# NVlabs/ODISE

Hardware: AMD Instinct MI355X
Metric: panoptic-inference images/sec @1024x1024 (higher is better)
Workload: dtype f16

## Files before the change

### include/odise_hip_tools.h

```cpp
#ifndef ODISE_HIP_TOOLS_H
#define ODISE_HIP_TOOLS_H

#include "odise_hip.h"

#ifdef __cplusplus
extern "C" {
#endif

int odise_hip_sizeof_gemm_desc(void);
int odise_hip_sizeof_conv_desc(void);
int odise_hip_sizeof_attn_desc(void);
int odise_hip_sizeof_post_desc(void);
int odise_hip_sizeof_infer_desc(void);

int odise_hip_gemm_forced(odise_hip_ctx* ctx, const odise_gemm_desc* d, int tile, int splitk);
int odise_hip_conv2d_forced(odise_hip_ctx* ctx, const odise_conv_desc* d, int tile, int splitk);
int odise_hip_last_tile(void);
int odise_hip_gemm_ln(odise_hip_ctx* ctx, const odise_gemm_desc* d, const float* part, int parts, float inv_c, float eps, const float* colsum,
                      float* final_out, const float* fin, const float* rowsum, float* stats_out);
int odise_hip_conv2d_gn_forced(odise_hip_ctx* ctx, const odise_conv_desc* d, int tile, int splitk, const float* gamma, const float* beta,
                               int groups, float eps, int act, void* y_norm, float* stats_scratch, int* stats_blocks);
int odise_hip_gemm_debug(int flags);

int odise_hip_post_generic(int on);
int odise_hip_sem_tile(int tile);
int odise_hip_gn_tuning(int chunk_factor, int fold_in_apply);
int odise_hip_msda_unfused(int on);
int odise_hip_msda_fused_forward(odise_hip_ctx* ctx, const void* value, const float* off, const float* aw, const int* hs3, const int* ws3, int B, int M, int fused,
                                 void* out, float* loc_scratch, float* w_scratch);

int odise_hip_stage_timeline(odise_hip_ctx* ctx, int on);
int odise_hip_stage_timeline_read(odise_hip_ctx* ctx, char* names, int names_cap, float* gpu_ms, double* host_ms, int cap, int* n);

int odise_hip_prefetch_stats(odise_hip_ctx* ctx, int* enqueued, int* hits, int* dropped, int* failed);

int odise_hip_launch_log(odise_hip_ctx* ctx, int on);
int odise_hip_launch_log_read(odise_hip_ctx* ctx, int* out6, int cap, int* n);

int odise_hip_set_lanes(odise_hip_ctx* ctx, int lanes);

int odise_hip_backbone_maps(odise_hip_ctx* ctx, float** out4, int* shape_bchw4x4);

int odise_hip_mfma_probe(odise_hip_ctx* ctx, float* host_out);

int odise_hip_maskclip_token_mask(odise_hip_ctx* ctx, const void* logits_f16, void* out_u8, int B, int Q, int h, int w, int S, int patch, int T,
                                  int64_t ldm, int plain);
#ifdef __cplusplus
}
#endif
#endif
```

### odise_amd/csrc/common.h

```cpp
#pragma once
#include <hip/hip_runtime.h>
#include <hip/hip_fp16.h>
#include <stdint.h>
#include <stdio.h>
#include <atomic>
#include <string>

#include "../../include/odise_hip.h"

namespace odise {

typedef _Float16 f16;
typedef _Float16 f16x4 __attribute__((ext_vector_type(4)));
typedef _Float16 f16x8 __attribute__((ext_vector_type(8)));
typedef float f32x4 __attribute__((ext_vector_type(4)));
typedef float f32x16 __attribute__((ext_vector_type(16)));

void set_error(const char* fmt, ...);

#define ODISE_CHECK_HIP(expr)                                                              \
    do {                                                                                   \
        hipError_t _e = (expr);                                                            \
        if (_e != hipSuccess) {                                                            \
            ::odise::set_error("%s:%d: %s failed: %s", __FILE__, __LINE__, #expr,          \
                               hipGetErrorString(_e));                                     \
            return ODISE_ERR_HIP;                                                          \
        }                                                                                  \
    } while (0)

#define ODISE_REQUIRE(cond, ...)                                                           \
    do {                                                                                   \
        if (!(cond)) {                                                                     \
            ::odise::set_error(__VA_ARGS__);                                               \
            return ODISE_ERR_ARG;                                                          \
        }                                                                                  \
    } while (0)

#define ODISE_TRY(expr)                \
    do {                               \
        int _rc = (expr);              \
        if (_rc != ODISE_OK) return _rc; \
    } while (0)

static inline int64_t ceil_div(int64_t a, int64_t b) { return (a + b - 1) / b; }
static inline int64_t round_up(int64_t a, int64_t b) { return ceil_div(a, b) * b; }

__device__ __forceinline__ float mul_sigmoid(float x, float kx) { return x * __builtin_amdgcn_rcpf(1.0f + __expf(-kx)); }

__device__ __forceinline__ float gelu_erf(float v) {
    const float x = v * 0.70710678118654752f;
    const float a = fabsf(x);
    const float t = __builtin_amdgcn_rcpf(1.0f + 0.3275911f * a);
    const float p = t * (0.254829592f + t * (-0.284496736f + t * (1.421413741f + t * (-1.453152027f + t * 1.061405429f))));
    const float r = 1.0f - p * __expf(-a * a);
    return 0.5f * v * (1.0f + copysignf(r, x));
}

__device__ __forceinline__ float act_apply(float v, int act) {
    switch (act) {
        case ODISE_ACT_SILU: return mul_sigmoid(v, v);
        case ODISE_ACT_RELU: return v > 0.f ? v : 0.f;
        case ODISE_ACT_GELU: return gelu_erf(v);
        case ODISE_ACT_QUICKGELU: return mul_sigmoid(v, 1.702f * v);
        default: return v;
    }
}

}

struct odise_hip_ctx {
    int device = 0;
    hipStream_t stream = nullptr;
    bool own_stream = false;
    int cu_count = 256;
    int max_lds_optin = 65536;
    void* ws = nullptr;
    size_t ws_bytes = 0;
    void* zeros = nullptr;
    hipEvent_t ev0 = nullptr, ev1 = nullptr;
    void* models = nullptr;
    void* jpeg_host = nullptr;
    size_t jpeg_host_bytes = 0;
    void* jpeg_dev = nullptr;
    size_t jpeg_dev_bytes = 0;
    hipEvent_t jpeg_ev = nullptr;
    hipStream_t stream2 = nullptr;
    void* ws2 = nullptr;
    hipEvent_t ev_fork = nullptr, ev_mid = nullptr, ev_join = nullptr;
    hipEvent_t ev_mclip = nullptr;
    int lanes = 2;
    int prefetch_cu_eighths = 0;
    int prefetch_start = 1;
    hipStream_t stream3 = nullptr;
    void* ws3 = nullptr;
    hipEvent_t ev_pf_go = nullptr, ev_pf_done = nullptr;
    void* comm = nullptr;
    int clip_ln_fold = 0;
    int maskclip_passes = 0;
    int attn_kv_resident = 0;
    int64_t vae_chunk_bytes = 0;
    void* probe = nullptr;
    void* stages = nullptr;
    void* launch_log = nullptr;
    void* rle_buf = nullptr;
    size_t rle_bytes = 0;
};

namespace odise {
struct LdsAttrOnce {
    std::atomic<uint64_t> done{0};
};
static inline int ensure_dyn_lds(odise_hip_ctx* ctx, LdsAttrOnce& once, const void* kernel, int bytes) {
    const int d = ctx->device;
    if (d >= 0 && d < 64 && ((once.done.load(std::memory_order_acquire) >> d) & 1)) return ODISE_OK;
    ODISE_CHECK_HIP(hipFuncSetAttribute(kernel, hipFuncAttributeMaxDynamicSharedMemorySize, bytes));
    if (d >= 0 && d < 64) once.done.fetch_or(1ull << d, std::memory_order_release);
    return ODISE_OK;
}
}

namespace odise {
struct LaunchProbe {
    int conv = 0, M = 0, N = 0, K = 0;
    int cap = 0, n = 0;
    hipEvent_t* ev = nullptr;
    bool armed = false;
};
static inline LaunchProbe* probe_match(odise_hip_ctx* ctx, bool conv, int M, int N, int K) {
    LaunchProbe* p = (LaunchProbe*)ctx->probe;
    return (p && p->armed && p->n < p->cap && (p->conv != 0) == conv && p->M == M && p->N == N && p->K == K) ? p : nullptr;
}
void probe_release(odise_hip_ctx* ctx);
void stage_mark(odise_hip_ctx* ctx, const char* name);
void stage_log_release(odise_hip_ctx* ctx);
struct LaunchRec { int conv, M, N, K, tile, split; };
void launch_log_push(odise_hip_ctx* ctx, const LaunchRec& r);
void launch_log_release(odise_hip_ctx* ctx);
constexpr int kLnPartCols = 64;
struct LnEpi {
    const float* part = nullptr;
    int P = 0;
    float inv_c = 0.f, eps = 0.f;
    const float* colsum = nullptr;
    float* final_out = nullptr;
    const float* fin = nullptr;
    const float* rowsum = nullptr;
    float* stats_out = nullptr;
};
bool conv3_c8_ok(const odise_conv_desc* d);
int launch_conv3_c8(odise_hip_ctx* ctx, const odise_conv_desc* d, float* gn_stats, int* stats_blocks);
int gemm_forced(odise_hip_ctx* ctx, const odise_gemm_desc* d, int force_tile, int force_split, const LnEpi* ln = nullptr);
int gemm_ln(odise_hip_ctx* ctx, const odise_gemm_desc* d, const LnEpi& ln);
void jpeg_release(odise_hip_ctx* ctx);
void rle_release(odise_hip_ctx* ctx);
void comm_release(odise_hip_ctx* ctx);
}
```

### odise_amd/csrc/engine.cpp

```cpp
#include <stdlib.h>

#include "engine.h"

#include <string.h>

namespace odise {

void unet_destroy(ModelStore* ms);
void extractor_destroy(ModelStore* ms);
void maskgen_destroy(ModelStore* ms);
void classify_destroy(ModelStore* ms);

ModelStore* store_of(odise_hip_ctx* ctx) {
    if (!ctx->models) ctx->models = new ModelStore();
    return (ModelStore*)ctx->models;
}

void free_allocs(std::vector<void*>& owned) {
    if (owned.empty()) return;
    (void)hipDeviceSynchronize();
    for (void* p : owned) (void)hipFree(p);
    owned.clear();
}

void models_destroy(odise_hip_ctx* ctx) {
    if (!ctx->models) return;
    ModelStore* ms = (ModelStore*)ctx->models;
    unet_destroy(ms);
    extractor_destroy(ms);
    maskgen_destroy(ms);
    classify_destroy(ms);
    for (void* p : ms->dev_allocs) (void)hipFree(p);
    if (ms->arena.base) (void)hipFree(ms->arena.base);
    if (ms->arena2.base) (void)hipFree(ms->arena2.base);
    if (ms->mclip.buf) (void)hipFree(ms->mclip.buf);
    for (Arena& a : ms->pf.arena)
        if (a.base) (void)hipFree(a.base);
    delete ms;
    ctx->models = nullptr;
}

int ensure_prefetch_lane(odise_hip_ctx* ctx, ModelStore* ms, int slot, size_t arena_bytes) {
    if (!ctx->stream3) {
        int lo = 0, hi = 0;
        ODISE_CHECK_HIP(hipDeviceGetStreamPriorityRange(&lo, &hi));
        const int e8 = ctx->prefetch_cu_eighths;
        hipStream_t st = nullptr;
        void* ws = nullptr;
        hipEvent_t go = nullptr, done = nullptr;
        hipError_t err;
        if (e8 >= 1 && e8 <= 7) {
            uint32_t mask[8];
            const uint32_t byte = (1u << e8) - 1u;
            for (uint32_t& m : mask) m = byte * 0x01010101u;
            err = hipExtStreamCreateWithCUMask(&st, 8, mask);
        } else {
            err = hipStreamCreateWithPriority(&st, hipStreamNonBlocking, lo);
        }
        if (err == hipSuccess) err = hipMalloc(&ws, ctx->ws_bytes);
        if (err == hipSuccess) err = hipEventCreateWithFlags(&go, hipEventDisableTiming);
        if (err == hipSuccess) err = hipEventCreateWithFlags(&done, hipEventDisableTiming);
        if (err != hipSuccess) {
            if (done) (void)hipEventDestroy(done);
            if (go) (void)hipEventDestroy(go);
            if (ws) (void)hipFree(ws);
            if (st) (void)hipStreamDestroy(st);
            set_error("prefetch lane: %s", hipGetErrorString(err));
            return ODISE_ERR_HIP;
        }
        ctx->stream3 = st; ctx->ws3 = ws; ctx->ev_pf_go = go; ctx->ev_pf_done = done;
    }
    Arena& a = ms->pf.arena[slot];
    if (a.cap < arena_bytes) {
        ODISE_CHECK_HIP(hipStreamSynchronize(ctx->stream3));
        ODISE_CHECK_HIP(hipStreamSynchronize(ctx->stream));
        if (a.base) ODISE_CHECK_HIP(hipFree(a.base));
        a = Arena();
        ODISE_CHECK_HIP(hipMalloc((void**)&a.base, arena_bytes));
        a.cap = arena_bytes;
    }
    return ODISE_OK;
}

int ensure_lane2(odise_hip_ctx* ctx, ModelStore* ms, size_t arena_bytes) {
    if (!ctx->stream2) {
        int lo = 0, hi = 0;
        ODISE_CHECK_HIP(hipDeviceGetStreamPriorityRange(&lo, &hi));
        int prio = hi;
#ifdef ODISE_TOOLS
        if (getenv("ODISE_LANE2_NORMAL_PRIORITY")) prio = lo;
#endif
        ODISE_CHECK_HIP(hipStreamCreateWithPriority(&ctx->stream2, hipStreamNonBlocking, prio));
        ODISE_CHECK_HIP(hipMalloc(&ctx->ws2, ctx->ws_bytes));
        ODISE_CHECK_HIP(hipEventCreateWithFlags(&ctx->ev_fork, hipEventDisableTiming));
        ODISE_CHECK_HIP(hipEventCreateWithFlags(&ctx->ev_mid, hipEventDisableTiming));
        ODISE_CHECK_HIP(hipEventCreateWithFlags(&ctx->ev_join, hipEventDisableTiming));
        ODISE_CHECK_HIP(hipEventCreateWithFlags(&ctx->ev_mclip, hipEventDisableTiming));
    }
    if (ms->arena2.cap < arena_bytes) {
        ODISE_CHECK_HIP(hipStreamSynchronize(ctx->stream));
        ODISE_CHECK_HIP(hipStreamSynchronize(ctx->stream2));
        if (ms->arena2.base) ODISE_CHECK_HIP(hipFree(ms->arena2.base));
        ms->arena2 = Arena();
        ODISE_CHECK_HIP(hipMalloc((void**)&ms->arena2.base, arena_bytes));
        ms->arena2.cap = arena_bytes;
    }
    return ODISE_OK;
}

const HostTensor* Packer::find(const std::string& key) {
    auto it = ms->host.find(prefix + key);
    if (it == ms->host.end()) {
        if (missing.empty()) missing = prefix + key;
        return nullptr;
    }
    return &it->second;
}

int Packer::upload(const void* host, size_t bytes, void** dev) {
    ODISE_CHECK_HIP(hipMalloc(dev, bytes ? bytes : 16));
    ms->track(*dev);
    ODISE_CHECK_HIP(hipMemcpy(*dev, host, bytes, hipMemcpyHostToDevice));
    return ODISE_OK;
}

int Packer::vec_f32(const std::string& key, float** out, int64_t expect) {
    const HostTensor* t = find(key);
    if (!t) {
        set_error("weights: missing key '%s'", (prefix + key).c_str());
        return ODISE_ERR_STATE;
    }
    if (t->numel() != expect) {
        set_error("weights: '%s' has %lld elements, expected %lld", (prefix + key).c_str(), (long long)t->numel(), (long long)expect);
        return ODISE_ERR_STATE;
    }
    return upload(t->data.data(), t->data.size() * sizeof(float), (void**)out);
}

int Packer::conv(const std::string& key, ConvW& out, bool bias) {
    const HostTensor* t = find(key + ".weight");
    if (!t || t->shape.size() != 4) {
        set_error("weights: missing or non-4D conv weight '%s.weight'", (prefix + key).c_str());
        return ODISE_ERR_STATE;
    }
    const int O = (int)t->shape[0], I = (int)t->shape[1], KH = (int)t->shape[2], KW = (int)t->shape[3];
    if (KH != KW) {
        set_error("weights: non-square conv kernel '%s'", (prefix + key).c_str());
        return ODISE_ERR_STATE;
    }
    const int Ip = (int)round_up(I, 8);
    std::vector<f16> packed((size_t)O * KH * KW * Ip, (f16)0.f);
    for (int o = 0; o < O; ++o)
        for (int i = 0; i < I; ++i)
            for (int y = 0; y < KH; ++y)
                for (int x = 0; x < KW; ++x)
                    packed[(((size_t)o * KH + y) * KW + x) * Ip + i] = (f16)t->data[(((size_t)o * I + i) * KH + y) * KW + x];
    out.cin = I; out.cin_pad = Ip; out.cout = O; out.k = KH;
    ODISE_TRY(upload(packed.data(), packed.size() * sizeof(f16), (void**)&out.w));
    out.b = nullptr;
    if (bias) ODISE_TRY(vec_f32(key + ".bias", &out.b, O));
    return ODISE_OK;
}

int Packer::linear(const std::string& key, LinW& out, bool bias) {
    const HostTensor* t = find(key + ".weight");
    if (!t || t->shape.size() < 2) {
        set_error("weights: missing linear weight '%s.weight'", (prefix + key).c_str());
        return ODISE_ERR_STATE;
    }
    const int O = (int)t->shape[0], I = (int)t->shape[1];
    if (t->numel() != (int64_t)O * I || I % 8 != 0) {
        set_error("weights: '%s.weight' is not a [O,I] / [O,I,1,1] matrix with I %% 8 == 0", (prefix + key).c_str());
        return ODISE_ERR_STATE;
    }
    std::vector<f16> packed((size_t)O * I);
    for (size_t i = 0; i < packed.size(); ++i) packed[i] = (f16)t->data[i];
    out.in = I; out.out = O;
    ODISE_TRY(upload(packed.data(), packed.size() * sizeof(f16), (void**)&out.w));
    out.b = nullptr;
    if (bias) ODISE_TRY(vec_f32(key + ".bias", &out.b, O));
    return ODISE_OK;
}

int Packer::norm(const std::string& key, NormW& out) {
    const HostTensor* t = find(key + ".weight");
    if (!t) {
        set_error("weights: missing norm weight '%s.weight'", (prefix + key).c_str());
        return ODISE_ERR_STATE;
    }
    out.c = (int)t->numel();
    ODISE_TRY(vec_f32(key + ".weight", &out.g, out.c));
    ODISE_TRY(vec_f32(key + ".bias", &out.b, out.c));
    return ODISE_OK;
}

void* Exec::alloc_bytes(size_t bytes) {
    void* p = ms->arena.alloc(bytes);
    if (!p) set_error("arena exhausted: need %zu more bytes (capacity %zu, used %zu)", bytes, ms->arena.cap, ms->arena.off);
    return p;
}

int Exec::alloc(Act& a, int n, int h, int w, int c) {
    a.n = n; a.h = h; a.w = w; a.c = c;
    a.p = (f16*)alloc_bytes((size_t)a.elems() * sizeof(f16));
    return a.p ? ODISE_OK : ODISE_ERR_NOMEM;
}

int Exec::gemm(const odise_gemm_desc& d) {
    ms->macs += (double)d.M * d.N * d.K * (d.batch > 1 ? d.batch : 1);
    return odise_hip_gemm(ctx, &d);
}

int Exec::attention(const odise_attn_desc& d) {
    ms->macs += 2.0 * d.B * d.H * (double)d.Lq * d.Lk * d.D;
    return odise_hip_attention(ctx, &d);
}

int Exec::conv(const Act& x, const ConvW& w, Act& y, int stride, int pad, bool upsample, const Act* residual,
               const float* per_image_add, int64_t pia_ld, int act, int pad_t, int pad_l, int oh, int ow) {
    if (x.c != w.cin_pad) {
        set_error("conv: input has %d channels, weight expects %d", x.c, w.cin_pad);
        return ODISE_ERR_ARG;
    }
    if (pad < 0) pad = w.k / 2;
    if (pad_t < 0) pad_t = pad;
    if (pad_l < 0) pad_l = pad;
    const int hin = upsample ? 2 * x.h : x.h, win = upsample ? 2 * x.w : x.w;
    if (oh < 0) oh = (hin + 2 * pad - w.k) / stride + 1;
    if (ow < 0) ow = (win + 2 * pad - w.k) / stride + 1;
    if (!y.p) ODISE_TRY(alloc(y, x.n, oh, ow, w.cout));
    odise_conv_desc d;
    memset(&d, 0, sizeof(d));
    d.N = x.n; d.H = x.h; d.W = x.w; d.Cin = x.c;
    d.Cout = w.cout; d.KH = w.k; d.KW = w.k; d.stride = stride; d.pad_t = pad_t; d.pad_l = pad_l; d.OH = oh; d.OW = ow;
    d.upsample2x = upsample ? 1 : 0;
    d.X = x.p; d.Wt = w.w; d.Y = y.p; d.y_dtype = ODISE_F16;
    d.bias = w.b;
    d.residual = residual ? residual->p : nullptr;
    d.per_image_add = per_image_add;
    d.per_image_add_ld = pia_ld;
    d.act = act;
    ms->macs += (double)x.n * oh * ow * w.cout * w.k * w.k * w.cin;
    y.gn_blocks = 0;
#ifdef ODISE_TOOLS
    if (y.gn_part && getenv("ODISE_NO_GN_FUSION")) return odise_hip_conv2d(ctx, &d);
#endif
    if (y.gn_part) return conv_forced(ctx, &d, -1, 0, y.gn_part, &y.gn_blocks);
    return odise_hip_conv2d(ctx, &d);
}

int Exec::alloc_gn_stats(Act& a) {
    const int64_t blocks = ceil_div((int64_t)a.h * a.w, 64);
    a.gn_part = (float*)alloc_bytes((size_t)a.n * blocks * a.c * 2 * sizeof(float));
    a.gn_blocks = 0;
    return a.gn_part ? ODISE_OK : ODISE_ERR_NOMEM;
}

int Exec::linear(const f16* x, int64_t M, const LinW& w, f16* y, int act, const f16* residual, bool geglu) {
    odise_gemm_desc d;
    memset(&d, 0, sizeof(d));
    d.M = (int)M; d.N = w.out; d.K = w.in;
    d.A = x; d.lda = w.in;
    d.W = w.w; d.ldw = w.in;
    d.C = y; d.ldc = geglu ? w.out / 2 : w.out; d.c_dtype = ODISE_F16;
    d.bias_n = w.b;
    d.residual = residual; d.ldr = d.ldc;
    d.act = act; d.geglu = geglu ? 1 : 0; d.alpha = 1.f; d.batch = 1;
    return gemm(d);
}

int Exec::group_norm(const Act& x, const NormW& w, Act& y, float eps, int act) {
    if (!y.p) ODISE_TRY(alloc(y, x.n, x.h, x.w, x.c));
    if (x.gn_part && x.gn_blocks > 0)
        return group_norm_from_colpart(ctx, x.p, y.p, w.g, w.b, x.n, x.h * x.w, x.c, 32, eps, act, x.gn_part, x.gn_blocks);
    return odise_hip_group_norm(ctx, x.p, y.p, w.g, w.b, x.n, x.h * x.w, x.c, 32, eps, act);
}

int Exec::layer_norm(const f16* x, f16* y, int64_t rows, const NormW& w, float eps) {
    return odise_hip_layer_norm(ctx, x, y, w.g, w.b, (int)rows, w.c, eps);
}

}

using namespace odise;

extern "C" int odise_hip_load_weight(odise_hip_ctx* ctx, const char* name, const float* host_data, const int64_t* shape, int ndim) {
    ODISE_REQUIRE(ctx && name && host_data && (ndim == 0 || shape), "load_weight: null argument");
    ODISE_REQUIRE(ndim >= 0 && ndim <= 4, "load_weight: rank %d not in [0,4]", ndim);
    ModelStore* ms = store_of(ctx);
    HostTensor t;
    int64_t n = 1;
    for (int i = 0; i < ndim; ++i) {
        ODISE_REQUIRE(shape[i] >= 0, "load_weight: negative dim");
        t.shape.push_back(shape[i]);
        n *= shape[i];
    }
    t.data.assign(host_data, host_data + n);
    ms->host[std::string(name)] = std::move(t);
    return ODISE_OK;
}

extern "C" int odise_hip_clear_host_weights(odise_hip_ctx* ctx) {
    ODISE_REQUIRE(ctx, "clear_host_weights: null context");
    store_of(ctx)->host.clear();
    return ODISE_OK;
}
```

### odise_amd/csrc/engine.h

```cpp
#pragma once
#include <map>
#include <utility>
#include <string>
#include <vector>

#include "common.h"

namespace odise {

struct HostTensor {
    std::vector<float> data;
    std::vector<int64_t> shape;
    int64_t numel() const {
        int64_t n = 1;
        for (auto s : shape) n *= s;
        return n;
    }
};

struct Arena {
    char* base = nullptr;
    size_t cap = 0, off = 0, peak = 0;
    void* alloc(size_t bytes) {
        off = (off + 255) & ~(size_t)255;
        if (off + bytes > cap) return nullptr;
        void* p = base + off;
        off += bytes;
        if (off > peak) peak = off;
        return p;
    }
    size_t mark() const { return off; }
    void release(size_t m) { off = m; }
    void reset() { off = 0; }
};

struct Act {
    f16* p = nullptr;
    int n = 0, h = 0, w = 0, c = 0;
    float* gn_part = nullptr;
    int gn_blocks = 0;
    int64_t pixels() const { return (int64_t)n * h * w; }
    int64_t elems() const { return pixels() * c; }
};

struct ConvW {
    f16* w = nullptr;
    float* b = nullptr;
    int cin = 0, cin_pad = 0, cout = 0, k = 1;
};
struct LinW {
    f16* w = nullptr;
    float* b = nullptr;
    int in = 0, out = 0;
};
struct NormW {
    float* g = nullptr;
    float* b = nullptr;
    int c = 0;
};

struct UNetModel;

struct EncoderOut {
    Act tap0, tap1;
    Act xt, zdec;
};
struct PrefetchKey {
    int B = 0, layout = 0;
    std::vector<const void*> images;
    std::vector<int> hw;
    bool operator==(const PrefetchKey& o) const { return B == o.B && layout == o.layout && images == o.images && hw == o.hw; }
};
struct Prefetch {
    bool has_pending = false, has_ready = false;
    PrefetchKey pending, ready;
    int ready_slot = 0;
    EncoderOut out;
    int crops = 0;
    bool use_now = false;
    int n_enqueued = 0, n_hits = 0, n_dropped = 0, n_failed = 0;
    Arena arena[2];
};

struct ClipKV {
    void* buf = nullptr;
    size_t cap = 0;
    f16* qk = nullptr;
    f16* vt = nullptr;
    f16* cls = nullptr;
    int B = 0, TP = 0, layers = 0, width = 0;
    size_t qk_stride = 0, vt_stride = 0;
    int64_t ldvt = 0;
    const float* plan_image = nullptr;
    int plan_B = 0, plan_H = 0, plan_W = 0;
    bool planned = false, ready = false, on_lane2 = false;
};

struct ModelStore {
    std::map<std::string, HostTensor> host;
    std::vector<void*> dev_allocs;
    std::vector<void*>* alloc_sink = nullptr;
    void track(void* p) { (alloc_sink ? *alloc_sink : dev_allocs).push_back(p); }
    Arena arena;
    Arena arena2;
    Prefetch pf;
    ClipKV mclip;
    UNetModel* unet = nullptr;
    struct ExtractorModel* extractor = nullptr;
    struct MaskGenModel* maskgen = nullptr;
    struct ClassifyModel* classify = nullptr;
    double macs = 0.0;
};

ModelStore* store_of(odise_hip_ctx* ctx);
struct AllocScope {
    ModelStore* ms;
    std::vector<void*>* prev;
    AllocScope(ModelStore* m, std::vector<void*>& owned) : ms(m), prev(m->alloc_sink) { m->alloc_sink = &owned; }
    ~AllocScope() { ms->alloc_sink = prev; }
};
void free_allocs(std::vector<void*>& owned);

struct Packer {
    odise_hip_ctx* ctx;
    ModelStore* ms;
    std::string prefix;
    std::string missing;

    const HostTensor* find(const std::string& key);
    int upload(const void* host, size_t bytes, void** dev);
    int conv(const std::string& key, ConvW& out, bool bias = true);
    int linear(const std::string& key, LinW& out, bool bias = true);
    int norm(const std::string& key, NormW& out);
    int vec_f32(const std::string& key, float** out, int64_t expect);
};

struct Exec {
    odise_hip_ctx* ctx;
    ModelStore* ms;
    int alloc(Act& a, int n, int h, int w, int c);
    int alloc_gn_stats(Act& a);
    void* alloc_bytes(size_t bytes);

    int conv(const Act& x, const ConvW& w, Act& y, int stride = 1, int pad = -1, bool upsample = false, const Act* residual = nullptr,
             const float* per_image_add = nullptr, int64_t pia_ld = 0, int act = ODISE_ACT_NONE, int pad_t = -1, int pad_l = -1,
             int oh = -1, int ow = -1);
    int linear(const f16* x, int64_t M, const LinW& w, f16* y, int act = ODISE_ACT_NONE, const f16* residual = nullptr,
               bool geglu = false);
    int group_norm(const Act& x, const NormW& w, Act& y, float eps, int act);
    int layer_norm(const f16* x, f16* y, int64_t rows, const NormW& w, float eps);
    int gemm(const odise_gemm_desc& d);
    int attention(const odise_attn_desc& d);
};


int ensure_lane2(odise_hip_ctx* ctx, ModelStore* ms, size_t arena_bytes);
struct Lane2 {
    odise_hip_ctx* ctx;
    ModelStore* ms;
    hipStream_t s0;
    void* w0;
    Lane2(odise_hip_ctx* c, ModelStore* m) : ctx(c), ms(m), s0(c->stream), w0(c->ws) {
        ctx->stream = ctx->stream2;
        ctx->ws = ctx->ws2;
        std::swap(ms->arena, ms->arena2);
    }
    ~Lane2() {
        ctx->stream = s0;
        ctx->ws = w0;
        std::swap(ms->arena, ms->arena2);
    }
};

int ensure_prefetch_lane(odise_hip_ctx* ctx, ModelStore* ms, int slot, size_t arena_bytes);
struct PrefetchLane {
    odise_hip_ctx* ctx;
    ModelStore* ms;
    int slot;
    hipStream_t s0;
    void* w0;
    void* stages0;
    PrefetchLane(odise_hip_ctx* c, ModelStore* m, int sl) : ctx(c), ms(m), slot(sl), s0(c->stream), w0(c->ws), stages0(c->stages) {
        ctx->stream = ctx->stream3;
        ctx->ws = ctx->ws3;
        ctx->stages = nullptr;
        std::swap(ms->arena, ms->pf.arena[slot]);
    }
    ~PrefetchLane() {
        ctx->stream = s0;
        ctx->ws = w0;
        ctx->stages = stages0;
        std::swap(ms->arena, ms->pf.arena[slot]);
    }
};

int ensure_arena(odise_hip_ctx* ctx, ModelStore* ms, size_t bytes);
int unet_build(odise_hip_ctx* ctx, const char* prefix);
int unet_prepare_timestep(odise_hip_ctx* ctx, ModelStore* ms, UNetModel* u, int B, int t);
int unet_launch(odise_hip_ctx* ctx, ModelStore* ms, UNetModel* u, const float* x_t, const f16* x_nhwc, const float* context,
                const float* cond_emb, int B, int h, int w, bool standalone);
const Act* unet_taps(ModelStore* ms);
size_t extractor_arena_bytes(int B, int H, int W);
const Act* extractor_taps(ModelStore* ms);
bool extractor_ready(ModelStore* ms);
int extractor_launch(odise_hip_ctx* ctx, ModelStore* ms, const float* image, int B, int H, int W, bool standalone, bool join = true);
int extractor_join(odise_hip_ctx* ctx);
int extractor_encoder_only(odise_hip_ctx* ctx, ModelStore* ms, const float* image, int B, int H, int W, EncoderOut& out);
size_t encoder_arena_bytes(int B, int H, int W);

struct LatentW {
    float wq[4][8];
    float bq[4];
    float wp[4][4];
    float bp[4];
    float scale, qa, qb;
};
int launch_latent_heads(odise_hip_ctx* ctx, const f16* h, const float* noise, f16* xt, f16* zdec, float* latent, int B, int P,
                        const LatentW& w);
int launch_image_to_nhwc(odise_hip_ctx* ctx, const float* x, f16* y, int N, int C, int HW, int Cpad, const float* scale3,
                         const float* shift3);
int launch_clip_preprocess(odise_hip_ctx* ctx, const float* x, f16* y, int N, int H, int W, int S);
int launch_softmax_rows(odise_hip_ctx* ctx, const f16* x, f16* y, int64_t rows, int cols, int64_t ld, float scale);
int launch_clip_assemble(odise_hip_ctx* ctx, const f16* patches, const float* cls, const float* pos, f16* tok, int B, int T, int extra,
                         int TP, int Cw);
int clip_tower(Exec& ex, const Act& img, int extra, const uint8_t* mask, int64_t ldm, f16* out, ClipKV* kv = nullptr, int kv_images = 0);
bool maskclip_kv_available(odise_hip_ctx* ctx, ModelStore* ms, int B);
int maskclip_image_pass(Exec& ex, const float* image01, int B, int H, int W);
int maskclip_mask_pass(Exec& ex, int Q, const uint8_t* mask, int64_t ldm, int64_t stride_mask, f16* out);
int maskclip_planned_pass(odise_hip_ctx* ctx, ModelStore* ms);
int clip_dims(ModelStore* ms, int* image, int* patch, int* tokens, int* out_dim);
int launch_cond_inputs(odise_hip_ctx* ctx, const float* proj, const float* A1, const float* A2, float* out, int B, int T, int Cw);


int launch_crop_extract(odise_hip_ctx* ctx, const float* img, float* crops, int B, int C, int H, int W, int S, int K, const int* boxes_dev);
int launch_crop_resize_bicubic(odise_hip_ctx* ctx, const float* img, float* crops, int B, int C, int H, int W, int s, int S, int K, const int* boxes_dev);
int launch_upsample_nearest(odise_hip_ctx* ctx, const f16* x, f16* y, int N, int H, int W, int OH, int OW, int C);
int launch_stitch(odise_hip_ctx* ctx, const f16* feat, f16* out, float* out_nchw, int B, int K, const int* boxes_dev, int ch, int cw, int OH,
                  int OW, int C);
int launch_broadcast_rows(odise_hip_ctx* ctx, const f16* x, f16* y, int64_t n, int B);
int layer_norm_add_table(odise_hip_ctx* ctx, const void* x, void* y, const float* gamma, const float* beta, int rows, int C, float eps, f16* y2,
                         const float* table, int P);
int launch_add_vec_table(odise_hip_ctx* ctx, const f16* x, const float* vec, const float* table, f16* y, int64_t N, int P, int C);
bool msda_fused_ok(int M, int D, int L, int P);
int launch_msda_fused(odise_hip_ctx* ctx, const f16* value, const float* off, const float* aw, f16* out, const int* Hs, const int* Ws, const int* starts, int B,
                      int S, int M, int Lq, int ld_off = 0, int ld_aw = 0);
int launch_msda_prepare(odise_hip_ctx* ctx, const float* off, const float* aw, float* loc, float* w, int B, int Lq, int M, int L, int P,
                        const int* Hs, const int* Ws, const int* starts);
int launch_bilinear_add(odise_hip_ctx* ctx, const f16* a, const f16* b, f16* y, int N, int H, int W, int OH, int OW, int C);
int launch_mask_binarize_f16(odise_hip_ctx* ctx, const f16* mask, f16* m01, float* inv, int64_t rows, int HW);
int launch_attn_mask(odise_hip_ctx* ctx, const f16* logits, uint8_t* out, int64_t rows, int H, int W, int oh, int ow, int64_t ldm);
int launch_attn_mask_f32(odise_hip_ctx* ctx, const float* logits, uint8_t* out, int64_t rows, int H, int W, int oh, int ow, int64_t ldm);


struct PostGeom {
    int h4, w4;
    int ph, pw;
    int ih, iw;
    int oh, ow;
    int Q, Qpad;
};
int launch_resize_bilinear_norm(odise_hip_ctx* ctx, const float* x, f16* y, int B, int H, int W, int S);
int launch_maskclip_token_mask(odise_hip_ctx* ctx, const f16* logits, uint8_t* out, int B, int Q, int h, int w, int S, int patch, int T,
                               int64_t ldm);
int launch_l2_normalize_f16(odise_hip_ctx* ctx, const f16* x, f16* y, int64_t rows, int C);
int launch_l2_normalize_f32(odise_hip_ctx* ctx, const float* x, f16* y, int64_t rows, int C);
int launch_classify_rows(odise_hip_ctx* ctx, const float* L1, const float* L2, const int* seg, const int* ovl, const float* binary, float* out, int64_t rows, int K,
                         int Ktot, float ls1, float ls2, float alpha, float beta);
int launch_postprocess_pixels(odise_hip_ctx* ctx, const f16* logits, const float* kscore, f16* S, int* ids, int* counts, const PostGeom& g, const f16* PT = nullptr,
                              float* sem = nullptr, int K = 0, unsigned int* stats_partial = nullptr);
bool postprocess_pixels_tiled(const PostGeom& g);
int postprocess_pixels_stat_blocks(const PostGeom& g);
int launch_column_fold(odise_hip_ctx* ctx, const unsigned int* partial, float* out2, int nb, int Qpad);
bool postprocess_pixels_fuses_semantic(const PostGeom& g);
int launch_column_stats(odise_hip_ctx* ctx, const f16* S, unsigned int* partial, float* out2, int npix, int Qpad);
int launch_panoptic_write(odise_hip_ctx* ctx, const int* ids, const int* map, int* seg, int npix);
int launch_instance_masks(odise_hip_ctx* ctx, const f16* logits, const int* idx, float* out, int n, const PostGeom& g, const int* n_dev = nullptr);
bool instance_masks_x4(const PostGeom& g);
int launch_post_decide(odise_hip_ctx* ctx, const float* mask_cls, float* kscore, int* label, f16* semT, float* probs, int B, int Q, int Qpad, int K,
                       float object_mask_threshold);
int launch_panoptic_decide(odise_hip_ctx* ctx, const int* counts, const float* kscore, const int* label, const uint8_t* isthing, int* map, int* table,
                           int Q, int K, double overlap_threshold, int max_segments, int* stuff_scratch);
int launch_instance_topk(odise_hip_ctx* ctx, const float* probs, const float* inst_stats, const uint8_t* isthing, int* table, float* scores, int B,
                         int Q, int Qpad, int K, int topk, int things_only);
int launch_image_pad(odise_hip_ctx* ctx, const void* src, int layout, int h, int w, float* dst, int Hp, int Wp);
int launch_semantic_argmax(odise_hip_ctx* ctx, const f16* S, const f16* PT, int* out, int npix, int Qpad, int K);
struct HeadOutputs {
    const f16* pred_masks;
    const f16* mask_embed;
    int B, Q, C, h4, w4;
    float logit_scale;
    const float* class_logits;
};
int head_outputs(ModelStore* ms, HeadOutputs* out);
void maskgen_invalidate_outputs(ModelStore* ms);

int conv_forced(odise_hip_ctx* ctx, const odise_conv_desc* d, int force_tile, int force_split, float* gn_stats, int* stats_blocks);
int group_norm_from_colpart(odise_hip_ctx* ctx, const void* x, void* y, const float* gamma, const float* beta, int N, int HW, int C, int groups,
                            float eps, int act, const float* colpart, int nblk);

}
```

### odise_amd/csrc/extractor.cpp

```cpp
#include <math.h>
#include <string.h>

#include <functional>
#include "engine.h"

namespace odise {

struct VaeRes {
    NormW n1, n2;
    ConvW c1, c2, nin;
    bool has_nin = false;
};
struct VaeAttn {
    NormW norm;
    LinW qk, v, proj;
    float* v_bias = nullptr;
    int c = 0;
};
struct ClipBlock {
    NormW ln1, ln2;
    LinW qk, v, out, fc, proj;
    float* v_bias = nullptr;
    LinW qk_f, v_f, fc_f;
    float *qk_cs = nullptr, *v_cs = nullptr, *fc_cs = nullptr, *v_f_bias = nullptr;
};

struct ExtractorModel {
    std::vector<void*> owned;
    bool built = false;
    ConvW enc_conv_in, enc_conv_out;
    VaeRes enc_blocks[4][2];
    ConvW enc_down[3];
    VaeRes enc_mid1, enc_mid2;
    VaeAttn enc_attn;
    NormW enc_norm_out;
    ConvW dec_conv_in;
    VaeRes dec_mid1, dec_mid2;
    VaeAttn dec_attn;
    VaeRes dec_l3[3], dec_l2[2];
    ConvW dec_up3;
    LatentW lat;
    float* noise = nullptr;
    int noise_hw = 0;
    ConvW clip_conv1;
    float *clip_cls = nullptr, *clip_pos = nullptr;
    NormW clip_ln_pre, clip_ln_post;
    std::vector<ClipBlock> clip_blocks;
    LinW clip_proj;
    int clip_width = 0, clip_heads = 16, clip_tokens = 0, clip_image = 336, clip_patch = 14, clip_out = 768;
    LinW cap_proj;
    LinW cap_time;
    float *cap_A1 = nullptr, *cap_A2 = nullptr;
    int ctx_dim = 768, ted = 1280;
    Act taps[8];
    double last_macs = 0.0;
};

void extractor_destroy(ModelStore* ms) {
    if (ms->extractor) free_allocs(ms->extractor->owned);
    delete ms->extractor;
    ms->extractor = nullptr;
}

static int build_vae_res(Packer& pk, const std::string& key, VaeRes& r) {
    ODISE_TRY(pk.norm(key + ".norm1", r.n1));
    ODISE_TRY(pk.conv(key + ".conv1", r.c1));
    ODISE_TRY(pk.norm(key + ".norm2", r.n2));
    ODISE_TRY(pk.conv(key + ".conv2", r.c2));
    r.has_nin = pk.find(key + ".nin_shortcut.weight") != nullptr;
    if (r.has_nin) ODISE_TRY(pk.conv(key + ".nin_shortcut", r.nin));
    return ODISE_OK;
}

static int build_vae_attn(Packer& pk, const std::string& key, VaeAttn& a) {
    ODISE_TRY(pk.norm(key + ".norm", a.norm));
    a.c = a.norm.c;
    const HostTensor *wq = pk.find(key + ".q.weight"), *wk = pk.find(key + ".k.weight"), *bq = pk.find(key + ".q.bias"),
                     *bk = pk.find(key + ".k.bias");
    const size_t cc = (size_t)a.c * a.c;
    if (!wq || !wk || !bq || !bk || (size_t)wq->numel() != cc || (size_t)wk->numel() != cc) {
        set_error("vae: bad or missing '%s.q/k'", key.c_str());
        return ODISE_ERR_STATE;
    }
    std::vector<f16> qk(2 * cc);
    std::vector<float> b(2 * (size_t)a.c);
    for (size_t i = 0; i < cc; ++i) { qk[i] = (f16)wq->data[i]; qk[cc + i] = (f16)wk->data[i]; }
    for (int i = 0; i < a.c; ++i) { b[i] = bq->data[i]; b[a.c + i] = bk->data[i]; }
    a.qk.in = a.c; a.qk.out = 2 * a.c;
    ODISE_TRY(pk.upload(qk.data(), qk.size() * sizeof(f16), (void**)&a.qk.w));
    ODISE_TRY(pk.upload(b.data(), b.size() * sizeof(float), (void**)&a.qk.b));
    ODISE_TRY(pk.linear(key + ".v", a.v, false));
    ODISE_TRY(pk.vec_f32(key + ".v.bias", &a.v_bias, a.c));
    ODISE_TRY(pk.linear(key + ".proj_out", a.proj));
    return ODISE_OK;
}

static int fold_layer_norm(Packer& pk, const float* W, const float* bias, int O, int I, const float* gamma, const float* beta, LinW& lw, float** bias_dev,
                           float** cs_dev) {
    std::vector<f16> wf((size_t)O * I);
    std::vector<float> bf(O), cs(O);
    for (int o = 0; o < O; ++o) {
        double bb = bias[o], c = 0.0;
        for (int i = 0; i < I; ++i) {
            const float w = W[(size_t)o * I + i];
            const f16 h = (f16)(w * gamma[i]);
            wf[(size_t)o * I + i] = h;
            c += (double)(float)h;
            bb += (double)w * beta[i];
        }
        bf[o] = (float)bb;
        cs[o] = (float)c;
    }
    lw.in = I; lw.out = O; lw.b = nullptr;
    ODISE_TRY(pk.upload(wf.data(), wf.size() * sizeof(f16), (void**)&lw.w));
    ODISE_TRY(pk.upload(bf.data(), bf.size() * sizeof(float), (void**)bias_dev));
    ODISE_TRY(pk.upload(cs.data(), cs.size() * sizeof(float), (void**)cs_dev));
    return ODISE_OK;
}

static int build_clip_block(Packer& pk, const std::string& key, ClipBlock& b, int W) {
    ODISE_TRY(pk.norm(key + ".ln_1", b.ln1));
    ODISE_TRY(pk.norm(key + ".ln_2", b.ln2));
    const HostTensor* w = pk.find(key + ".attn.in_proj_weight");
    const HostTensor* bias = pk.find(key + ".attn.in_proj_bias");
    if (!w || !bias || w->numel() != (int64_t)3 * W * W || bias->numel() != 3 * W) {
        set_error("clip: bad or missing '%s.attn.in_proj_*'", key.c_str());
        return ODISE_ERR_STATE;
    }
    const size_t ww = (size_t)W * W;
    std::vector<f16> qk(2 * ww), v(ww);
    for (size_t i = 0; i < 2 * ww; ++i) qk[i] = (f16)w->data[i];
    for (size_t i = 0; i < ww; ++i) v[i] = (f16)w->data[2 * ww + i];
    b.qk.in = W; b.qk.out = 2 * W;
    ODISE_TRY(pk.upload(qk.data(), qk.size() * sizeof(f16), (void**)&b.qk.w));
    ODISE_TRY(pk.upload(bias->data.data(), (size_t)2 * W * sizeof(float), (void**)&b.qk.b));
    b.v.in = W; b.v.out = W; b.v.b = nullptr;
    ODISE_TRY(pk.upload(v.data(), v.size() * sizeof(f16), (void**)&b.v.w));
    ODISE_TRY(pk.upload(bias->data.data() + 2 * W, (size_t)W * sizeof(float), (void**)&b.v_bias));
    ODISE_TRY(pk.linear(key + ".attn.out_proj", b.out));
    ODISE_TRY(pk.linear(key + ".mlp.c_fc", b.fc));
    ODISE_TRY(pk.linear(key + ".mlp.c_proj", b.proj));
    const HostTensor *g1 = pk.find(key + ".ln_1.weight"), *b1 = pk.find(key + ".ln_1.bias");
    const HostTensor *g2 = pk.find(key + ".ln_2.weight"), *b2 = pk.find(key + ".ln_2.bias");
    const HostTensor *fw = pk.find(key + ".mlp.c_fc.weight"), *fb = pk.find(key + ".mlp.c_fc.bias");
    if (!g1 || !b1 || !g2 || !b2 || !fw || !fb || g1->numel() != W || b1->numel() != W || g2->numel() != W || b2->numel() != W ||
        fw->numel() != (int64_t)4 * W * W || fb->numel() != 4 * W) {
        set_error("clip: bad or missing '%s.ln_* / mlp.c_fc'", key.c_str());
        return ODISE_ERR_STATE;
    }
    ODISE_TRY(fold_layer_norm(pk, w->data.data(), bias->data.data(), 2 * W, W, g1->data.data(), b1->data.data(), b.qk_f, &b.qk_f.b, &b.qk_cs));
    ODISE_TRY(fold_layer_norm(pk, w->data.data() + 2 * ww, bias->data.data() + 2 * W, W, W, g1->data.data(), b1->data.data(), b.v_f, &b.v_f_bias, &b.v_cs));
    ODISE_TRY(fold_layer_norm(pk, fw->data.data(), fb->data.data(), 4 * W, W, g2->data.data(), b2->data.data(), b.fc_f, &b.fc_f.b, &b.fc_cs));
    return ODISE_OK;
}

static int extractor_build(odise_hip_ctx* ctx) {
    ModelStore* ms = store_of(ctx);
    extractor_destroy(ms);
    ms->pf.has_pending = ms->pf.has_ready = ms->pf.use_now = false;
    ExtractorModel* e = new ExtractorModel();
    ms->extractor = e;
    ODISE_TRY(unet_build(ctx, "model.diffusion_model."));
    AllocScope scope(ms, e->owned);
    Packer pk{ctx, ms, "first_stage_model.", ""};
    ODISE_TRY(pk.conv("encoder.conv_in", e->enc_conv_in));
    for (int l = 0; l < 4; ++l) {
        for (int b = 0; b < 2; ++b)
            ODISE_TRY(build_vae_res(pk, "encoder.down." + std::to_string(l) + ".block." + std::to_string(b), e->enc_blocks[l][b]));
        if (l < 3) ODISE_TRY(pk.conv("encoder.down." + std::to_string(l) + ".downsample.conv", e->enc_down[l]));
    }
    ODISE_TRY(build_vae_res(pk, "encoder.mid.block_1", e->enc_mid1));
    ODISE_TRY(build_vae_attn(pk, "encoder.mid.attn_1", e->enc_attn));
    ODISE_TRY(build_vae_res(pk, "encoder.mid.block_2", e->enc_mid2));
    ODISE_TRY(pk.norm("encoder.norm_out", e->enc_norm_out));
    ODISE_TRY(pk.conv("encoder.conv_out", e->enc_conv_out));
    ODISE_TRY(pk.conv("decoder.conv_in", e->dec_conv_in));
    ODISE_TRY(build_vae_res(pk, "decoder.mid.block_1", e->dec_mid1));
    ODISE_TRY(build_vae_attn(pk, "decoder.mid.attn_1", e->dec_attn));
    ODISE_TRY(build_vae_res(pk, "decoder.mid.block_2", e->dec_mid2));
    for (int b = 0; b < 3; ++b) ODISE_TRY(build_vae_res(pk, "decoder.up.3.block." + std::to_string(b), e->dec_l3[b]));
    ODISE_TRY(pk.conv("decoder.up.3.upsample.conv", e->dec_up3));
    for (int b = 0; b < 2; ++b) ODISE_TRY(build_vae_res(pk, "decoder.up.2.block." + std::to_string(b), e->dec_l2[b]));
    {
        const HostTensor *wq = pk.find("quant_conv.weight"), *bq = pk.find("quant_conv.bias"), *wp = pk.find("post_quant_conv.weight"),
                         *bp = pk.find("post_quant_conv.bias");
        if (!wq || !bq || !wp || !bp || wq->numel() != 64 || bq->numel() != 8 || wp->numel() != 16 || bp->numel() != 4) {
            set_error("vae: bad or missing quant_conv / post_quant_conv (expected 8x8 and 4x4 1x1 convs)");
            return ODISE_ERR_STATE;
        }
        for (int c = 0; c < 4; ++c) {
            for (int k = 0; k < 8; ++k) e->lat.wq[c][k] = wq->data[c * 8 + k];
            e->lat.bq[c] = bq->data[c];
            for (int k = 0; k < 4; ++k) e->lat.wp[c][k] = wp->data[c * 4 + k];
            e->lat.bp[c] = bp->data[c];
        }
        e->lat.scale = 0.18215f;
        const double beta0 = pow(sqrt(0.00085), 2.0);
        e->lat.qa = (float)sqrt(1.0 - beta0);
        e->lat.qb = (float)sqrt(1.0 - (1.0 - beta0));
    }
    Packer pc{ctx, ms, "clip.visual.", ""};
    ODISE_TRY(pc.conv("conv1", e->clip_conv1, false));
    e->clip_width = e->clip_conv1.cout;
    e->clip_patch = e->clip_conv1.k;
    const HostTensor* pos = pc.find("positional_embedding");
    if (!pos || pos->shape.size() != 2 || pos->shape[1] != e->clip_width) {
        set_error("clip: bad or missing visual.positional_embedding");
        return ODISE_ERR_STATE;
    }
    e->clip_tokens = (int)pos->shape[0];
    {
        const int grid = (int)lround(sqrt((double)(e->clip_tokens - 1)));
        e->clip_image = grid * e->clip_patch;
    }
    ODISE_TRY(pc.vec_f32("positional_embedding", &e->clip_pos, (int64_t)e->clip_tokens * e->clip_width));
    ODISE_TRY(pc.vec_f32("class_embedding", &e->clip_cls, e->clip_width));
    ODISE_TRY(pc.norm("ln_pre", e->clip_ln_pre));
    ODISE_TRY(pc.norm("ln_post", e->clip_ln_post));
    for (int i = 0;; ++i) {
        const std::string key = "transformer.resblocks." + std::to_string(i);
        if (!pc.find(key + ".ln_1.weight")) break;
        ClipBlock b;
        ODISE_TRY(build_clip_block(pc, key, b, e->clip_width));
        e->clip_blocks.push_back(b);
    }
    if (e->clip_blocks.empty()) {
        set_error("clip: no transformer.resblocks found");
        return ODISE_ERR_STATE;
    }
    e->clip_heads = e->clip_width / 64;
    {
        const HostTensor* pr = pc.find("proj");
        if (!pr || pr->shape.size() != 2 || pr->shape[0] != e->clip_width) {
            set_error("clip: bad or missing visual.proj");
            return ODISE_ERR_STATE;
        }
        e->clip_out = (int)pr->shape[1];
        std::vector<f16> wt((size_t)e->clip_out * e->clip_width);
        for (int o = 0; o < e->clip_out; ++o)
            for (int i = 0; i < e->clip_width; ++i) wt[(size_t)o * e->clip_width + i] = (f16)pr->data[(size_t)i * e->clip_out + o];
        e->clip_proj.in = e->clip_width; e->clip_proj.out = e->clip_out; e->clip_proj.b = nullptr;
        ODISE_TRY(pc.upload(wt.data(), wt.size() * sizeof(f16), (void**)&e->clip_proj.w));
    }
    Packer pf{ctx, ms, "backbone.feature_extractor.", ""};
    ODISE_TRY(pf.linear("clip_project.linear", e->cap_proj));
    e->ctx_dim = e->cap_proj.out;
    {
        const HostTensor *unc = pf.find("ldm_extractor.ldm.uncond_inputs"), *alpha = pf.find("alpha_cond"),
                         *posc = pf.find("clip_project.positional_embedding");
        const int64_t n = (int64_t)77 * e->ctx_dim;
        if (!unc || !alpha || !posc || unc->numel() != n || alpha->numel() != n || posc->numel() != n) {
            set_error("captioner: bad or missing uncond_inputs / alpha_cond / clip_project.positional_embedding");
            return ODISE_ERR_STATE;
        }
        std::vector<float> A1(n), A2(n);
        for (int64_t i = 0; i < n; ++i) {
            A2[i] = tanhf(alpha->data[i]);
            A1[i] = unc->data[i] + A2[i] * posc->data[i];
        }
        ODISE_TRY(pf.upload(A1.data(), n * sizeof(float), (void**)&e->cap_A1));
        ODISE_TRY(pf.upload(A2.data(), n * sizeof(float), (void**)&e->cap_A2));
    }
    {
        const HostTensor *w = pf.find("time_embed_project.linear.weight"), *b = pf.find("time_embed_project.linear.bias"),
                         *post = pf.find("time_embed_project.positional_embedding"), *al = pf.find("alpha_cond_time_embed");
        if (!w || !b || !post || !al || w->shape.size() != 2 || post->numel() != w->shape[0] || al->numel() != w->shape[0]) {
            set_error("captioner: bad or missing time_embed_project / alpha_cond_time_embed (num_timesteps must be 1)");
            return ODISE_ERR_STATE;
        }
        e->ted = (int)w->shape[0];
        const int in = (int)w->shape[1];
        std::vector<f16> wf((size_t)e->ted * in);
        std::vector<float> bf(e->ted);
        for (int o = 0; o < e->ted; ++o) {
            const float t = tanhf(al->data[o]);
            for (int i = 0; i < in; ++i) wf[(size_t)o * in + i] = (f16)(t * w->data[(size_t)o * in + i]);
            bf[o] = t * (b->data[o] + post->data[o]);
        }
        e->cap_time.in = in; e->cap_time.out = e->ted;
        ODISE_TRY(pf.upload(wf.data(), wf.size() * sizeof(f16), (void**)&e->cap_time.w));
        ODISE_TRY(pf.upload(bf.data(), bf.size() * sizeof(float), (void**)&e->cap_time.b));
    }
    {
        const HostTensor* nz = pf.find("ldm_extractor.shared_noise");
        if (!nz || nz->shape.size() != 4 || nz->shape[1] != 4) {
            set_error("extractor: bad or missing ldm_extractor.shared_noise [1,4,h,w]");
            return ODISE_ERR_STATE;
        }
        e->noise_hw = (int)(nz->shape[2] * nz->shape[3]);
        ODISE_TRY(pf.upload(nz->data.data(), nz->data.size() * sizeof(float), (void**)&e->noise));
    }
    e->built = true;
    return ODISE_OK;
}

static Act crop_slice(const Act& a, int n0, int n) {
    Act s = a;
    s.p = a.p + (size_t)n0 * a.h * a.w * a.c;
    s.n = n;
    s.gn_part = nullptr;
    s.gn_blocks = 0;
    return s;
}

static int vae_chunk(const odise_hip_ctx* ctx, int B, size_t per_crop_bytes) {
    if (ctx->vae_chunk_bytes <= 0) return B;
    const int64_t c = ctx->vae_chunk_bytes / (int64_t)per_crop_bytes;
    return (int)std::max<int64_t>(1, std::min<int64_t>(B, c));
}

static int run_vae_res(Exec& ex, const VaeRes& w, const Act& x, Act& out) {
    if (!out.p) ODISE_TRY(ex.alloc(out, x.n, x.h, x.w, w.c1.cout));
    ODISE_REQUIRE(out.n == x.n && out.h == x.h && out.w == x.w && out.c == w.c1.cout, "vae block: output tensor does not match");
    ODISE_TRY(ex.alloc_gn_stats(out));
    const size_t mk = ex.ms->arena.mark();
    Act t1, h, t2, sk;
    ODISE_TRY(ex.group_norm(x, w.n1, t1, 1e-6f, ODISE_ACT_SILU));
    ODISE_TRY(ex.alloc(h, x.n, x.h, x.w, w.c1.cout));
    ODISE_TRY(ex.alloc_gn_stats(h));
    ODISE_TRY(ex.conv(t1, w.c1, h, 1, 1));
    ODISE_TRY(ex.group_norm(h, w.n2, t2, 1e-6f, ODISE_ACT_SILU));
    const Act* resid = &x;
    if (w.has_nin) {
        ODISE_TRY(ex.conv(x, w.nin, sk, 1, 0));
        resid = &sk;
    }
    ODISE_TRY(ex.conv(t2, w.c2, out, 1, 1, false, resid));
    ex.ms->arena.release(mk);
    return ODISE_OK;
}

static int run_vae_attn(Exec& ex, const VaeAttn& w, const Act& x, Act& out) {
    const int C = w.c;
    const int64_t HW = (int64_t)x.h * x.w, M = x.pixels();
    ODISE_TRY(ex.alloc(out, x.n, x.h, x.w, C));
    const size_t mk = ex.ms->arena.mark();
    Act t;
    ODISE_TRY(ex.group_norm(x, w.norm, t, 1e-6f, ODISE_ACT_NONE));
    const int64_t ldv = round_up(HW, 8);
    ODISE_REQUIRE(HW % 8 == 0, "vae attention: H*W=%lld must be a multiple of 8", (long long)HW);
    f16* qk = (f16*)ex.alloc_bytes((size_t)M * 2 * C * 2);
    f16* vt = (f16*)ex.alloc_bytes((size_t)x.n * C * ldv * 2);
    f16* S = (f16*)ex.alloc_bytes((size_t)x.n * HW * ldv * 2);
    f16* o = (f16*)ex.alloc_bytes((size_t)M * C * 2);
    if (!qk || !vt || !S || !o) return ODISE_ERR_NOMEM;
    ODISE_TRY(ex.linear(t.p, M, w.qk, qk));
    odise_gemm_desc d;
    memset(&d, 0, sizeof(d));
    d.M = C; d.N = (int)HW; d.K = C;
    d.A = w.v.w; d.lda = C; d.W = t.p; d.ldw = C; d.strideW = HW * C;
    d.C = vt; d.ldc = ldv; d.strideC = (int64_t)C * ldv; d.c_dtype = ODISE_F16;
    d.bias_m = w.v_bias; d.alpha = 1.f; d.batch = x.n;
    ODISE_TRY(ex.gemm(d));
    memset(&d, 0, sizeof(d));
    d.M = (int)HW; d.N = (int)HW; d.K = C;
    d.A = qk; d.lda = 2 * C; d.strideA = HW * 2 * C;
    d.W = qk + C; d.ldw = 2 * C; d.strideW = HW * 2 * C;
    d.C = S; d.ldc = ldv; d.strideC = HW * ldv; d.c_dtype = ODISE_F16;
    d.alpha = 1.0f / sqrtf((float)C); d.batch = x.n;
    ODISE_TRY(ex.gemm(d));
    ODISE_TRY(launch_softmax_rows(ex.ctx, S, S, (int64_t)x.n * HW, (int)HW, ldv, 1.0f));
    memset(&d, 0, sizeof(d));
    d.M = (int)HW; d.N = C; d.K = (int)HW;
    d.A = S; d.lda = ldv; d.strideA = HW * ldv;
    d.W = vt; d.ldw = ldv; d.strideW = (int64_t)C * ldv;
    d.C = o; d.ldc = C; d.strideC = HW * C; d.c_dtype = ODISE_F16;
    d.alpha = 1.f; d.batch = x.n;
    ODISE_TRY(ex.gemm(d));
    ODISE_TRY(ex.linear(o, M, w.proj, out.p, ODISE_ACT_NONE, x.p));
    ex.ms->arena.release(mk);
    return ODISE_OK;
}

int clip_tower(Exec& ex, const Act& img, int extra, const uint8_t* mask, int64_t ldm, f16* out, ClipKV* kv, int kv_images) {
    ExtractorModel* e = ex.ms->extractor;
    const int B = img.n, S = e->clip_image, Wd = e->clip_width, T = e->clip_tokens, G = S / e->clip_patch;
    const int TA = T + extra;
    const int TP = (int)round_up(TA, 8);
    const size_t mk = ex.ms->arena.mark();
    Act patches;
    ODISE_TRY(ex.conv(img, e->clip_conv1, patches, e->clip_patch, 0, false, nullptr, nullptr, 0, ODISE_ACT_NONE, 0, 0, G, G));
    const int64_t M = (int64_t)B * TP;
    const int64_t ldvt = kv ? kv->ldvt : M;
    const int Bk = kv ? kv_images : 0;
    ODISE_REQUIRE(!kv || (extra == 0 && Bk >= 1 && Bk <= B && kv->B == Bk && kv->TP == TP), "clip_tower: key / value store laid out for another batch");
    f16* x = (f16*)ex.alloc_bytes((size_t)M * Wd * 2);
    f16* x2 = (f16*)ex.alloc_bytes((size_t)M * Wd * 2);
    f16* n = (f16*)ex.alloc_bytes((size_t)M * Wd * 2);
    f16* qk = kv ? kv->qk : (f16*)ex.alloc_bytes((size_t)M * 2 * Wd * 2);
    f16* vt = kv ? kv->vt : (f16*)ex.alloc_bytes((size_t)Wd * ldvt * 2);
    f16* att = (f16*)ex.alloc_bytes((size_t)M * Wd * 2);
    f16* hid = (f16*)ex.alloc_bytes((size_t)M * 4 * Wd * 2);
    if (!x || !x2 || !n || !qk || !vt || !att || !hid) return ODISE_ERR_NOMEM;
    if (TP > TA) ODISE_CHECK_HIP(hipMemsetAsync(att, 0, (size_t)M * Wd * 2, ex.ctx->stream));
    ODISE_TRY(launch_clip_assemble(ex.ctx, patches.p, e->clip_cls, e->clip_pos, n, B, T, extra, TP, Wd));
    ODISE_TRY(ex.layer_norm(n, x, M, e->clip_ln_pre, 1e-5f));
    if (kv) ODISE_TRY(launch_broadcast_rows(ex.ctx, x, kv->cls, Wd, 1));
    const int heads = e->clip_heads, D = Wd / heads;
    const int fold_mode = ex.ctx->clip_ln_fold;
    const bool fold = Wd % 256 == 0 && (fold_mode == 1 || (fold_mode == 0 && M >= 8192));
    const int P = Wd / kLnPartCols;
    float *part_a = nullptr, *part_b = nullptr, *fin = nullptr;
    if (fold) {
        part_a = (float*)ex.alloc_bytes((size_t)M * P * 2 * sizeof(float));
        part_b = (float*)ex.alloc_bytes((size_t)M * P * 2 * sizeof(float));
        fin = (float*)ex.alloc_bytes((size_t)M * 2 * sizeof(float));
        if (!part_a || !part_b || !fin) return ODISE_ERR_NOMEM;
    }
    auto lin = [&](const f16* a, const LinW& w, f16* y, int act, const f16* residual, const LnEpi& ln) -> int {
        odise_gemm_desc d;
        memset(&d, 0, sizeof(d));
        d.M = (int)M; d.N = w.out; d.K = w.in;
        d.A = a; d.lda = w.in; d.W = w.w; d.ldw = w.in;
        d.C = y; d.ldc = w.out; d.c_dtype = ODISE_F16;
        d.bias_n = w.b; d.residual = residual; d.ldr = w.out;
        d.act = act; d.alpha = 1.f; d.batch = 1;
        ex.ms->macs += (double)d.M * d.N * d.K;
        return gemm_ln(ex.ctx, &d, ln);
    };
    bool first = true;
    int layer = 0;
    for (const ClipBlock& b : e->clip_blocks) {
        const bool folded1 = fold && !first;
        first = false;
        if (kv) {
            qk = kv->qk + (size_t)layer * kv->qk_stride;
            vt = kv->vt + (size_t)layer * kv->vt_stride;
            ++layer;
        }
        odise_gemm_desc d;
        memset(&d, 0, sizeof(d));
        d.M = Wd; d.N = (int)M; d.K = Wd;
        d.lda = Wd; d.ldw = Wd;
        d.C = vt; d.ldc = ldvt; d.c_dtype = ODISE_F16;
        d.alpha = 1.f; d.batch = 1;
        if (folded1) {
            LnEpi l1;
            l1.part = part_b; l1.P = P; l1.inv_c = 1.f / (float)Wd; l1.eps = 1e-5f; l1.colsum = b.qk_cs; l1.final_out = fin;
            ODISE_TRY(lin(x, b.qk_f, qk, ODISE_ACT_NONE, nullptr, l1));
            LnEpi lv;
            lv.fin = fin; lv.rowsum = b.v_cs;
            d.A = b.v_f.w; d.W = x; d.bias_m = b.v_f_bias;
            ex.ms->macs += (double)d.M * d.N * d.K;
            ODISE_TRY(gemm_ln(ex.ctx, &d, lv));
        } else {
            ODISE_TRY(ex.layer_norm(x, n, M, b.ln1, 1e-5f));
            ODISE_TRY(ex.linear(n, M, b.qk, qk));
            d.A = b.v.w; d.W = n; d.bias_m = b.v_bias;
            ODISE_TRY(ex.gemm(d));
        }
        const bool last = &b == &e->clip_blocks.back();
        if (kv && last && Bk == B) {
            ex.ms->arena.release(mk);
            return ODISE_OK;
        }
        odise_attn_desc a;
        memset(&a, 0, sizeof(a));
        const bool cls_only = extra == 0 && last;
        a.B = B; a.H = heads; a.Lq = cls_only ? 1 : TA; a.Lk = T; a.D = D;
        a.Q = qk; a.ldq = 2 * Wd; a.strideQ = (int64_t)TP * 2 * Wd;
        a.K = qk + Wd; a.ldk = 2 * Wd; a.strideK = (int64_t)TP * 2 * Wd;
        a.Vt = vt; a.ldvt = ldvt; a.strideVt = TP;
        a.O = att; a.ldo = Wd; a.strideO = (int64_t)TP * Wd;
        if (extra > 0) { a.mask = mask; a.ldmask = ldm; a.strideMask = (int64_t)TA * ldm; }
        a.scale = 1.0f / sqrtf((float)D);
        if (Bk > 0 && Bk < B) {
            odise_attn_desc ac = a;
            ac.B = B - Bk;
            ac.Q = qk + (size_t)Bk * a.strideQ; ac.K = qk + Wd + (size_t)Bk * a.strideK; ac.Vt = vt + (size_t)Bk * a.strideVt; ac.O = att + (size_t)Bk * a.strideO;
            ODISE_TRY(ex.attention(ac));
            if (!last) {
                a.B = Bk;
                ODISE_TRY(ex.attention(a));
            }
        } else {
            ODISE_TRY(ex.attention(a));
        }
        if (cls_only) {
            const int Bc = B - Bk;
            const size_t skip = (size_t)Bk * TP * Wd;
            f16* x2c = (f16*)ex.alloc_bytes((size_t)Bc * Wd * 2);
            f16* nc = (f16*)ex.alloc_bytes((size_t)Bc * Wd * 2);
            f16* hc = (f16*)ex.alloc_bytes((size_t)Bc * 4 * Wd * 2);
            f16* xc = (f16*)ex.alloc_bytes((size_t)Bc * Wd * 2);
            if (!x2c || !nc || !hc || !xc) return ODISE_ERR_NOMEM;
            memset(&d, 0, sizeof(d));
            d.M = Bc; d.N = Wd; d.K = Wd;
            d.A = att + skip; d.lda = (int64_t)TP * Wd; d.W = b.out.w; d.ldw = Wd;
            d.C = x2c; d.ldc = Wd; d.c_dtype = ODISE_F16; d.bias_n = b.out.b;
            d.residual = x + skip; d.ldr = (int64_t)TP * Wd; d.alpha = 1.f; d.batch = 1;
            ODISE_TRY(ex.gemm(d));
            ODISE_TRY(ex.layer_norm(x2c, nc, Bc, b.ln2, 1e-5f));
            ODISE_TRY(ex.linear(nc, Bc, b.fc, hc, ODISE_ACT_QUICKGELU));
            ODISE_TRY(ex.linear(hc, Bc, b.proj, xc, ODISE_ACT_NONE, x2c));
            ODISE_TRY(ex.layer_norm(xc, nc, Bc, e->clip_ln_post, 1e-5f));
            memset(&d, 0, sizeof(d));
            d.M = Bc; d.N = e->clip_out; d.K = Wd; d.A = nc; d.lda = Wd; d.W = e->clip_proj.w; d.ldw = Wd;
            d.C = out; d.ldc = e->clip_out; d.c_dtype = ODISE_F16; d.alpha = 1.f; d.batch = 1;
            ODISE_TRY(ex.gemm(d));
            ex.ms->arena.release(mk);
            return ODISE_OK;
        }
        if (fold) {
            LnEpi lo, lf, lp;
            lo.stats_out = part_a;
            ODISE_TRY(lin(att, b.out, x2, ODISE_ACT_NONE, x, lo));
            lf.part = part_a; lf.P = P; lf.inv_c = 1.f / (float)Wd; lf.eps = 1e-5f; lf.colsum = b.fc_cs;
            ODISE_TRY(lin(x2, b.fc_f, hid, ODISE_ACT_QUICKGELU, nullptr, lf));
            lp.stats_out = part_b;
            ODISE_TRY(lin(hid, b.proj, x, ODISE_ACT_NONE, x2, lp));
        } else {
            ODISE_TRY(ex.linear(att, M, b.out, x2, ODISE_ACT_NONE, x));
            ODISE_TRY(ex.layer_norm(x2, n, M, b.ln2, 1e-5f));
            ODISE_TRY(ex.linear(n, M, b.fc, hid, ODISE_ACT_QUICKGELU));
            ODISE_TRY(ex.linear(hid, M, b.proj, x, ODISE_ACT_NONE, x2));
        }
    }
    ODISE_TRY(ex.layer_norm(x, n, M, e->clip_ln_post, 1e-5f));
    odise_gemm_desc d;
    memset(&d, 0, sizeof(d));
    d.N = e->clip_out; d.K = Wd; d.W = e->clip_proj.w; d.ldw = Wd;
    d.C = out; d.ldc = e->clip_out; d.c_dtype = ODISE_F16; d.alpha = 1.f;
    if (extra == 0) {
        d.M = B; d.A = n; d.lda = (int64_t)TP * Wd; d.batch = 1;
    } else {
        d.M = extra; d.A = n + (size_t)T * Wd; d.lda = Wd; d.strideA = (int64_t)TP * Wd;
        d.strideC = (int64_t)extra * e->clip_out; d.batch = B;
    }
    ODISE_TRY(ex.gemm(d));
    ex.ms->arena.release(mk);
    return ODISE_OK;
}


static int maskclip_kv_layout(odise_hip_ctx* ctx, ModelStore* ms, int B, int others) {
    const ExtractorModel* e = ms->extractor;
    ClipKV& kv = ms->mclip;
    kv.ready = false;
    const int Wd = e->clip_width, L = (int)e->clip_blocks.size();
    const int TP = (int)round_up(e->clip_tokens, 8);
    const size_t Mp = (size_t)B * TP, Mo = (size_t)others * TP;
    const size_t rows = Mp * L + Mo;
    const size_t need = (rows * 2 * Wd + (size_t)Wd * rows + Wd) * sizeof(f16) + 256;
    if (kv.cap < need) {
        ODISE_CHECK_HIP(hipDeviceSynchronize());
        if (kv.buf) ODISE_CHECK_HIP(hipFree(kv.buf));
        kv.buf = nullptr;
        kv.cap = 0;
        ODISE_CHECK_HIP(hipMalloc(&kv.buf, need + need / 8));
        kv.cap = need + need / 8;
    }
    kv.qk = (f16*)kv.buf;
    kv.vt = kv.qk + rows * 2 * Wd;
    kv.cls = kv.vt + (size_t)Wd * rows;
    kv.B = B; kv.TP = TP; kv.layers = L; kv.width = Wd;
    kv.qk_stride = Mp * 2 * Wd; kv.vt_stride = Mp; kv.ldvt = (int64_t)rows;
    return ODISE_OK;
}

bool maskclip_kv_available(odise_hip_ctx* ctx, ModelStore* ms, int B) {
    if (maskclip_kv_layout(ctx, ms, B, 0) == ODISE_OK) return true;
    (void)hipGetLastError();
    return false;
}

int maskclip_image_pass(Exec& ex, const float* image01, int B, int H, int W) {
    ExtractorModel* e = ex.ms->extractor;
    ODISE_TRY(maskclip_kv_layout(ex.ctx, ex.ms, B, 0));
    const int S = e->clip_image;
    const size_t mk = ex.ms->arena.mark();
    Act img;
    int rc = ex.alloc(img, B, S, S, 8);
    if (rc == ODISE_OK) rc = launch_resize_bilinear_norm(ex.ctx, image01, img.p, B, H, W, S);
    if (rc == ODISE_OK) rc = clip_tower(ex, img, 0, nullptr, 0, nullptr, &ex.ms->mclip, B);
    ex.ms->arena.release(mk);
    return rc;
}

int maskclip_mask_pass(Exec& ex, int Q, const uint8_t* mask, int64_t ldm, int64_t stride_mask, f16* out) {
    ExtractorModel* e = ex.ms->extractor;
    const ClipKV& kv = ex.ms->mclip;
    const int B = kv.B, TP = kv.TP, Wd = e->clip_width, T = e->clip_tokens, heads = e->clip_heads, D = Wd / heads;
    ODISE_REQUIRE(kv.buf && kv.layers == (int)e->clip_blocks.size() && kv.width == Wd, "maskclip: the image-token pass has not run for this tower");
    const int64_t M = (int64_t)B * Q;
    const size_t mk = ex.ms->arena.mark();
    f16* x = (f16*)ex.alloc_bytes((size_t)M * Wd * 2);
    f16* x2 = (f16*)ex.alloc_bytes((size_t)M * Wd * 2);
    f16* n = (f16*)ex.alloc_bytes((size_t)M * Wd * 2);
    f16* q = (f16*)ex.alloc_bytes((size_t)M * Wd * 2);
    f16* att = (f16*)ex.alloc_bytes((size_t)M * Wd * 2);
    f16* hid = (f16*)ex.alloc_bytes((size_t)M * 4 * Wd * 2);
    if (!x || !x2 || !n || !q || !att || !hid) return ODISE_ERR_NOMEM;
    ODISE_TRY(launch_broadcast_rows(ex.ctx, kv.cls, x, Wd, (int)M));
    int layer = 0;
    for (const ClipBlock& b : e->clip_blocks) {
        ODISE_TRY(ex.layer_norm(x, n, M, b.ln1, 1e-5f));
        LinW wq = b.qk;
        wq.out = Wd;
        ODISE_TRY(ex.linear(n, M, wq, q));
        odise_attn_desc a;
        memset(&a, 0, sizeof(a));
        a.B = B; a.H = heads; a.Lq = Q; a.Lk = T; a.D = D;
        a.Q = q; a.ldq = Wd; a.strideQ = (int64_t)Q * Wd;
        a.K = kv.qk + (size_t)layer * kv.qk_stride + Wd; a.ldk = 2 * Wd; a.strideK = (int64_t)TP * 2 * Wd;
        a.Vt = kv.vt + (size_t)layer * kv.vt_stride; a.ldvt = kv.ldvt; a.strideVt = TP;
        a.O = att; a.ldo = Wd; a.strideO = (int64_t)Q * Wd;
        a.mask = mask; a.ldmask = ldm; a.strideMask = stride_mask;
        a.scale = 1.0f / sqrtf((float)D);
        ODISE_TRY(ex.attention(a));
        ODISE_TRY(ex.linear(att, M, b.out, x2, ODISE_ACT_NONE, x));
        ODISE_TRY(ex.layer_norm(x2, n, M, b.ln2, 1e-5f));
        ODISE_TRY(ex.linear(n, M, b.fc, hid, ODISE_ACT_QUICKGELU));
        ODISE_TRY(ex.linear(hid, M, b.proj, x, ODISE_ACT_NONE, x2));
        ++layer;
    }
    ODISE_TRY(ex.layer_norm(x, n, M, e->clip_ln_post, 1e-5f));
    odise_gemm_desc d;
    memset(&d, 0, sizeof(d));
    d.M = (int)M; d.N = e->clip_out; d.K = Wd; d.A = n; d.lda = Wd; d.W = e->clip_proj.w; d.ldw = Wd;
    d.C = out; d.ldc = e->clip_out; d.c_dtype = ODISE_F16; d.alpha = 1.f; d.batch = 1;
    ODISE_TRY(ex.gemm(d));
    ex.ms->arena.release(mk);
    return ODISE_OK;
}

int clip_dims(ModelStore* ms, int* image, int* patch, int* tokens, int* out_dim) {
    ExtractorModel* e = ms->extractor;
    if (!e || !e->built) return ODISE_ERR_STATE;
    if (image) *image = e->clip_image;
    if (patch) *patch = e->clip_patch;
// ... 328 lines not shown
```

### odise_amd/csrc/gemm.hip

```cpp
#include "common.h"
#include <stdlib.h>

#ifdef ODISE_TOOLS
#define ODISE_ABLATE(g, bit) ((g).dbg & (bit))
#else
#define ODISE_ABLATE(g, bit) false
#endif

namespace odise {

struct GemmEpi {
    void* C;
    int64_t ldc;
    int c_dtype;
    const float* bias_n;
    const float* bias_m;
    const float* scale_m;
    const f16* residual;
    int64_t ldr;
    const float* rowgroup_add;
    int rows_per_group;
    int64_t ldg;
    int act;
    int geglu;
    float alpha;
    int64_t strideC, strideR;
    int fast;
    int f16path;
    const float* ln_part;
    int ln_P;
    float ln_inv_c, ln_eps;
    const float* ln_colsum;
    float* ln_final_out;
    const float* ln_final;
    const float* ln_rowsum;
    float* ln_stats_out;
    float* gn_stats;
};

struct ConvGeom {
    int H, W, Cin, KH, KW, stride, pad_t, pad_l, OH, OW, ups;
    int chunk_major;
    int halo_tx, halo_ty;
};

struct GemmArgs {
    int M, N, K;
    const f16* A;
    int64_t lda, strideA;
    const f16* W;
    int64_t ldw, strideW;
    GemmEpi epi;
    ConvGeom cg;
    int splitk;
    int ktiles_per_split;
    float* ws;
    const f16* zeros;
    int dbg;
    int stats_blocks;
    int epi_block;
};

__device__ __forceinline__ void lds_barrier() {
    asm volatile("s_waitcnt lgkmcnt(0)" ::: "memory");
    __builtin_amdgcn_s_barrier();
}

__device__ __forceinline__ void glds16(const void* gsrc, void* lds_base) {
    __builtin_amdgcn_global_load_lds((const __attribute__((address_space(1))) void*)gsrc,
                                     (__attribute__((address_space(3))) void*)lds_base, 16, 0, 0);
}

__device__ __forceinline__ void epi_store8(const GemmEpi& e, float (&v)[8], int m, int n, int N, int z) {
    const int nvalid = (N - n) < 8 ? (N - n) : 8;
    if (nvalid <= 0) return;
#pragma unroll
    for (int i = 0; i < 8; ++i) {
        float x = v[i] * e.alpha;
        if (e.scale_m) x *= e.scale_m[m];
        if (i < nvalid) {
            if (e.bias_n) x += e.bias_n[n + i];
            if (e.bias_m) x += e.bias_m[m];
            if (e.rowgroup_add) x += e.rowgroup_add[(int64_t)(m / e.rows_per_group) * e.ldg + n + i];
        }
        v[i] = x;
    }
    if (e.geglu) {
        float o[4];
#pragma unroll
        for (int i = 0; i < 4; ++i) o[i] = v[2 * i] * gelu_erf(v[2 * i + 1]);
        const int no = n >> 1;
        const int nov = nvalid >> 1;
        if (e.c_dtype == ODISE_F16) {
            f16* c = (f16*)e.C + (int64_t)z * e.strideC + (int64_t)m * e.ldc + no;
            if (nov == 4 && ((e.ldc & 3) == 0)) {
                f16x4 t;
                t[0] = (f16)o[0]; t[1] = (f16)o[1]; t[2] = (f16)o[2]; t[3] = (f16)o[3];
                *reinterpret_cast<f16x4*>(c) = t;
            } else {
                for (int i = 0; i < nov; ++i) c[i] = (f16)o[i];
            }
        } else {
            float* c = (float*)e.C + (int64_t)z * e.strideC + (int64_t)m * e.ldc + no;
            for (int i = 0; i < nov; ++i) c[i] = o[i];
        }
        return;
    }
#pragma unroll
    for (int i = 0; i < 8; ++i) v[i] = act_apply(v[i], e.act);
    if (e.residual) {
        const f16* r = e.residual + (int64_t)z * e.strideR + (int64_t)m * e.ldr + n;
        if (nvalid == 8 && ((e.ldr & 7) == 0)) {
            const f16x8 t = *reinterpret_cast<const f16x8*>(r);
#pragma unroll
            for (int i = 0; i < 8; ++i) v[i] += (float)t[i];
        } else {
            for (int i = 0; i < nvalid; ++i) v[i] += (float)r[i];
        }
    }
    if (e.c_dtype == ODISE_F16) {
        f16* c = (f16*)e.C + (int64_t)z * e.strideC + (int64_t)m * e.ldc + n;
        if (nvalid == 8 && ((e.ldc & 7) == 0)) {
            f16x8 t;
#pragma unroll
            for (int i = 0; i < 8; ++i) t[i] = (f16)v[i];
            *reinterpret_cast<f16x8*>(c) = t;
        } else {
            for (int i = 0; i < nvalid; ++i) c[i] = (f16)v[i];
        }
    } else {
        float* c = (float*)e.C + (int64_t)z * e.strideC + (int64_t)m * e.ldc + n;
        if (nvalid == 8 && ((e.ldc & 3) == 0)) {
            *reinterpret_cast<float4*>(c) = make_float4(v[0], v[1], v[2], v[3]);
            *reinterpret_cast<float4*>(c + 4) = make_float4(v[4], v[5], v[6], v[7]);
        } else {
            for (int i = 0; i < nvalid; ++i) c[i] = v[i];
        }
    }
}

__device__ __forceinline__ void epi_fast8(const GemmEpi& e, float (&v)[8], int m, int n, int z, float* rounded = nullptr) {
    float b[8];
#pragma unroll
    for (int i = 0; i < 8; ++i) b[i] = 0.f;
    if (e.bias_n) {
        const float4 b0 = *reinterpret_cast<const float4*>(e.bias_n + n);
        const float4 b1 = *reinterpret_cast<const float4*>(e.bias_n + n + 4);
        b[0] = b0.x; b[1] = b0.y; b[2] = b0.z; b[3] = b0.w; b[4] = b1.x; b[5] = b1.y; b[6] = b1.z; b[7] = b1.w;
    }
    if (e.rowgroup_add) {
        const float* rg = e.rowgroup_add + (int64_t)((unsigned)m / (unsigned)e.rows_per_group) * e.ldg + n;
        const float4 r0 = *reinterpret_cast<const float4*>(rg);
        const float4 r1 = *reinterpret_cast<const float4*>(rg + 4);
        b[0] += r0.x; b[1] += r0.y; b[2] += r0.z; b[3] += r0.w; b[4] += r1.x; b[5] += r1.y; b[6] += r1.z; b[7] += r1.w;
    }
    float alpha = e.alpha;
    if (e.scale_m) alpha *= e.scale_m[m];
    if (e.bias_m) {
        const float bm = e.bias_m[m];
#pragma unroll
        for (int i = 0; i < 8; ++i) b[i] += bm;
    }
#pragma unroll
    for (int i = 0; i < 8; ++i) v[i] = v[i] * alpha + b[i];
    if (e.geglu) {
        float o[4];
#pragma unroll
        for (int i = 0; i < 4; ++i) o[i] = v[2 * i] * gelu_erf(v[2 * i + 1]);
        const int64_t off = (int64_t)z * e.strideC + (int64_t)m * e.ldc + (n >> 1);
        if (e.c_dtype == ODISE_F16) {
            f16x4 t;
#pragma unroll
            for (int i = 0; i < 4; ++i) t[i] = (f16)o[i];
            *reinterpret_cast<f16x4*>((f16*)e.C + off) = t;
        } else {
            *reinterpret_cast<float4*>((float*)e.C + off) = make_float4(o[0], o[1], o[2], o[3]);
        }
        return;
    }
    f16x8 r = {0, 0, 0, 0, 0, 0, 0, 0};
    if (e.residual) r = *reinterpret_cast<const f16x8*>(e.residual + (int64_t)z * e.strideR + (int64_t)m * e.ldr + n);
    if (e.act == ODISE_ACT_SILU) {
#pragma unroll
        for (int i = 0; i < 8; ++i) v[i] = mul_sigmoid(v[i], v[i]);
    } else if (e.act == ODISE_ACT_RELU) {
#pragma unroll
        for (int i = 0; i < 8; ++i) v[i] = v[i] > 0.f ? v[i] : 0.f;
    } else if (e.act == ODISE_ACT_QUICKGELU) {
#pragma unroll
        for (int i = 0; i < 8; ++i) v[i] = mul_sigmoid(v[i], 1.702f * v[i]);
    } else if (e.act == ODISE_ACT_GELU) {
#pragma unroll
        for (int i = 0; i < 8; ++i) v[i] = gelu_erf(v[i]);
    }
    const int64_t off = (int64_t)z * e.strideC + (int64_t)m * e.ldc + n;
    if (e.c_dtype == ODISE_F16) {
        f16x8 t;
#pragma unroll
        for (int i = 0; i < 8; ++i) t[i] = (f16)(v[i] + (float)r[i]);
        *reinterpret_cast<f16x8*>((f16*)e.C + off) = t;
        if (rounded) {
#pragma unroll
            for (int i = 0; i < 8; ++i) rounded[i] = (float)t[i];
        }
    } else {
        float* c = (float*)e.C + off;
        *reinterpret_cast<float4*>(c) = make_float4(v[0] + (float)r[0], v[1] + (float)r[1], v[2] + (float)r[2], v[3] + (float)r[3]);
        *reinterpret_cast<float4*>(c + 4) = make_float4(v[4] + (float)r[4], v[5] + (float)r[5], v[6] + (float)r[6], v[7] + (float)r[7]);
    }
}

constexpr int plain_lds_bytes(int BM, int BN, int WAVES_M) {
    const int stage = (BM + BN) * 64 * 2 * 2;
    const int all_rows = BM * (BN + 4) * 4;
    const int f32 = (all_rows > stage && (160 * 1024) / all_rows == (160 * 1024) / stage) ? all_rows : stage;
    const int f16_all = BM * (BN + 8) * 2;
    return (f16_all > f32 && f16_all <= 160 * 1024 && (160 * 1024) / f16_all == (160 * 1024) / f32) ? f16_all : f32;
}
constexpr int pp_lds_bytes(int BM, int BN, int WAVES_M) {
    const int stage = (BM + BN) * 64 * 2 * 2;
    const int half_rows = (BM / 2) * (BN + 4) * 4;
    const int f32 = (half_rows > stage && half_rows <= 160 * 1024) ? half_rows : stage;
    const int f16_all = BM * (BN + 8) * 2;
    return (f16_all > f32 && f16_all <= 160 * 1024) ? f16_all : f32;
}
constexpr int halo_lds_bytes(int BN) {
    const int layout = 2 * BN * 64 * 2 + 2 * (41 + 1) * 1024;
    const int all = 256 * (BN + 4) * 4;
    const int epi = all <= 160 * 1024 ? all : all / 2;
    return layout > epi ? layout : epi;
}
constexpr int epi16_bytes(int BM, int BN, int WAVES_M, int EW) { return EW * (BM / WAVES_M) * (BN + 8) * 2; }
constexpr int epi16_wave_rows(int BM, int BN, int WAVES_M, int lds_bytes) {
    int ew = lds_bytes / ((BM / WAVES_M) * (BN + 8) * 2);
    if (ew < 1) ew = 1;
    if (ew > WAVES_M) ew = WAVES_M;
    while (WAVES_M % ew) --ew;
    return ew;
}
constexpr int epi16_rows_if_enabled(int BM, int BN, int WAVES_M, int lds_bytes) {
    return (BN != 320 && BM * BN >= 256 * 128) ? epi16_wave_rows(BM, BN, WAVES_M, lds_bytes) : 0;
}
constexpr int max_int(int a, int b) { return a > b ? a : b; }
constexpr int halo4_lds_bytes(int BN) {
    const int layout = 2 * BN * 64 * 2 + (41 + 1) * 1024;
    const int f16_all = 256 * (BN + 8) * 2;
    const int f32_row = 64 * (BN + 4) * 4;
    return max_int(max_int(layout, f16_all <= 80 * 1024 ? f16_all : 0), f32_row);
}
constexpr int epi_wave_rows(int BM, int BN, int WAVES_M, int lds_bytes) {
    const int per_row = (BM / WAVES_M) * (BN + 4) * 4;
    int wg = lds_bytes / per_row;
    if (wg < 1) wg = 1;
    if (wg > WAVES_M) wg = WAVES_M;
    while (WAVES_M % wg) --wg;
    return wg;
}
constexpr int epi_lds_bytes(int BM, int BN, int WAVES_M, int WG) { return WG * (BM / WAVES_M) * (BN + 4) * 4; }

struct FragLayout {
    static constexpr int NR = 2, NC = 2;
    static __device__ __forceinline__ int row(int lane, int rr) { return 16 * rr + (lane & 15); }
    static __device__ __forceinline__ int col(int lane, int cc) { return 16 * cc + 4 * (lane >> 4); }
    static __device__ __forceinline__ bool leader(int lane) { return lane < 16; }
    static __device__ __forceinline__ float row_sum(float v) { v += __shfl_xor(v, 16); return v + __shfl_xor(v, 32); }
};
typedef f32x4 AccBlock[4];
template <int BM, int BN, int WAVES_M, int WAVES_N>
using WaveAcc = AccBlock[BM / WAVES_M / 32][BN / WAVES_N / 32];
template <int TM, int TN>
__device__ __forceinline__ float acc_get(const AccBlock (&a)[TM][TN], int p, int j, int r) { return a[p][j][r >> 2][r & 3]; }

template <int BM, int BN, int WAVES_M, int WAVES_N, int EW, bool HALO, bool STATS, bool GEGLU>
__device__ __forceinline__ void gemm_epilogue_f16(const GemmArgs& g, WaveAcc<BM, BN, WAVES_M, WAVES_N>& acc, char* smem, int m0, int n0, int zb) {
    constexpr int NT = 64 * WAVES_M * WAVES_N;
    constexpr int WTM = BM / WAVES_M, WTN = BN / WAVES_N;
    constexpr int TM = WTM / 32, TN = WTN / 32;
    using FL = FragLayout;
    constexpr int NR = FL::NR, NC = FL::NC, TR = TM * NR;
    constexpr int ROWS = EW * WTM;
    constexpr int BNO = GEGLU ? BN / 2 : BN;
    constexpr int PITCH = BN + 8;
    constexpr int CH = BNO / 8;
    constexpr int TOTAL = ROWS * CH, ITERS = (TOTAL + NT - 1) / NT;
    const GemmEpi& e = g.epi;
    const int tid = threadIdx.x;
    const int lane = tid & 63;
    const int wave = tid >> 6;
    const int wm = wave / WAVES_N, wn = wave % WAVES_N;
    f16* stg = reinterpret_cast<f16*>(smem);
    const int NO = GEGLU ? (g.N >> 1) : g.N;
    const int no0 = GEGLU ? (n0 >> 1) : n0;
    auto row_to_m = [&](int rt) -> int {
        if (HALO) {
            const int patch = m0 / BM;
            const int per_img = g.cg.halo_tx * g.cg.halo_ty;
            const int img = patch / per_img, pr = patch - img * per_img;
            const int oy = (pr / g.cg.halo_tx) * 16 + (rt >> 4), ox = (pr % g.cg.halo_tx) * 16 + (rt & 15);
            return (oy < g.cg.OH && ox < g.cg.OW) ? (img * g.cg.OH + oy) * g.cg.OW + ox : g.M;
        }
        return m0 + rt;
    };
    const bool stats = STATS && (NT % CH == 0) && e.gn_stats != nullptr;
    constexpr bool LN_OK = !HALO && !STATS && !GEGLU;
    const float* const ln_part = LN_OK ? e.ln_part : nullptr;
    const float* const ln_colsum = LN_OK ? e.ln_colsum : nullptr;
    float* const ln_final_out = LN_OK ? e.ln_final_out : nullptr;
    const float* const ln_final = LN_OK ? e.ln_final : nullptr;
    const float* const ln_rowsum = LN_OK ? e.ln_rowsum : nullptr;
    float* const ln_stats_out = LN_OK ? e.ln_stats_out : nullptr;
    float s8[8], q8[8];
#pragma unroll
    for (int i = 0; i < 8; ++i) s8[i] = q8[i] = 0.f;
#pragma unroll
    for (int gp = 0; gp < WAVES_M / EW; ++gp) {
        if (gp > 0) lds_barrier();
        if (wm / EW == gp) {
            int mr[TR];
            float alpha_r[TR], bm_r[TR];
            unsigned grp_r[TR];
            constexpr int NPW = (WTN % kLnPartCols == 0) ? WTN / kLnPartCols : 1;
            float r1_r[TR], rs_r[TR], ps_r[TR][NPW], pq_r[TR][NPW];
#pragma unroll
            for (int p = 0; p < TR; ++p) {
                const int m = row_to_m(wm * WTM + (p / NR) * 32 + FL::row(lane, p % NR));
                mr[p] = m;
                const bool ok = m < g.M;
                float alpha = e.alpha;
                if (e.scale_m && ok) alpha *= e.scale_m[m];
                r1_r[p] = rs_r[p] = 0.f;
#pragma unroll
                for (int u = 0; u < NPW; ++u) ps_r[p][u] = pq_r[p][u] = 0.f;
                if (ln_part && ok) {
                    const float* pp = ln_part + (int64_t)m * e.ln_P * 2;
                    float s1 = 0.f, s2 = 0.f;
                    for (int i = 0; i < e.ln_P; ++i) { s1 += pp[2 * i]; s2 += pp[2 * i + 1]; }
                    const float mean = s1 * e.ln_inv_c;
                    const float var = fmaxf(s2 * e.ln_inv_c - mean * mean, 0.f);
                    const float rstd = rsqrtf(var + e.ln_eps);
                    alpha *= rstd;
                    r1_r[p] = -mean * rstd;
                    if (ln_final_out && n0 == 0 && wn == 0 && FL::leader(lane)) {
                        ln_final_out[2 * (int64_t)m] = r1_r[p];
                        ln_final_out[2 * (int64_t)m + 1] = rstd;
                    }
                }
                if (ln_rowsum && ok) rs_r[p] = ln_rowsum[m];
                alpha_r[p] = alpha;
                bm_r[p] = (e.bias_m && ok) ? e.bias_m[m] : 0.f;
                grp_r[p] = (e.rowgroup_add && ok) ? (unsigned)m / (unsigned)e.rows_per_group : 0u;
            }
#pragma unroll
            for (int j = 0; j < TN; ++j)
#pragma unroll
                for (int q = 0; q < NC; ++q) {
                    const int cl = wn * WTN + j * 32 + FL::col(lane, q);
                    const int n = n0 + cl;
                    const bool nok = n < g.N;
                    float4 bn = make_float4(0.f, 0.f, 0.f, 0.f);
                    if (e.bias_n && nok) bn = *reinterpret_cast<const float4*>(e.bias_n + n);
                    float4 cs4 = make_float4(0.f, 0.f, 0.f, 0.f), fa = cs4, fb = cs4;
                    if (ln_colsum && nok) cs4 = *reinterpret_cast<const float4*>(ln_colsum + n);
                    if (ln_final && nok) {
                        fa = *reinterpret_cast<const float4*>(ln_final + 2 * (int64_t)n);
// ... 1233 lines not shown
    __syncthreads();
    if (ODISE_ABLATE(g, 4)) return;
    gemm_epilogue<BM, BN, WAVES_M, WAVES_N, epi_wave_rows(BM, BN, WAVES_M, pp_lds_bytes(BM, BN, WAVES_M)), false, (CONV && BM == 512), true,
                  epi16_rows_if_enabled(BM, BN, WAVES_M, pp_lds_bytes(BM, BN, WAVES_M)), !CONV, pp_lds_bytes(BM, BN, WAVES_M)>(g, acc, smem, m0, n0, z, zb, split);
}


namespace pp2 {
constexpr int read_phase(int l, int JA, int TPB, int PT) { return l < JA ? 0 : ((l - JA) * TPB) / PT; }
constexpr int slot(int l, int JA, int NP, int TPB, int PT) {
    return l < JA ? (NP >= 3 ? 1 + (l * (NP - 1)) / JA : 1) : read_phase(l, JA, TPB, PT) + 1;
}
constexpr int allowed(int p, int nf, int JA, int JB, int NP, int TPB, int PT) {
    const int NL = JA + JB;
    const int np = p + 2, Tn = np / NP, pn = np % NP;
    int last = -1;
    for (int T = 0; T <= Tn && T <= nf; ++T)
        for (int l = 0; l < NL; ++l)
            if (T < Tn || read_phase(l, JA, TPB, PT) <= pn) {
                const int key = (T * (NP + 1) + slot(l, JA, NP, TPB, PT)) * 64 + l;
                if (key > last) last = key;
            }
    int cnt = 0;
    for (int T = 0; T <= 2 && T <= nf; ++T)
        for (int l = 0; l < NL; ++l) {
            const int sl = slot(l, JA, NP, TPB, PT);
            const int time = (T - 2) * NP + sl;
            const int key = (T * (NP + 1) + sl) * 64 + l;
            if (time <= p && key > last) ++cnt;
        }
    return cnt;
}
template <int NF, int JA, int JB, int NP, int TPB, int PT>
__device__ __forceinline__ void wait_phase(int p) {
    switch (p) {
        case 0: wait_vmcnt<allowed(0, NF, JA, JB, NP, TPB, PT)>(); break;
        case 1: wait_vmcnt<allowed(1, NF, JA, JB, NP, TPB, PT)>(); break;
        case 2: wait_vmcnt<allowed(NP > 2 ? 2 : 0, NF, JA, JB, NP, TPB, PT)>(); break;
        case 3: wait_vmcnt<allowed(NP > 3 ? 3 : 0, NF, JA, JB, NP, TPB, PT)>(); break;
        default: wait_vmcnt<allowed(NP > 4 ? 4 : 0, NF, JA, JB, NP, TPB, PT)>(); break;
    }
}
}

template <int BM, int BN, int WAVES_N, int PT, bool CONV>
__global__ void __launch_bounds__(512) gemm_pp2_kernel(GemmArgs g) {
    constexpr int BK = 64, WAVES_M = 8 / WAVES_N;
    constexpr int WTN = BN / WAVES_N;
    constexpr int TM = 2, TN = WTN / 32;
    constexpr int NP = (TN + PT - 1) / PT;
    constexpr int JA = BM / 64, JB = BN / 64;
    constexpr int TPB = TN / JB;
    constexpr int NL = JA + JB;
    constexpr int A_BYTES = BM * BK * 2, B_BYTES = BN * BK * 2, STAGE_BYTES = A_BYTES + B_BYTES;
    static_assert(PT == 1 || PT == 2, "one or two N-tiles per phase");
    static_assert(BM / WAVES_M == 64 && WTN % 32 == 0 && TN % JB == 0, "bad tile");
    extern __shared__ __attribute__((aligned(16))) char smem[];

    const int tid = threadIdx.x;
    const int lane = tid & 63;
    const int wave = __builtin_amdgcn_readfirstlane(tid >> 6);
    const int wm = wave / WAVES_N, wn = wave % WAVES_N;
    const int grp = wave >> 2;
    const int hi = lane >> 5, l31 = lane & 31;
    int bx, by;
    {
        const int nbx = gridDim.x, nb = gridDim.x * gridDim.y;
        const int bid = blockIdx.y * nbx + blockIdx.x;
        const int q = nb >> 3, r = nb & 7;
        const int xcd = bid & 7, idx = bid >> 3;
        const int logical = (xcd < r ? xcd * (q + 1) : r * (q + 1) + (xcd - r) * q) + idx;
        by = logical / nbx;
        bx = logical - by * nbx;
    }
    const int m0 = by * BM;
    const int n0 = bx * BN;
    const int z = blockIdx.z;
    const bool split = g.splitk > 1;
    const int zb = split ? 0 : z;
    const int nk_total = g.K / BK;
    int kt_begin = 0, kt_end = nk_total;
    if (split) {
        kt_begin = z * g.ktiles_per_split;
        kt_end = kt_begin + g.ktiles_per_split;
        if (kt_end > nk_total) kt_end = nk_total;
    }
    const f16* Ab = g.A + (int64_t)zb * g.strideA;
    const f16* Wb = g.W + (int64_t)zb * g.strideW;

    const int rbase = wave * 8 + (lane >> 3);
    const int ls = (lane & 7) ^ ((rbase >> 1) & 7);
    int64_t a_off[JA];
    int a_iy0[JA], a_ix0[JA];
#pragma unroll
    for (int j = 0; j < JA; ++j) {
        const int m = m0 + rbase + 64 * j;
        const bool ok = m < g.M;
        if (CONV) {
            const int ohw = g.cg.OH * g.cg.OW;
            const int mm = ok ? m : 0;
            const int img = mm / ohw;
            const int rem = mm - img * ohw;
            const int oy = rem / g.cg.OW;
            const int ox = rem - oy * g.cg.OW;
            a_iy0[j] = ok ? oy * g.cg.stride - g.cg.pad_t : -(1 << 28);
            a_ix0[j] = ox * g.cg.stride - g.cg.pad_l;
            a_off[j] = ((int64_t)img * g.cg.H * g.cg.W + (int64_t)a_iy0[j] * g.cg.W + a_ix0[j]) * g.cg.Cin + ls * 8;
        } else {
            a_iy0[j] = ok ? 0 : -1;
            a_ix0[j] = 0;
            a_off[j] = (int64_t)m * g.lda + ls * 8;
        }
    }
    constexpr int RB = 64 / WAVES_N;
    const int b_row0 = (WAVES_N == 2) ? (wave >> 2) * WTN + (wave & 3) * 8 : wave * 8;
    const int nb0 = n0 + b_row0 + (lane >> 3);
    const int64_t b_off0 = (int64_t)nb0 * g.ldw + ls * 8;
    const int b_lds0 = b_row0 * 128;

    struct TileK {
        int ky, kx, c0;
        int64_t a_delta;
        int kw;
    };
    auto finish = [&](TileK& t) {
        if (CONV) {
            t.a_delta = ((int64_t)t.ky * g.cg.W + t.kx) * g.cg.Cin + t.c0;
            t.kw = (t.ky * g.cg.KW + t.kx) * g.cg.Cin + t.c0;
        } else {
            t.a_delta = t.c0;
            t.kw = t.c0;
        }
    };
    auto decode = [&](int kt) {
        TileK t;
        t.ky = t.kx = 0;
        t.c0 = kt * BK;
        if (CONV) {
            int tap;
            if (g.cg.chunk_major) {
                const int taps = g.cg.KH * g.cg.KW;
                const int chunk = kt / taps;
                tap = kt - chunk * taps;
                t.c0 = chunk * BK;
            } else {
                tap = (kt * BK) / g.cg.Cin;
                t.c0 = kt * BK - tap * g.cg.Cin;
            }
            t.ky = tap / g.cg.KW;
            t.kx = tap - t.ky * g.cg.KW;
        }
        finish(t);
        return t;
    };
    auto advance = [&](TileK& t) {
        if (CONV) {
            if (g.cg.chunk_major) {
                if (++t.kx == g.cg.KW) {
                    t.kx = 0;
                    if (++t.ky == g.cg.KH) { t.ky = 0; t.c0 += BK; }
                }
            } else {
                t.c0 += BK;
                if (t.c0 == g.cg.Cin) {
                    t.c0 = 0;
                    if (++t.kx == g.cg.KW) { t.kx = 0; ++t.ky; }
                }
            }
        } else {
            t.c0 += BK;
        }
        finish(t);
    };
    auto issue_A = [&](int j, int stage, const TileK& t) {
        bool ok;
        if (CONV) {
            const int iy = a_iy0[j] + t.ky, ix = a_ix0[j] + t.kx;
            ok = (unsigned)iy < (unsigned)g.cg.H && (unsigned)ix < (unsigned)g.cg.W;
        } else {
            ok = a_iy0[j] >= 0;
        }
        const f16* src = ok ? Ab + a_off[j] + t.a_delta : g.zeros;
        glds16(src, smem + stage * STAGE_BYTES + (j * 64 + wave * 8) * 128);
    };
    auto issue_B = [&](int j, int stage, const TileK& t) {
        const bool ok = (nb0 + j * RB) < g.N;
        const f16* src = ok ? Wb + b_off0 + (int64_t)(j * RB) * g.ldw + t.kw : g.zeros;
        glds16(src, smem + stage * STAGE_BYTES + A_BYTES + b_lds0 + j * RB * 128);
    };

    AccBlock acc[TM][TN];
#pragma unroll
    for (int i = 0; i < TM; ++i)
#pragma unroll
        for (int j = 0; j < TN; ++j) acc_zero(acc[i][j]);

    const int lrow = Frag::lrow(lane), lkq = Frag::lk(lane);
    int koff[Frag::NSTEP];
#pragma unroll
    for (int s = 0; s < Frag::NSTEP; ++s) koff[s] = (Frag::kslot(s, lkq) ^ ((lrow >> 1) & 7)) << 4;
    const int a_lane_off = (wm * 64 + lrow) * 128;
    const int b_lane_off = A_BYTES + (wn * WTN + lrow) * 128;

    auto issue_slot = [&](int sl, int stage, const TileK& t) {
#pragma unroll
        for (int l = 0; l < NL; ++l)
            if (pp2::slot(l, JA, NP, TPB, PT) == sl) {
                if (l < JA) issue_A(l, stage, t);
                else issue_B(l - JA, stage, t);
            }
    };
    constexpr int pro1 = []() { int c = 0; for (int l = 0; l < JA + JB; ++l) c += pp2::slot(l, JA, NP, TPB, PT) < NP ? 1 : 0; return c; }();
    TileK t1 = decode(kt_begin), t2;
    if (kt_begin < kt_end) {
        const TileK t0 = t1;
        advance(t1);
#pragma unroll
        for (int sl = 1; sl <= NP; ++sl) issue_slot(sl, 0, t0);
        if (kt_begin + 1 < kt_end) {
#pragma unroll
            for (int sl = 1; sl < NP; ++sl) issue_slot(sl, 1, t1);
            wait_vmcnt<pro1>();
        } else {
            wait_vmcnt<0>();
        }
    }
    t2 = t1;
    advance(t2);
    __builtin_amdgcn_s_barrier();
    f16x8 af[TM][Frag::NSTEP][Frag::PER], bf[PT][Frag::NSTEP][Frag::PER];
    {
        const char* fa = smem + a_lane_off;
        const char* fb = smem + b_lane_off;
#pragma unroll
        for (int s = 0; s < Frag::NSTEP; ++s)
#pragma unroll
            for (int u = 0; u < Frag::PER; ++u) {
#pragma unroll
                for (int i = 0; i < TM; ++i) af[i][s][u] = *reinterpret_cast<const f16x8*>(fa + koff[s] + i * 4096 + u * 2048);
#pragma unroll
                for (int jj = 0; jj < PT; ++jj) bf[jj][s][u] = *reinterpret_cast<const f16x8*>(fb + koff[s] + jj * 4096 + u * 2048);
            }
    }
    if (grp == 1) __builtin_amdgcn_s_barrier();

    for (int kt = kt_begin; kt < kt_end; ++kt) {
        const int cur = (kt - kt_begin) & 1;
        const bool has1 = (kt + 1) < kt_end, has2 = (kt + 2) < kt_end;
#pragma unroll
        for (int p = 0; p < NP; ++p) {
            const int j0 = PT * p;
            if (p == 0) {
                if (has1) issue_slot(NP, cur ^ 1, t1);
            } else {
                if (has2) issue_slot(p, cur, t2);
            }
            if (has2) pp2::wait_phase<2, JA, JB, NP, TPB, PT>(p);
            else if (has1) pp2::wait_phase<1, JA, JB, NP, TPB, PT>(p);
            else pp2::wait_phase<0, JA, JB, NP, TPB, PT>(p);
            asm volatile("s_waitcnt lgkmcnt(0)" ::: "memory");
            __builtin_amdgcn_sched_barrier(0);
            __builtin_amdgcn_s_barrier();
            __builtin_amdgcn_sched_barrier(0);
            const bool next_in_tile = (p + 1 < NP);
            const bool have_next = next_in_tile || has1;
            const char* nfa = smem + (cur ^ 1) * STAGE_BYTES + a_lane_off;
            const char* nfb = smem + (next_in_tile ? cur : (cur ^ 1)) * STAGE_BYTES + b_lane_off + (next_in_tile ? (j0 + PT) * 4096 : 0);
            __builtin_amdgcn_s_setprio(1);
#pragma unroll
            for (int s = 0; s < Frag::NSTEP; ++s) {
#pragma unroll
                for (int jj = 0; jj < PT; ++jj)
#pragma unroll
                    for (int i = 0; i < TM; ++i) mma_step(acc[i][j0 + jj], bf[jj][s], af[i][s]);
                if (have_next) {
#pragma unroll
                    for (int u = 0; u < Frag::PER; ++u) {
                        if (!next_in_tile) {
#pragma unroll
                            for (int i = 0; i < TM; ++i) af[i][s][u] = *reinterpret_cast<const f16x8*>(nfa + koff[s] + i * 4096 + u * 2048);
                        }
#pragma unroll
                        for (int jj = 0; jj < PT; ++jj) bf[jj][s][u] = *reinterpret_cast<const f16x8*>(nfb + koff[s] + jj * 4096 + u * 2048);
                    }
                }
            }
            __builtin_amdgcn_s_setprio(0);
            __builtin_amdgcn_sched_barrier(0);
            __builtin_amdgcn_s_barrier();
            __builtin_amdgcn_sched_barrier(0);
        }
        t1 = t2;
        advance(t2);
    }
    if (grp == 0) __builtin_amdgcn_s_barrier();
    asm volatile("s_waitcnt vmcnt(0) lgkmcnt(0)" ::: "memory");
    __syncthreads();
    if (ODISE_ABLATE(g, 4)) return;
    gemm_epilogue<BM, BN, WAVES_M, WAVES_N, epi_wave_rows(BM, BN, WAVES_M, pp_lds_bytes(BM, BN, WAVES_M)), false, CONV, true,
                  epi16_rows_if_enabled(BM, BN, WAVES_M, pp_lds_bytes(BM, BN, WAVES_M)), !CONV, pp_lds_bytes(BM, BN, WAVES_M)>(g, acc, smem, m0, n0, z, zb, split);
}


template <int BN, int PT>
__global__ void __launch_bounds__(512) conv3_halo_kernel(GemmArgs g) {
    constexpr int BM = 256, BK = 64, WAVES_N = 2, WAVES_M = 4;
    constexpr int WTN = BN / WAVES_N;
    constexpr int TM = 2, TN = WTN / 32;
    constexpr int NP = 2;
    constexpr int JB = BN / 64;
    constexpr int LB = JB / 2;
    constexpr int RB = 32;
    constexpr int HW_ = 18, HPIX = HW_ * HW_;
    constexpr int HGROUPS = (HPIX + 7) / 8;
    constexpr int H = 6;
    constexpr int B_BYTES = BN * BK * 2;
    constexpr int HALO_BYTES = (HGROUPS + 1) * 1024;
    constexpr int HALO0 = 2 * B_BYTES;
    static_assert(TN == PT * NP && JB == 2 * LB, "two phases of PT N-tiles, one B piece per N-tile");
    extern __shared__ __attribute__((aligned(16))) char smem[];

    const int tid = threadIdx.x;
    const int lane = tid & 63;
    const int wave = __builtin_amdgcn_readfirstlane(tid >> 6);
    const int wm = wave / WAVES_N, wn = wave % WAVES_N;
    const int grp = wave >> 2;
    const int hi = lane >> 5, l31 = lane & 31;
    int bx, by;
    {
        const int nbx = gridDim.x, nb = gridDim.x * gridDim.y;
        const int bid = blockIdx.y * nbx + blockIdx.x;
        const int q = nb >> 3, r = nb & 7;
        const int xcd = bid & 7, idx = bid >> 3;
        const int logical = (xcd < r ? xcd * (q + 1) : r * (q + 1) + (xcd - r) * q) + idx;
        by = logical / nbx;
        bx = logical - by * nbx;
    }
    const int m0 = by * BM;
    const int n0 = bx * BN;
    const int z = blockIdx.z;
    const bool split = g.splitk > 1;
    const int zb = 0;
    const int nk_total = g.K / BK;
    int kt_begin = 0, kt_end = nk_total;
    if (split) {
        kt_begin = z * g.ktiles_per_split;
        kt_end = kt_begin + g.ktiles_per_split;
        if (kt_end > nk_total) kt_end = nk_total;
    }
    const f16* Ab = g.A;
    const f16* Wb = g.W;
    const int per_img = g.cg.halo_tx * g.cg.halo_ty;
    const int img = by / per_img, pr = by - img * per_img;
    const int py0 = (pr / g.cg.halo_tx) * 16 - 1, px0 = (pr % g.cg.halo_tx) * 16 - 1;

    int64_t h_off[H];
#pragma unroll
    for (int h = 0; h < H; ++h) {
        const int group = h * 8 + wave;
        const int hp = group * 8 + (lane >> 3);
        h_off[h] = -1;
        if (group < HGROUPS && hp < HPIX) {
            const int hy = hp / HW_, hx = hp - hy * HW_;
            const int iy = py0 + hy, ix = px0 + hx;
            const int up = g.cg.ups ? 1 : 0;
            if ((unsigned)iy < (unsigned)(g.cg.H << up) && (unsigned)ix < (unsigned)(g.cg.W << up))
                h_off[h] = (((int64_t)img * g.cg.H + (iy >> up)) * g.cg.W + (ix >> up)) * g.cg.Cin + (((lane & 7) ^ ((hx >> 1) & 7)) << 3);
        }
    }
    auto issue_halo = [&](int chunk) {
        char* dst = smem + HALO0 + (chunk & 1) * HALO_BYTES;
#pragma unroll
        for (int h = 0; h < H; ++h) {
            const int group = h * 8 + wave;
            const f16* src = h_off[h] >= 0 ? Ab + h_off[h] + chunk * BK : g.zeros;
            glds16(src, dst + (group < HGROUPS ? group : HGROUPS) * 1024);
        }
    };
    const int rbase = wave * 8 + (lane >> 3);
    const int ls = (lane & 7) ^ ((rbase >> 1) & 7);
    const int b_row0 = (wave >> 2) * WTN + (wave & 3) * 8;
    const int nb0 = n0 + b_row0 + (lane >> 3);
    const int64_t b_off0 = (int64_t)nb0 * g.ldw + ls * 8;
    const int b_lds0 = b_row0 * 128;
    auto issue_B = [&](int j, int stage, int kw) {
        const bool ok = (nb0 + j * RB) < g.N;
        const f16* src = ok ? Wb + b_off0 + (int64_t)(j * RB) * g.ldw + kw : g.zeros;
        glds16(src, smem + stage * B_BYTES + b_lds0 + j * RB * 128);
    };
    struct TileK {
        int ky, kx, chunk, kw;
    };
    auto finish = [&](TileK& t) { t.kw = (t.ky * 3 + t.kx) * g.cg.Cin + t.chunk * BK; };
    auto advance = [&](TileK& t) {
        if (++t.kx == 3) {
            t.kx = 0;
            if (++t.ky == 3) { t.ky = 0; ++t.chunk; }
        }
        finish(t);
    };

    AccBlock acc[TM][TN];
#pragma unroll
    for (int i = 0; i < TM; ++i)
#pragma unroll
        for (int j = 0; j < TN; ++j) acc_zero(acc[i][j]);

    const int lrow = Frag::lrow(lane), lkq = Frag::lk(lane);
    int koff[Frag::NSTEP];
#pragma unroll
    for (int s = 0; s < Frag::NSTEP; ++s) koff[s] = (Frag::kslot(s, lkq) ^ ((lrow >> 1) & 7)) << 4;
    const int b_lane_off = (wn * WTN + lrow) * 128;
    const int a_pix0 = (wm * 4 + (lrow >> 4)) * HW_ + (lrow & 15);

    auto read_a = [&](const TileK& t, int s, f16x8 (&dst)[TM][Frag::NSTEP][Frag::PER]) {
        const char* ha = smem + HALO0 + (t.chunk & 1) * HALO_BYTES;
        const int pix = a_pix0 + t.ky * HW_ + t.kx;
        const int key = (((lrow & 15) + t.kx) >> 1) & 7;
#pragma unroll
        for (int i = 0; i < TM; ++i)
#pragma unroll
            for (int u = 0; u < Frag::PER; ++u)
                dst[i][s][u] = *reinterpret_cast<const f16x8*>(ha + (pix + (i * 2 + u) * HW_) * 128 + ((Frag::kslot(s, lkq) ^ key) << 4));
    };
    TileK t0;
    t0.ky = t0.kx = 0;
    t0.chunk = kt_begin / 9;
    finish(t0);
    TileK t1 = t0, t2;
    if (kt_begin < kt_end) {
        advance(t1);
        issue_halo(t0.chunk);
#pragma unroll
        for (int j = 0; j < JB; ++j) issue_B(j, 0, t0.kw);
        if (kt_begin + 1 < kt_end) {
#pragma unroll
            for (int j = 0; j < LB; ++j) issue_B(j, 1, t1.kw);
            wait_vmcnt<LB>();
        } else {
            wait_vmcnt<0>();
        }
    }
    t2 = t1;
    advance(t2);
    __builtin_amdgcn_s_barrier();
    TileK tc = t0;
    f16x8 af[TM][Frag::NSTEP][Frag::PER], bf[PT][Frag::NSTEP][Frag::PER];
    {
        const char* fb = smem + b_lane_off;
#pragma unroll
        for (int s = 0; s < Frag::NSTEP; ++s) {
            read_a(tc, s, af);
#pragma unroll
            for (int jj = 0; jj < PT; ++jj)
#pragma unroll
                for (int u = 0; u < Frag::PER; ++u) bf[jj][s][u] = *reinterpret_cast<const f16x8*>(fb + koff[s] + jj * 4096 + u * 2048);
        }
    }
    if (grp == 1) __builtin_amdgcn_s_barrier();

    for (int kt = kt_begin; kt < kt_end; ++kt) {
        const int cur = (kt - kt_begin) & 1;
        const bool has1 = (kt + 1) < kt_end, has2 = (kt + 2) < kt_end;
        const bool opens = tc.ky == 0 && tc.kx == 0;
        const bool halo_next = opens && (kt + 9) < kt_end;
#pragma unroll
        for (int p = 0; p < NP; ++p) {
            const int j0 = PT * p;
            if (p == 0) {
                if (has1) {
#pragma unroll
                    for (int j = LB; j < JB; ++j) issue_B(j, cur ^ 1, t1.kw);
                }
                if (halo_next) issue_halo(tc.chunk + 1);
                if (halo_next) { if (has1) wait_vmcnt<LB + H>(); else wait_vmcnt<H>(); }
                else { if (has1) wait_vmcnt<LB>(); else wait_vmcnt<0>(); }
            } else {
                if (has2) {
#pragma unroll
                    for (int j = 0; j < LB; ++j) issue_B(j, cur, t2.kw);
                }
                if (halo_next) { if (has2) wait_vmcnt<LB + H>(); else wait_vmcnt<H>(); }
                else { if (has2) wait_vmcnt<LB>(); else wait_vmcnt<0>(); }
            }
            asm volatile("s_waitcnt lgkmcnt(0)" ::: "memory");
            __builtin_amdgcn_sched_barrier(0);
            __builtin_amdgcn_s_barrier();
            __builtin_amdgcn_sched_barrier(0);
            const bool next_in_tile = (p + 1 < NP);
            const bool have_next = next_in_tile || has1;
            const char* nfb = smem + (next_in_tile ? cur : (cur ^ 1)) * B_BYTES + b_lane_off + (next_in_tile ? (j0 + PT) * 4096 : 0);
            __builtin_amdgcn_s_setprio(1);
#pragma unroll
            for (int s = 0; s < Frag::NSTEP; ++s) {
#pragma unroll
                for (int jj = 0; jj < PT; ++jj)
#pragma unroll
                    for (int i = 0; i < TM; ++i) mma_step(acc[i][j0 + jj], bf[jj][s], af[i][s]);
                if (have_next) {
                    if (!next_in_tile) read_a(t1, s, af);
#pragma unroll
                    for (int jj = 0; jj < PT; ++jj)
#pragma unroll
                        for (int u = 0; u < Frag::PER; ++u) bf[jj][s][u] = *reinterpret_cast<const f16x8*>(nfb + koff[s] + jj * 4096 + u * 2048);
                }
            }
            __builtin_amdgcn_s_setprio(0);
            __builtin_amdgcn_sched_barrier(0);
            __builtin_amdgcn_s_barrier();
            __builtin_amdgcn_sched_barrier(0);
        }
        tc = t1;
        t1 = t2;
        advance(t2);
    }
    if (grp == 0) __builtin_amdgcn_s_barrier();
    asm volatile("s_waitcnt vmcnt(0) lgkmcnt(0)" ::: "memory");
    __syncthreads();
    gemm_epilogue<BM, BN, WAVES_M, WAVES_N, epi_wave_rows(BM, BN, WAVES_M, halo_lds_bytes(BN)), true, true, true,
                  epi16_rows_if_enabled(BM, BN, WAVES_M, halo_lds_bytes(BN)), false, halo_lds_bytes(BN)>(g, acc, smem, m0, n0, z, zb, split);
}

template <int BN>
__global__ void __launch_bounds__(256, 2) conv3_halo4_kernel(GemmArgs g) {
    constexpr int BM = 256, BK = 64, WAVES_M = 4, WAVES_N = 1;
    constexpr int TM = 2, TN = BN / 32;
    constexpr int JB = BN / 32;
    constexpr int HW_ = 18, HPIX = HW_ * HW_;
    constexpr int HGROUPS = (HPIX + 7) / 8;
    constexpr int H = 11;
    constexpr int B_BYTES = BN * BK * 2;
    constexpr int HALO0 = 2 * B_BYTES;
    extern __shared__ __attribute__((aligned(16))) char smem[];

    const int tid = threadIdx.x;
    const int lane = tid & 63;
    const int wave = __builtin_amdgcn_readfirstlane(tid >> 6);
    const int wm = wave;
    const int hi = lane >> 5, l31 = lane & 31;
    int bx, by;
    {
        const int nbx = gridDim.x, nb = gridDim.x * gridDim.y;
        const int bid = blockIdx.y * nbx + blockIdx.x;
        const int q = nb >> 3, r = nb & 7;
        const int xcd = bid & 7, idx = bid >> 3;
        const int logical = (xcd < r ? xcd * (q + 1) : r * (q + 1) + (xcd - r) * q) + idx;
        by = logical / nbx;
        bx = logical - by * nbx;
    }
    const int m0 = by * BM;
    const int n0 = bx * BN;
    const int z = blockIdx.z;
    const bool split = g.splitk > 1;
    const int zb = 0;
    const int nk_total = g.K / BK;
    int kt_begin = 0, kt_end = nk_total;
    if (split) {
        kt_begin = z * g.ktiles_per_split;
        kt_end = kt_begin + g.ktiles_per_split;
        if (kt_end > nk_total) kt_end = nk_total;
    }
    const f16* Wb = g.W;
    const int per_img = g.cg.halo_tx * g.cg.halo_ty;
    const int img = by / per_img, pr = by - img * per_img;
    const int py0 = (pr / g.cg.halo_tx) * 16 - 1, px0 = (pr % g.cg.halo_tx) * 16 - 1;
    const f16* Ab = g.A + (int64_t)img * g.cg.H * g.cg.W * g.cg.Cin;

    int h_off[H];
#pragma unroll
    for (int h = 0; h < H; ++h) {
        const int group = h * 4 + wave;
        const int hp = group * 8 + (lane >> 3);
        h_off[h] = -1;
        if (group < HGROUPS && hp < HPIX) {
            const int hy = hp / HW_, hx = hp - hy * HW_;
            const int iy = py0 + hy, ix = px0 + hx;
            const int up = g.cg.ups ? 1 : 0;
            if ((unsigned)iy < (unsigned)(g.cg.H << up) && (unsigned)ix < (unsigned)(g.cg.W << up))
                h_off[h] = ((iy >> up) * g.cg.W + (ix >> up)) * g.cg.Cin + (((lane & 7) ^ ((hx >> 1) & 7)) << 3);
        }
    }
    auto issue_halo = [&](int chunk) {
#pragma unroll
        for (int h = 0; h < H; ++h) {
            const int group = h * 4 + wave;
            const f16* src = h_off[h] >= 0 ? Ab + h_off[h] + chunk * BK : g.zeros;
            glds16(src, smem + HALO0 + (group < HGROUPS ? group : HGROUPS) * 1024);
        }
    };
    const int rb = wave * 8 + (lane >> 3);
    const int ls = (lane & 7) ^ ((rb >> 1) & 7);
    const int64_t b_off0 = (int64_t)(n0 + rb) * g.ldw + ls * 8;
    auto issue_B = [&](int stage, int kw) {
#pragma unroll
        for (int j = 0; j < JB; ++j) {
            const bool ok = (n0 + rb + 32 * j) < g.N;
            const f16* src = ok ? Wb + b_off0 + (int64_t)(32 * j) * g.ldw + kw : g.zeros;
            glds16(src, smem + stage * B_BYTES + (32 * j + wave * 8) * 128);
        }
    };

    AccBlock acc[TM][TN];
#pragma unroll
    for (int i = 0; i < TM; ++i)
#pragma unroll
        for (int j = 0; j < TN; ++j) acc_zero(acc[i][j]);

    const int lrow = Frag::lrow(lane), lkq = Frag::lk(lane);
    int koff[Frag::NSTEP];
#pragma unroll
    for (int s = 0; s < Frag::NSTEP; ++s) koff[s] = (Frag::kslot(s, lkq) ^ ((lrow >> 1) & 7)) << 4;
    const int b_lane_off = lrow * 128;
    const int a_pix0 = (wm * 4 + (lrow >> 4)) * HW_ + (lrow & 15);

    int ky = 0, kx = 0, chunk = kt_begin / 9;
    if (kt_begin < kt_end) {
        issue_halo(chunk);
        issue_B(0, chunk * BK);
    }
    for (int kt = kt_begin; kt < kt_end; ++kt) {
        const int cur = (kt - kt_begin) & 1;
        asm volatile("s_waitcnt vmcnt(0)" ::: "memory");
        __builtin_amdgcn_s_barrier();
        int nky = ky, nkx = kx + 1, nchunk = chunk;
        if (nkx == 3) { nkx = 0; if (++nky == 3) { nky = 0; ++nchunk; } }
        const bool more = kt + 1 < kt_end;
        if (more) issue_B(cur ^ 1, (nky * 3 + nkx) * g.cg.Cin + nchunk * BK);
        const char* ha = smem + HALO0;
        const char* fb = smem + cur * B_BYTES + b_lane_off;
        const int pix = a_pix0 + ky * HW_ + kx;
        const int key = (((lrow & 15) + kx) >> 1) & 7;
        f16x8 af[2][TM][Frag::PER], bf[2][TN][Frag::PER];
        auto read_frags = [&](int s, int b) {
#pragma unroll
            for (int u = 0; u < Frag::PER; ++u) {
#pragma unroll
                for (int i = 0; i < TM; ++i) af[b][i][u] = *reinterpret_cast<const f16x8*>(ha + (pix + (i * 2 + u) * HW_) * 128 + ((Frag::kslot(s, lkq) ^ key) << 4));
#pragma unroll
                for (int j = 0; j < TN; ++j) bf[b][j][u] = *reinterpret_cast<const f16x8*>(fb + koff[s] + j * 4096 + u * 2048);
            }
        };
        read_frags(0, 0);
#pragma unroll
        for (int s = 0; s < Frag::NSTEP; ++s) {
            if (s + 1 < Frag::NSTEP) read_frags(s + 1, (s + 1) & 1);
            __builtin_amdgcn_sched_barrier(0);
#pragma unroll
            for (int j = 0; j < TN; ++j)
#pragma unroll
                for (int i = 0; i < TM; ++i) mma_step(acc[i][j], bf[s & 1][j], af[s & 1][i]);
            __builtin_amdgcn_sched_barrier(0);
        }
        if (more && nchunk != chunk) {
            asm volatile("s_waitcnt lgkmcnt(0)" ::: "memory");
            __builtin_amdgcn_s_barrier();
            issue_halo(nchunk);
        }
        ky = nky; kx = nkx; chunk = nchunk;
    }
    asm volatile("s_waitcnt vmcnt(0) lgkmcnt(0)" ::: "memory");
    __syncthreads();
    gemm_epilogue<BM, BN, WAVES_M, WAVES_N, epi_wave_rows(BM, BN, WAVES_M, halo4_lds_bytes(BN)), true, true, true,
                  epi16_rows_if_enabled(BM, BN, WAVES_M, halo4_lds_bytes(BN)), false, halo4_lds_bytes(BN)>(g, acc, smem, m0, n0, z, zb, split);
}

__global__ void __launch_bounds__(256) splitk_reduce_kernel(const float* __restrict__ ws, int splitk, int M, int N, GemmEpi e) {
    const int CH = (N + 7) / 8;
    const int64_t total = (int64_t)M * CH;
    const bool vec = (N & 3) == 0;
    for (int64_t idx = (int64_t)blockIdx.x * blockDim.x + threadIdx.x; idx < total; idx += (int64_t)gridDim.x * blockDim.x) {
        const int m = (int)(idx / CH);
        const int n = (int)(idx - (int64_t)m * CH) * 8;
        const int nv = (N - n) < 8 ? (N - n) : 8;
        float v[8];
#pragma unroll
        for (int i = 0; i < 8; ++i) v[i] = 0.f;
        if (vec && nv == 8) {
            for (int s = 0; s < splitk; ++s) {
                const float4* w = reinterpret_cast<const float4*>(ws + ((int64_t)s * M + m) * N + n);
                const float4 a = w[0], b = w[1];
                v[0] += a.x; v[1] += a.y; v[2] += a.z; v[3] += a.w;
                v[4] += b.x; v[5] += b.y; v[6] += b.z; v[7] += b.w;
            }
        } else {
            for (int s = 0; s < splitk; ++s) {
                const float* w = ws + ((int64_t)s * M + m) * N + n;
                for (int i = 0; i < nv; ++i) v[i] += w[i];
            }
        }
        if (e.fast && n + 8 <= N) epi_fast8(e, v, m, n, 0);
        else epi_store8(e, v, m, n, N, 0);
    }
}

template <int BM, int BN, int WAVES_M, int WAVES_N, bool CONV>
static int launch_gemm_t(odise_hip_ctx* ctx, GemmArgs& g, int batch) {
    constexpr int NT = 64 * WAVES_M * WAVES_N;
    constexpr int lds = plain_lds_bytes(BM, BN, WAVES_M);
    static_assert(epi_lds_bytes(BM, BN, WAVES_M, epi_wave_rows(BM, BN, WAVES_M, lds)) <= lds, "epilogue staging exceeds the LDS request");
    auto kern = gemm_kernel<BM, BN, WAVES_M, WAVES_N, CONV>;
    if (lds > 65536) {
        static LdsAttrOnce once;
        ODISE_TRY(ensure_dyn_lds(ctx, once, (const void*)kern, lds));
    }
    dim3 grid((unsigned)ceil_div(g.N, BN), (unsigned)ceil_div(g.M, BM), (unsigned)(g.splitk > 1 ? g.splitk : batch));
    hipLaunchKernelGGL(kern, grid, dim3(NT), lds, ctx->stream, g);
    ODISE_CHECK_HIP(hipGetLastError());
    if (g.splitk > 1) {
        const int64_t total = (int64_t)g.M * ceil_div(g.N, 8);
        const int blocks = (int)std::min<int64_t>(ceil_div(total, 256), 2048);
        hipLaunchKernelGGL(splitk_reduce_kernel, dim3(blocks), dim3(256), 0, ctx->stream, g.ws, g.splitk, g.M, g.N, g.epi);
        ODISE_CHECK_HIP(hipGetLastError());
    }
    return ODISE_OK;
}

template <int BM, int BN, int WAVES_N, int PT, bool CONV>
static int launch_gemm_pp(odise_hip_ctx* ctx, GemmArgs& g, int batch) {
    constexpr int lds = pp_lds_bytes(BM, BN, 8 / WAVES_N);
    static_assert(epi_lds_bytes(BM, BN, 8 / WAVES_N, epi_wave_rows(BM, BN, 8 / WAVES_N, lds)) <= lds, "epilogue staging exceeds the LDS request");
    auto kern = gemm_pp_kernel<BM, BN, WAVES_N, PT, CONV>;
    static LdsAttrOnce once;
    ODISE_TRY(ensure_dyn_lds(ctx, once, (const void*)kern, lds));
    dim3 grid((unsigned)ceil_div(g.N, BN), (unsigned)ceil_div(g.M, BM), (unsigned)(g.splitk > 1 ? g.splitk : batch));
    hipLaunchKernelGGL(kern, grid, dim3(512), lds, ctx->stream, g);
    ODISE_CHECK_HIP(hipGetLastError());
    if (g.splitk > 1) {
        const int64_t total = (int64_t)g.M * ceil_div(g.N, 8);
        const int blocks = (int)std::min<int64_t>(ceil_div(total, 256), 2048);
        hipLaunchKernelGGL(splitk_reduce_kernel, dim3(blocks), dim3(256), 0, ctx->stream, g.ws, g.splitk, g.M, g.N, g.epi);
        ODISE_CHECK_HIP(hipGetLastError());
    }
    return ODISE_OK;
}

template <int BM, int BN, int WAVES_N, int PT, bool CONV>
static int launch_gemm_pp2(odise_hip_ctx* ctx, GemmArgs& g, int batch) {
    static_assert((BN / WAVES_N / 32) % PT == 0, "whole phases");
    constexpr int lds = pp_lds_bytes(BM, BN, 8 / WAVES_N);
    auto kern = gemm_pp2_kernel<BM, BN, WAVES_N, PT, CONV>;
    static LdsAttrOnce once;
    ODISE_TRY(ensure_dyn_lds(ctx, once, (const void*)kern, lds));
    dim3 grid((unsigned)ceil_div(g.N, BN), (unsigned)ceil_div(g.M, BM), (unsigned)(g.splitk > 1 ? g.splitk : batch));
    hipLaunchKernelGGL(kern, grid, dim3(512), lds, ctx->stream, g);
    ODISE_CHECK_HIP(hipGetLastError());
    if (g.splitk > 1) {
        const int64_t total = (int64_t)g.M * ceil_div(g.N, 8);
        const int blocks = (int)std::min<int64_t>(ceil_div(total, 256), 2048);
        hipLaunchKernelGGL(splitk_reduce_kernel, dim3(blocks), dim3(256), 0, ctx->stream, g.ws, g.splitk, g.M, g.N, g.epi);
        ODISE_CHECK_HIP(hipGetLastError());
    }
    return ODISE_OK;
}

template <int BN, int PT>
static int launch_conv3_halo(odise_hip_ctx* ctx, GemmArgs& g) {
    constexpr int lds = halo_lds_bytes(BN);
    static_assert(epi_lds_bytes(256, BN, 4, epi_wave_rows(256, BN, 4, lds)) <= lds, "epilogue staging exceeds the LDS request");
    auto kern = conv3_halo_kernel<BN, PT>;
    static LdsAttrOnce once;
    ODISE_TRY(ensure_dyn_lds(ctx, once, (const void*)kern, lds));
    const int n_img = g.M / (g.cg.OH * g.cg.OW);
    dim3 grid((unsigned)ceil_div(g.N, BN), (unsigned)(n_img * g.cg.halo_tx * g.cg.halo_ty), (unsigned)(g.splitk > 1 ? g.splitk : 1));
    hipLaunchKernelGGL(kern, grid, dim3(512), lds, ctx->stream, g);
    ODISE_CHECK_HIP(hipGetLastError());
    if (g.splitk > 1) {
        const int64_t total = (int64_t)g.M * ceil_div(g.N, 8);
        const int blocks = (int)std::min<int64_t>(ceil_div(total, 256), 2048);
        hipLaunchKernelGGL(splitk_reduce_kernel, dim3(blocks), dim3(256), 0, ctx->stream, g.ws, g.splitk, g.M, g.N, g.epi);
        ODISE_CHECK_HIP(hipGetLastError());
    }
    return ODISE_OK;
}

template <int BN>
static int launch_conv3_halo4(odise_hip_ctx* ctx, GemmArgs& g) {
    constexpr int lds = halo4_lds_bytes(BN);
    static_assert(2 * lds <= 160 * 1024, "two blocks must fit a CU's LDS");
    static_assert(epi_lds_bytes(256, BN, 4, epi_wave_rows(256, BN, 4, lds)) <= lds, "epilogue staging exceeds the LDS request");
    auto kern = conv3_halo4_kernel<BN>;
    static LdsAttrOnce once;
    ODISE_TRY(ensure_dyn_lds(ctx, once, (const void*)kern, lds));
    const int n_img = g.M / (g.cg.OH * g.cg.OW);
    dim3 grid((unsigned)ceil_div(g.N, BN), (unsigned)(n_img * g.cg.halo_tx * g.cg.halo_ty), (unsigned)(g.splitk > 1 ? g.splitk : 1));
    hipLaunchKernelGGL(kern, grid, dim3(256), lds, ctx->stream, g);
    ODISE_CHECK_HIP(hipGetLastError());
    if (g.splitk > 1) {
        const int64_t total = (int64_t)g.M * ceil_div(g.N, 8);
        const int blocks = (int)std::min<int64_t>(ceil_div(total, 256), 2048);
        hipLaunchKernelGGL(splitk_reduce_kernel, dim3(blocks), dim3(256), 0, ctx->stream, g.ws, g.splitk, g.M, g.N, g.epi);
        ODISE_CHECK_HIP(hipGetLastError());
    }
    return ODISE_OK;
}

static int g_gemm_debug = 0;
static int g_conv_flags = 0;

static const int kNumTiles = 10;
static const int kTileBM[kNumTiles] = {128, 64, 64, 256, 256, 256, 512, 256, 256, 256};
static const int kTileBN[kNumTiles] = {128, 128, 64, 320, 256, 128, 128, 256, 128, 128};

struct TileCost {
    double t_ktile, t_fixed;
    int slots_per_cu;
};
static const TileCost kTileCost[kNumTiles] = {
    {1.45, 6.0, 2},
    {1.25, 3.5, 3},
    {1.06, 2.6, 4},
    {2.65, 15.0, 1},
    {2.10, 15.0, 1},
    {1.42, 6.0, 1},
    {2.25, 12.0, 1},
    {1.47, 22.5, 1},
    {1.12, 9.0, 1},
    {1.70, 12.0, 2},
};
static const TileCost kTileCostPP[2] = {
    {2.00, 16.0, 1},
    {1.56, 10.0, 1},
};
static const TileCost kTileCostConv512 = {2.5, 16.0, 1};
static const TileCost kTileCostPPConv256 = {1.49, 25.5, 1};
static thread_local int g_last_tile = -1;
static int env_gemm_flags() {
#ifdef ODISE_TOOLS
    static int v = -1;
    if (v < 0) {
        const char* e = getenv("ODISE_GEMM_FLAGS");
        v = e ? atoi(e) : 0;
    }
    return v;
#else
    return 0;
#endif
}

template <bool CONV>
static int launch_gemm_select(odise_hip_ctx* ctx, GemmArgs& g, int batch, int force_tile, int force_split, unsigned tile_mask);

template <bool CONV>
static int launch_gemm(odise_hip_ctx* ctx, GemmArgs& g, int batch, int force_tile, int force_split, unsigned tile_mask = ~0u) {
    LaunchProbe* pr = probe_match(ctx, CONV, g.M, g.N, g.K);
    if (pr && CONV && g.cg.ups) pr = nullptr;
    if (pr) {
        hipStreamCaptureStatus st = hipStreamCaptureStatusNone;
        if (hipStreamIsCapturing(ctx->stream, &st) != hipSuccess || st != hipStreamCaptureStatusNone) pr = nullptr;
    }
    if (!pr) return launch_gemm_select<CONV>(ctx, g, batch, force_tile, force_split, tile_mask);
    const int i = pr->n;
    const bool started = hipEventRecord(pr->ev[2 * i], ctx->stream) == hipSuccess;
    const int rc = launch_gemm_select<CONV>(ctx, g, batch, force_tile, force_split, tile_mask);
    if (started && hipEventRecord(pr->ev[2 * i + 1], ctx->stream) == hipSuccess) pr->n = i + 1;
    else { (void)hipGetLastError(); pr->armed = false; }
    return rc;
}

static int flags_early() { return g_conv_flags | env_gemm_flags(); }
template <bool CONV>
static int launch_gemm_select(odise_hip_ctx* ctx, GemmArgs& g, int batch, int force_tile, int force_split, unsigned tile_mask) {
    const int64_t cus = ctx->cu_count;
    const int nk = (int)ceil_div(g.K, 64);
    bool halo_ok = false;
    int64_t halo_patches = 0;
    if (CONV) {
        const int up = g.cg.ups ? 1 : 0;
        halo_ok = g.cg.KH == 3 && g.cg.KW == 3 && g.cg.stride == 1 && g.cg.pad_t == 1 && g.cg.pad_l == 1 && g.cg.Cin % 64 == 0 &&
                  g.cg.OH == (g.cg.H << up) && g.cg.OW == (g.cg.W << up) && batch == 1 && !(up && (flags_early() & 131072));
        g.cg.halo_tx = (int)ceil_div(g.cg.OW, 16);
        g.cg.halo_ty = (int)ceil_div(g.cg.OH, 16);
        halo_patches = (int64_t)(g.M / (g.cg.OH * g.cg.OW)) * g.cg.halo_tx * g.cg.halo_ty;
    }
    auto blocks = [&](int t) {
        return ((t >= 7 && t <= 9) ? halo_patches : ceil_div(g.M, kTileBM[t])) * ceil_div(g.N, kTileBN[t]) * (int64_t)batch;
    };
    int tile = 2, best_split = 1;
    double best = 1e30;
    const int flags = g_conv_flags | env_gemm_flags();
    const bool pp_base = !(flags & 2) && g.K % 64 == 0 && (!CONV || g.cg.Cin % 64 == 0);
    const bool pp_ok = pp_base && !(CONV && g.cg.ups);
    for (int t = 0; t < kNumTiles; ++t) {
        if (force_tile >= 0 && force_tile < kNumTiles && t != force_tile) continue;
        if (!((tile_mask >> t) & 1)) continue;
        if (t == 6 && (!pp_ok || (flags & 16))) continue;
        if (t >= 7 && t <= 9 && (!halo_ok || !pp_base || (flags & 64))) continue;
        if (t == 9 && (flags & 2048)) continue;
        if (t == 9 && force_tile < 0 && g.N > 128) continue;
        const TileCost& tc = (CONV && pp_ok && t == 4) ? kTileCostPPConv256 : (pp_ok && (t == 3 || t == 4)) ? kTileCostPP[t - 3] :
                             (CONV && t == 6) ? kTileCostConv512 : kTileCost[t];
        if (force_tile < 0) {
            if (kTileBM[t] > 64 && g.M <= kTileBM[t] / 2) continue;
            if (kTileBN[t] > 64 && g.N <= kTileBN[t] / 2 && t != 2) continue;
        }
        const int64_t nb = blocks(t);
        const int64_t slots = cus * tc.slots_per_cu;
        const int max_split = (batch == 1) ? std::max(1, std::min(nk / 2, 32)) : 1;
        for (int sp = 1; sp <= max_split; ++sp) {
            if (force_split > 0 && sp != std::min(force_split, std::max(1, nk))) continue;
            if (sp > 1 && (size_t)sp * g.M * g.N * sizeof(float) > ctx->ws_bytes) break;
            const int per = (t >= 7 && t <= 9) ? (int)ceil_div(nk / 9, sp) * 9 : (int)ceil_div(nk, sp);
            const int eff_sp = (int)ceil_div(nk, per);
            const int64_t nblk = nb * eff_sp;
            const int64_t rounds = ceil_div(nblk, slots);
            const double fill_last = (double)(nblk - (rounds - 1) * slots) / (double)slots;
            double t_us = per * tc.t_ktile * ((double)(rounds - 1) + 0.55 + 0.45 * fill_last) + (double)rounds * tc.t_fixed;
            if (eff_sp > 1) t_us += 4.0 + ((2.0 * eff_sp * 4.0 + 2.0) * (double)g.M * g.N) / 6.0e6;
            if (t_us < best) { best = t_us; tile = t; best_split = eff_sp; }
        }
    }
    if (force_tile >= 0 && force_tile < kNumTiles && !(force_tile == 6 && !pp_ok) && !(force_tile >= 7 && force_tile <= 9 && !(halo_ok && pp_base)))
        tile = force_tile;
    g.splitk = 1;
    g.ktiles_per_split = nk;
    if (force_split > 0 && batch == 1) best_split = std::min(force_split, nk);
    if (best_split > 1 && batch == 1) {
        g.ktiles_per_split = (tile >= 7 && tile <= 9) ? (int)ceil_div(nk / 9, best_split) * 9 : (int)ceil_div(nk, best_split);
        g.splitk = (int)ceil_div(nk, g.ktiles_per_split);
        ODISE_REQUIRE((size_t)g.splitk * g.M * g.N * sizeof(float) <= ctx->ws_bytes, "gemm: split-K workspace too small");
    }
    g_last_tile = tile | (best_split << 8);
    if (ctx->launch_log) launch_log_push(ctx, LaunchRec{(int)CONV, g.M, g.N, g.K, tile, g.splitk});
    if (flags & 32) {
        fprintf(stderr, "GEMMLOG conv=%d M=%d N=%d K=%d batch=%d cin=%d kh=%d h=%d w=%d stride=%d ups=%d tile=%d split=%d pp=%d\n", (int)CONV, g.M, g.N,
                g.K, batch, g.cg.Cin, g.cg.KH, g.cg.H, g.cg.W, g.cg.stride, g.cg.ups, tile, best_split, (int)pp_ok);
    }
    g.ws = (float*)ctx->ws;
    {
        const GemmEpi& e = g.epi;
        const int esz = e.c_dtype == ODISE_F16 ? 2 : 4;
        const int out_vec = (e.geglu ? 4 : 8) * esz;
        auto aligned = [](const void* p, int64_t ld_elems, int64_t stride_elems, int elem, int bytes) {
            return ((uintptr_t)p % bytes) == 0 && (ld_elems * elem) % bytes == 0 && (stride_elems * elem) % bytes == 0;
        };
        bool ok = aligned(e.C, e.ldc, e.strideC, esz, out_vec);
        ok = ok && (!e.residual || (!e.geglu && aligned(e.residual, e.ldr, e.strideR, 2, 16)));
        ok = ok && (!e.bias_n || ((uintptr_t)e.bias_n & 15) == 0);
        ok = ok && (!e.rowgroup_add || (((uintptr_t)e.rowgroup_add & 15) == 0 && e.ldg % 4 == 0));
        ok = ok && (!e.geglu || e.act == ODISE_ACT_NONE);
        g.epi.fast = ok ? 1 : 0;
        const int n_out = e.geglu ? g.N / 2 : g.N;
        g.epi.f16path = (ok && e.c_dtype == ODISE_F16 && g.N % 8 == 0 && n_out % 8 == 0 && aligned(e.C, e.ldc, e.strideC, 2, 16) &&
                         (!e.residual || aligned(e.residual, e.ldr, e.strideR, 2, 8))) ? 1 : 0;
    }
    if (g.epi.ln_part || g.epi.ln_final || g.epi.ln_stats_out) {
        ODISE_REQUIRE(!CONV && (tile == 4 || tile == 5) && g.splitk == 1 && g.epi.f16path && !g.epi.geglu && batch == 1 &&
                          (!g.epi.ln_stats_out || (tile == 4 && g.N % kLnPartCols == 0)),
                      "gemm_ln: M=%d N=%d K=%d cannot take the folded-LayerNorm path", g.M, g.N, g.K);
    }
    g.stats_blocks = 0;
    if (g.epi.gn_stats) {
        const int ohw = CONV ? g.cg.OH * g.cg.OW : 0;
        const bool pp2_used = (tile == 4) && pp_ok && ((flags & 512) || (!(flags & 1024) && CONV));
        bool ok = CONV && g.splitk == 1 && g.epi.fast && g.N % 8 == 0 && ((tile >= 7 && tile <= 9) || (tile == 6 && pp_ok && !(flags & 512)) || pp2_used);
        if (ok && tile >= 7) g.stats_blocks = g.cg.halo_tx * g.cg.halo_ty;
        else if (ok && ohw % kTileBM[tile] == 0) g.stats_blocks = ohw / kTileBM[tile];
        else ok = false;
        if (!ok) { g.epi.gn_stats = nullptr; g.stats_blocks = 0; }
    }
    g.zeros = (const f16*)ctx->zeros;
    g.epi_block = (flags & 32768) ? 1 : 0;
#ifdef ODISE_TOOLS
    static const int freeze_k = (getenv("ODISE_GEMM_FREEZE_K") ? 16 : 0) | (getenv("ODISE_NO_RES_PREFETCH") ? 64 : 0);
    g.dbg = g_gemm_debug | freeze_k;
#else
    g.dbg = 0;
#endif
    if (tile >= 7) {
        g.cg.chunk_major = 1;
        if (tile == 9) return launch_conv3_halo4<128>(ctx, g);
        return tile == 7 ? launch_conv3_halo<256, 2>(ctx, g) : launch_conv3_halo<128, 1>(ctx, g);
    }
    g.cg.halo_tx = g.cg.halo_ty = 0;
    const bool pp2_auto = !(flags & 1024) && ((CONV && tile != 6) || (!CONV && blocks(tile) * (g.splitk > 1 ? g.splitk : 1) <= 2 * cus));
    if ((tile == 3 || tile == 4 || tile == 6) && pp_ok && ((flags & 512) || pp2_auto)) {
        if (tile == 6) return launch_gemm_pp2<512, 128, 1, 2, CONV>(ctx, g, batch);
        if (tile == 3) return launch_gemm_pp2<256, 320, 2, 1, CONV>(ctx, g, batch);
        return launch_gemm_pp2<256, 256, 2, 2, CONV>(ctx, g, batch);
    }
    if ((tile == 3 || tile == 4 || tile == 6) && pp_ok) {
        if (tile == 6) return launch_gemm_pp<512, 128, 1, 2, CONV>(ctx, g, batch);
        if (tile == 3) return launch_gemm_pp<256, 320, 2, 1, CONV>(ctx, g, batch);
        return launch_gemm_pp<256, 256, 2, 2, CONV>(ctx, g, batch);
    }
    switch (tile) {
        case 0: return launch_gemm_t<128, 128, 2, 2, CONV>(ctx, g, batch);
        case 1: return launch_gemm_t<64, 128, 2, 2, CONV>(ctx, g, batch);
        case 3: return launch_gemm_t<256, 320, 4, 2, CONV>(ctx, g, batch);
        case 4: return launch_gemm_t<256, 256, 4, 2, CONV>(ctx, g, batch);
        case 5: return launch_gemm_t<256, 128, 4, 2, CONV>(ctx, g, batch);
        default: return launch_gemm_t<64, 64, 2, 2, CONV>(ctx, g, batch);
    }
}

int conv_forced(odise_hip_ctx* ctx, const odise_conv_desc* d, int force_tile, int force_split, float* gn_stats = nullptr, int* stats_blocks = nullptr);

int gemm_forced(odise_hip_ctx* ctx, const odise_gemm_desc* d, int force_tile, int force_split, const LnEpi* ln) {
    ODISE_REQUIRE(ctx && d, "gemm: null argument");
    ODISE_REQUIRE(d->M >= 0 && d->N >= 0 && d->K > 0, "gemm: bad dims M=%d N=%d K=%d", d->M, d->N, d->K);
    if (d->M == 0 || d->N == 0) return ODISE_OK;
    ODISE_REQUIRE(d->K % 8 == 0, "gemm: K=%d must be a multiple of 8", d->K);
    ODISE_REQUIRE(d->lda % 8 == 0 && d->ldw % 8 == 0, "gemm: lda/ldw must be multiples of 8 (16-byte rows)");
    ODISE_REQUIRE(((uintptr_t)d->A & 15) == 0 && ((uintptr_t)d->W & 15) == 0, "gemm: A/W must be 16-byte aligned");
    ODISE_REQUIRE(d->A && d->W && d->C, "gemm: null device pointer");
    ODISE_REQUIRE(d->c_dtype == ODISE_F16 || d->c_dtype == ODISE_F32, "gemm: bad c_dtype");
    ODISE_REQUIRE(!d->geglu || (d->N % 2 == 0), "gemm: geglu needs even N");
    ODISE_REQUIRE(!d->rowgroup_add || d->rows_per_group > 0, "gemm: rows_per_group must be > 0");
    const int batch = d->batch < 1 ? 1 : d->batch;
    ODISE_REQUIRE(batch == 1 || ((d->strideA % 8 == 0) && (d->strideW % 8 == 0)), "gemm: batch strides must keep 16-byte alignment");
    GemmArgs g;
    g.M = d->M; g.N = d->N; g.K = d->K;
    g.A = (const f16*)d->A; g.lda = d->lda; g.strideA = d->strideA;
    g.W = (const f16*)d->W; g.ldw = d->ldw; g.strideW = d->strideW;
    g.epi.C = d->C; g.epi.ldc = d->ldc; g.epi.c_dtype = d->c_dtype;
    g.epi.bias_n = d->bias_n; g.epi.bias_m = d->bias_m; g.epi.scale_m = d->scale_m;
    g.epi.residual = (const f16*)d->residual; g.epi.ldr = d->ldr;
    g.epi.rowgroup_add = d->rowgroup_add; g.epi.rows_per_group = d->rows_per_group > 0 ? d->rows_per_group : 1;
    g.epi.ldg = d->ldg > 0 ? d->ldg : d->N;
    g.epi.act = d->act; g.epi.geglu = d->geglu; g.epi.alpha = d->alpha;
    g.epi.strideC = d->strideC; g.epi.strideR = d->strideR;
    g.epi.gn_stats = nullptr;
    g.epi.ln_part = nullptr; g.epi.ln_P = 0; g.epi.ln_inv_c = 0.f; g.epi.ln_eps = 0.f; g.epi.ln_colsum = nullptr; g.epi.ln_final_out = nullptr;
    g.epi.ln_final = nullptr; g.epi.ln_rowsum = nullptr; g.epi.ln_stats_out = nullptr;
    if (ln) {
        g.epi.ln_part = ln->part; g.epi.ln_P = ln->P; g.epi.ln_inv_c = ln->inv_c; g.epi.ln_eps = ln->eps; g.epi.ln_colsum = ln->colsum;
        g.epi.ln_final_out = ln->final_out; g.epi.ln_final = ln->fin; g.epi.ln_rowsum = ln->rowsum; g.epi.ln_stats_out = ln->stats_out;
        ODISE_REQUIRE((!ln->part || (ln->P > 0 && ln->colsum)) && (!ln->fin || ln->rowsum), "gemm_ln: incomplete LayerNorm terms");
    }
    g.cg = ConvGeom{};
    if (ln) return launch_gemm<false>(ctx, g, batch, force_tile, 1, ln->stats_out ? (1u << 4) : (1u << 4) | (1u << 5));
    return launch_gemm<false>(ctx, g, batch, force_tile, force_split);
}

int gemm_ln(odise_hip_ctx* ctx, const odise_gemm_desc* d, const LnEpi& ln) { return gemm_forced(ctx, d, -1, 1, &ln); }

int conv_forced(odise_hip_ctx* ctx, const odise_conv_desc* d, int force_tile, int force_split, float* gn_stats, int* stats_blocks) {
    ODISE_REQUIRE(ctx && d, "conv2d: null argument");
    ODISE_REQUIRE(d->N >= 0 && d->H > 0 && d->W > 0 && d->Cin > 0 && d->Cout > 0, "conv2d: bad dims");
    ODISE_REQUIRE(d->Cin % 8 == 0, "conv2d: Cin=%d must be a multiple of 8 (pad the input channels)", d->Cin);
    ODISE_REQUIRE(d->KH >= 1 && d->KW >= 1 && d->stride >= 1 && d->OH > 0 && d->OW > 0, "conv2d: bad kernel geometry");
    ODISE_REQUIRE(d->X && d->Wt && d->Y, "conv2d: null device pointer");
    ODISE_REQUIRE(((uintptr_t)d->X & 15) == 0 && ((uintptr_t)d->Wt & 15) == 0, "conv2d: X/Wt must be 16-byte aligned");
    if (d->N == 0) return ODISE_OK;
    if (force_tile < 0 && force_split <= 0 && conv3_c8_ok(d)) return launch_conv3_c8(ctx, d, gn_stats, stats_blocks);
    GemmArgs g;
    g.M = d->N * d->OH * d->OW;
    g.N = d->Cout;
    g.K = d->KH * d->KW * d->Cin;
    g.A = (const f16*)d->X; g.lda = 0; g.strideA = 0;
    g.W = (const f16*)d->Wt; g.ldw = g.K; g.strideW = 0;
    g.epi.C = d->Y; g.epi.ldc = d->Cout; g.epi.c_dtype = d->y_dtype;
    g.epi.bias_n = d->bias; g.epi.bias_m = nullptr; g.epi.scale_m = nullptr;
    g.epi.residual = (const f16*)d->residual; g.epi.ldr = d->Cout;
    g.epi.rowgroup_add = d->per_image_add; g.epi.rows_per_group = d->OH * d->OW;
    g.epi.ldg = d->per_image_add_ld > 0 ? d->per_image_add_ld : d->Cout;
    g.epi.act = d->act; g.epi.geglu = 0; g.epi.alpha = 1.0f;
    g.epi.strideC = 0; g.epi.strideR = 0;
    g.epi.gn_stats = gn_stats;
    g.epi.ln_part = nullptr; g.epi.ln_P = 0; g.epi.ln_inv_c = 0.f; g.epi.ln_eps = 0.f; g.epi.ln_colsum = nullptr; g.epi.ln_final_out = nullptr;
    g.epi.ln_final = nullptr; g.epi.ln_rowsum = nullptr; g.epi.ln_stats_out = nullptr;
    if (stats_blocks) *stats_blocks = 0;
    g.cg.H = d->H; g.cg.W = d->W; g.cg.Cin = d->Cin; g.cg.KH = d->KH; g.cg.KW = d->KW;
    g.cg.stride = d->stride; g.cg.pad_t = d->pad_t; g.cg.pad_l = d->pad_l; g.cg.OH = d->OH; g.cg.OW = d->OW;
    g.cg.ups = d->upsample2x;
    const int64_t in_bytes = (int64_t)d->N * d->H * d->W * d->Cin * 2;
    g.cg.chunk_major = (d->Cin % 64 == 0 && d->KH * d->KW > 1 && in_bytes <= (128ll << 20)) ? 1 : 0;
    if (d->KH == 1 && d->KW == 1 && d->stride == 1 && d->pad_t == 0 && d->pad_l == 0 && !d->upsample2x && d->OH == d->H &&
        d->OW == d->W) {
        g.lda = d->Cin;
        return launch_gemm<false>(ctx, g, 1, force_tile, force_split);
    }
    const int rc = launch_gemm<true>(ctx, g, 1, force_tile, force_split);
    if (stats_blocks) *stats_blocks = (rc == ODISE_OK) ? g.stats_blocks : 0;
    return rc;
}

int group_norm_from_colpart(odise_hip_ctx* ctx, const void* x, void* y, const float* gamma, const float* beta, int N, int HW, int C, int groups,
                            float eps, int act, const float* colpart, int nblk);

}

extern "C" int odise_hip_gemm_debug(int flags) {
    odise::g_gemm_debug = flags & 15;
    odise::g_conv_flags = (flags >> 4) & 0xfffff;
    return 0;
}
extern "C" int odise_hip_gemm(odise_hip_ctx* ctx, const odise_gemm_desc* d) { return odise::gemm_forced(ctx, d, -1, 0); }
extern "C" int odise_hip_conv2d(odise_hip_ctx* ctx, const odise_conv_desc* d) { return odise::conv_forced(ctx, d, -1, 0); }
extern "C" int odise_hip_gemm_forced(odise_hip_ctx* ctx, const odise_gemm_desc* d, int tile, int splitk) {
    return odise::gemm_forced(ctx, d, tile, splitk);
}
extern "C" int odise_hip_last_tile(void) { return odise::g_last_tile; }
extern "C" int odise_hip_gemm_ln(odise_hip_ctx* ctx, const odise_gemm_desc* d, const float* part, int parts, float inv_c, float eps,
                                 const float* colsum, float* final_out, const float* fin, const float* rowsum, float* stats_out) {
    odise::LnEpi ln;
    ln.part = part; ln.P = parts; ln.inv_c = inv_c; ln.eps = eps; ln.colsum = colsum; ln.final_out = final_out;
    ln.fin = fin; ln.rowsum = rowsum; ln.stats_out = stats_out;
    return odise::gemm_ln(ctx, d, ln);
}
extern "C" int odise_hip_conv2d_forced(odise_hip_ctx* ctx, const odise_conv_desc* d, int tile, int splitk) {
    return odise::conv_forced(ctx, d, tile, splitk);
}
extern "C" int odise_hip_conv2d_gn_forced(odise_hip_ctx* ctx, const odise_conv_desc* d, int tile, int splitk, const float* gamma, const float* beta,
                                          int groups, float eps, int act, void* y_norm, float* stats_scratch, int* stats_blocks) {
    ODISE_REQUIRE(ctx && d && gamma && beta && y_norm && stats_scratch && stats_blocks, "conv2d_gn_forced: null argument");
    ODISE_REQUIRE(d->y_dtype == ODISE_F16, "conv2d_gn_forced: f16 output only");
    if (int rc = odise::conv_forced(ctx, d, tile, splitk, stats_scratch, stats_blocks)) return rc;
    if (*stats_blocks > 0)
        return odise::group_norm_from_colpart(ctx, d->Y, y_norm, gamma, beta, d->N, d->OH * d->OW, d->Cout, groups, eps, act, stats_scratch, *stats_blocks);
    return odise_hip_group_norm(ctx, d->Y, y_norm, gamma, beta, d->N, d->OH * d->OW, d->Cout, groups, eps, act);
}
```

### odise_amd/csrc/norm.hip

```cpp
#include "common.h"
#include <stdlib.h>

namespace odise {

constexpr int GN_MAX_C = 4096;
static int g_gn_chunk_factor = 2;
static int g_ln_rows8 = 32768;
static int g_gn_fold_in_apply = 1;

__global__ void __launch_bounds__(256) gn_partial_kernel(const f16* __restrict__ x, float* __restrict__ partial, int HW, int C,
                                                        int G, int pix_per_chunk) {
    extern __shared__ __attribute__((aligned(16))) float sred[];
    const int n = blockIdx.y, chunk = blockIdx.x, nchunks = gridDim.x;
    const int tid = threadIdx.x;
    const int V = C >> 3;
    const int VW = V < 256 ? V : 256;
    const int PL = 256 / VW;
    float* ssum = sred;
    float* ssq = sred + PL * C;
    const int p_begin = chunk * pix_per_chunk;
    const int p_end = min(HW, p_begin + pix_per_chunk);
    const int pl = tid / VW;
    if (pl < PL) {
        for (int v = tid - pl * VW; v < V; v += VW) {
            float s[8], q[8];
#pragma unroll
            for (int i = 0; i < 8; ++i) s[i] = q[i] = 0.f;
            const f16* xb = x + ((int64_t)n * HW) * C + v * 8;
            int p = p_begin + pl;
            for (; p + 3 * PL < p_end; p += 4 * PL) {
                f16x8 t[4];
#pragma unroll
                for (int u = 0; u < 4; ++u) t[u] = *reinterpret_cast<const f16x8*>(xb + (int64_t)(p + u * PL) * C);
#pragma unroll
                for (int u = 0; u < 4; ++u)
#pragma unroll
                    for (int i = 0; i < 8; ++i) {
                        const float a = (float)t[u][i];
                        s[i] += a;
                        q[i] += a * a;
                    }
            }
            for (; p < p_end; p += PL) {
                const f16x8 t = *reinterpret_cast<const f16x8*>(xb + (int64_t)p * C);
#pragma unroll
                for (int i = 0; i < 8; ++i) {
                    const float a = (float)t[i];
                    s[i] += a;
                    q[i] += a * a;
                }
            }
#pragma unroll
            for (int i = 0; i < 8; ++i) {
                ssum[pl * C + v * 8 + i] = s[i];
                ssq[pl * C + v * 8 + i] = q[i];
            }
        }
    }
    __syncthreads();
    const int cpg = C / G;
    if (tid < G) {
        float s = 0.f, q = 0.f;
        for (int t = 0; t < PL; ++t)
            for (int c = tid * cpg; c < (tid + 1) * cpg; ++c) {
                s += ssum[t * C + c];
                q += ssq[t * C + c];
            }
        float* o = partial + (((int64_t)n * nchunks + chunk) * G + tid) * 2;
        o[0] = s;
        o[1] = q;
    }
}

__global__ void __launch_bounds__(256) gn_finalize_kernel(const float* __restrict__ partial, float* __restrict__ stats, int HW, int C, int G,
                                                         int nchunks, float eps) {
    __shared__ double red[2 * 256];
    const int n = blockIdx.x, tid = threadIdx.x;
    const int cpg = C / G;
    const int nsub = 256 / G;
    const int gI = tid % G, sub = tid / G;
    double s = 0.0, q = 0.0;
    if (sub < nsub) {
        for (int ch = sub; ch < nchunks; ch += nsub) {
            const float* o = partial + (((int64_t)n * nchunks + ch) * G + gI) * 2;
            s += (double)o[0];
            q += (double)o[1];
        }
    }
    red[2 * tid] = s;
    red[2 * tid + 1] = q;
    __syncthreads();
    if (tid < G) {
        s = q = 0.0;
        for (int u = 0; u < nsub; ++u) {
            s += red[2 * (u * G + tid)];
            q += red[2 * (u * G + tid) + 1];
        }
        const double cnt = (double)HW * cpg;
        const double mu = s / cnt;
        double var = q / cnt - mu * mu;
        if (var < 0.0) var = 0.0;
        stats[((int64_t)n * G + tid) * 2] = (float)mu;
        stats[((int64_t)n * G + tid) * 2 + 1] = (float)(1.0 / sqrt(var + (double)eps));
    }
}

__global__ void __launch_bounds__(256) gn_finalize_cols_kernel(const float* __restrict__ colpart, float* __restrict__ stats, int HW, int C, int G,
                                                              int nblk, float eps) {
    __shared__ double red[2 * 256];
    const int gI = blockIdx.x, n = blockIdx.y, tid = threadIdx.x;
    const int cpg = C / G;
    double s = 0.0, q = 0.0;
    for (int b = tid; b < nblk; b += 256) {
        const float* o = colpart + (((int64_t)n * nblk + b) * C + (int64_t)gI * cpg) * 2;
        if ((cpg & 1) == 0) {
            for (int c = 0; c < cpg; c += 2) {
                const float4 v = *reinterpret_cast<const float4*>(o + 2 * c);
                s += (double)v.x + (double)v.z;
                q += (double)v.y + (double)v.w;
            }
        } else {
            for (int c = 0; c < cpg; ++c) {
                s += (double)o[2 * c];
                q += (double)o[2 * c + 1];
            }
        }
    }
    red[2 * tid] = s;
    red[2 * tid + 1] = q;
    __syncthreads();
    for (int w = 128; w > 0; w >>= 1) {
        if (tid < w) {
            red[2 * tid] += red[2 * (tid + w)];
            red[2 * tid + 1] += red[2 * (tid + w) + 1];
        }
        __syncthreads();
    }
    if (tid == 0) {
        const double cnt = (double)HW * cpg;
        const double mu = red[0] / cnt;
        double var = red[1] / cnt - mu * mu;
        if (var < 0.0) var = 0.0;
        stats[((int64_t)n * G + gI) * 2] = (float)mu;
        stats[((int64_t)n * G + gI) * 2 + 1] = (float)(1.0 / sqrt(var + (double)eps));
    }
}

__global__ void __launch_bounds__(256) gn_apply_kernel(const f16* __restrict__ x, f16* __restrict__ y,
                                                      const float* __restrict__ stats, const float* __restrict__ gamma,
                                                      const float* __restrict__ beta, int HW, int C, int G,
                                                      int act, const f16* __restrict__ residual,
                                                      const f16* __restrict__ accum, int nchunks, float eps) {
    extern __shared__ __attribute__((aligned(16))) float sss[];
    float* scale = sss;
    float* shift = sss + C;
    const int n = blockIdx.y, tid = threadIdx.x;
    const int cpg = C / G;
    __shared__ double red[2 * 256];
    __shared__ float gstat[2 * 256];
    if (nchunks > 0) {
        const int nsub = 256 / G;
        const int gI = tid % G, sub = tid / G;
        double s = 0.0, q = 0.0;
        if (sub < nsub) {
            for (int ch = sub; ch < nchunks; ch += nsub) {
                const float2 o = *reinterpret_cast<const float2*>(stats + (((int64_t)n * nchunks + ch) * G + gI) * 2);
                s += (double)o.x;
                q += (double)o.y;
            }
        }
        red[2 * tid] = s;
        red[2 * tid + 1] = q;
        __syncthreads();
        if (tid < G) {
            s = q = 0.0;
            for (int u = 0; u < nsub; ++u) {
                s += red[2 * (u * G + tid)];
                q += red[2 * (u * G + tid) + 1];
            }
            const double cnt = (double)HW * cpg;
            const double mu = s / cnt;
            double var = q / cnt - mu * mu;
            if (var < 0.0) var = 0.0;
            gstat[2 * tid] = (float)mu;
            gstat[2 * tid + 1] = (float)(1.0 / sqrt(var + (double)eps));
        }
        __syncthreads();
    }
    for (int c = tid; c < C; c += blockDim.x) {
        const int gI = c / cpg;
        const float mu = nchunks > 0 ? gstat[2 * gI] : stats[((int64_t)n * G + gI) * 2];
        const float rs = nchunks > 0 ? gstat[2 * gI + 1] : stats[((int64_t)n * G + gI) * 2 + 1];
        const float sc = rs * (gamma ? gamma[c] : 1.f);
        scale[c] = sc;
        shift[c] = (beta ? beta[c] : 0.f) - mu * sc;
    }
    __syncthreads();
    const int C8 = C >> 3;
    const int total = HW * C8;
    const f16* xb = x + (int64_t)n * HW * C;
    f16* yb = y + (int64_t)n * HW * C;
    const f16* rb = residual ? residual + (int64_t)n * HW * C : nullptr;
    const f16* ab = accum ? accum + (int64_t)n * HW * C : nullptr;
    const int stride = gridDim.x * blockDim.x;
    for (int base = blockIdx.x * blockDim.x + tid; base < total; base += 4 * stride) {
        f16x8 v[4], r[4], a[4];
#pragma unroll
        for (int u = 0; u < 4; ++u) {
            const int idx = base + u * stride;
            const f16x8 z = {0, 0, 0, 0, 0, 0, 0, 0};
            v[u] = r[u] = a[u] = z;
            if (idx < total) {
                v[u] = *reinterpret_cast<const f16x8*>(xb + (int64_t)idx * 8);
                if (rb) r[u] = *reinterpret_cast<const f16x8*>(rb + (int64_t)idx * 8);
                if (ab) a[u] = *reinterpret_cast<const f16x8*>(ab + (int64_t)idx * 8);
            }
        }
#pragma unroll
        for (int u = 0; u < 4; ++u) {
            const int idx = base + u * stride;
            if (idx >= total) break;
            const int c0 = (idx % C8) * 8;
            const float4 s0 = *reinterpret_cast<const float4*>(scale + c0), s1 = *reinterpret_cast<const float4*>(scale + c0 + 4);
            const float4 h0 = *reinterpret_cast<const float4*>(shift + c0), h1 = *reinterpret_cast<const float4*>(shift + c0 + 4);
            const float sc[8] = {s0.x, s0.y, s0.z, s0.w, s1.x, s1.y, s1.z, s1.w};
            const float sh[8] = {h0.x, h0.y, h0.z, h0.w, h1.x, h1.y, h1.z, h1.w};
            float t[8];
#pragma unroll
            for (int i = 0; i < 8; ++i) t[i] = (float)v[u][i] * sc[i] + sh[i] + (float)r[u][i];
            if (act == ODISE_ACT_SILU) {
#pragma unroll
                for (int i = 0; i < 8; ++i) t[i] = mul_sigmoid(t[i], t[i]);
            } else if (act != ODISE_ACT_NONE) {
#pragma unroll
                for (int i = 0; i < 8; ++i) t[i] = act_apply(t[i], act);
            }
            f16x8 o;
#pragma unroll
            for (int i = 0; i < 8; ++i) o[i] = (f16)(t[i] + (float)a[u][i]);
            __builtin_nontemporal_store(o, reinterpret_cast<f16x8*>(yb + (int64_t)idx * 8));
        }
    }
}

template <int NV, int R>
__global__ void __launch_bounds__(256) layer_norm_kernel(const f16* __restrict__ x, f16* __restrict__ y,
                                                        const float* __restrict__ gamma, const float* __restrict__ beta,
                                                        int rows, int C, float eps) {
    const int lane = threadIdx.x & 63;
    const int row0 = (blockIdx.x * 4 + (threadIdx.x >> 6)) * R;
    if (row0 >= rows) return;
    f16x8 v[R][NV];
    float s[R];
#pragma unroll
    for (int r = 0; r < R; ++r) {
        s[r] = 0.f;
        const bool rok = row0 + r < rows;
#pragma unroll
        for (int k = 0; k < NV; ++k) {
            const int c = (lane + 64 * k) * 8;
            if (rok && c < C) v[r][k] = *reinterpret_cast<const f16x8*>(x + (int64_t)(row0 + r) * C + c);
        }
    }
#pragma unroll
    for (int r = 0; r < R; ++r) {
#pragma unroll
        for (int k = 0; k < NV; ++k) {
            const int c = (lane + 64 * k) * 8;
            if (c < C) {
#pragma unroll
                for (int i = 0; i < 8; ++i) s[r] += (float)v[r][k][i];
            }
        }
    }
#pragma unroll
    for (int o = 32; o > 0; o >>= 1) {
#pragma unroll
        for (int r = 0; r < R; ++r) s[r] += __shfl_xor(s[r], o);
    }
    float q[R], mu[R];
#pragma unroll
    for (int r = 0; r < R; ++r) {
        mu[r] = s[r] / (float)C;
        q[r] = 0.f;
#pragma unroll
        for (int k = 0; k < NV; ++k) {
            const int c = (lane + 64 * k) * 8;
            if (c < C) {
#pragma unroll
                for (int i = 0; i < 8; ++i) {
                    const float d = (float)v[r][k][i] - mu[r];
                    q[r] += d * d;
                }
            }
        }
    }
#pragma unroll
    for (int o = 32; o > 0; o >>= 1) {
#pragma unroll
        for (int r = 0; r < R; ++r) q[r] += __shfl_xor(q[r], o);
    }
#pragma unroll
    for (int k = 0; k < NV; ++k) {
        const int c = (lane + 64 * k) * 8;
        if (c < C) {
            float gm[8], bt[8];
#pragma unroll
            for (int i = 0; i < 8; ++i) {
                gm[i] = gamma ? gamma[c + i] : 1.f;
                bt[i] = beta ? beta[c + i] : 0.f;
            }
#pragma unroll
            for (int r = 0; r < R; ++r) {
                if (row0 + r < rows) {
                    const float rs = rsqrtf(q[r] / (float)C + eps);
                    f16x8 o;
#pragma unroll
                    for (int i = 0; i < 8; ++i) o[i] = (f16)(((float)v[r][k][i] - mu[r]) * rs * gm[i] + bt[i]);
                    *reinterpret_cast<f16x8*>(y + (int64_t)(row0 + r) * C + c) = o;
                }
            }
        }
    }
}

template <int R>
__global__ void __launch_bounds__(256) layer_norm_half_kernel(const f16* __restrict__ x, f16* __restrict__ y, const float* __restrict__ gamma,
                                                             const float* __restrict__ beta, int rows, int C, float eps, f16* __restrict__ y2,
                                                             const float* __restrict__ table, int P) {
    const int lane = threadIdx.x & 63, l31 = lane & 31, half = lane >> 5;
    const int row0 = ((blockIdx.x * 4 + (threadIdx.x >> 6)) * 2 + half) * R;
    const int c = l31 * 8;
    const bool cok = c < C;
    f16x8 v[R];
    float s[R], q[R], mu[R];
#pragma unroll
    for (int r = 0; r < R; ++r) {
        const f16x8 z = {0, 0, 0, 0, 0, 0, 0, 0};
        v[r] = z;
        if (cok && row0 + r < rows) v[r] = *reinterpret_cast<const f16x8*>(x + (int64_t)(row0 + r) * C + c);
    }
#pragma unroll
    for (int r = 0; r < R; ++r) {
        s[r] = 0.f;
        if (cok) {
#pragma unroll
            for (int i = 0; i < 8; ++i) s[r] += (float)v[r][i];
        }
    }
#pragma unroll
    for (int o = 16; o > 0; o >>= 1) {
#pragma unroll
        for (int r = 0; r < R; ++r) s[r] += __shfl_xor(s[r], o);
    }
#pragma unroll
    for (int r = 0; r < R; ++r) {
        mu[r] = s[r] / (float)C;
        q[r] = 0.f;
        if (cok) {
#pragma unroll
            for (int i = 0; i < 8; ++i) {
                const float d = (float)v[r][i] - mu[r];
                q[r] += d * d;
            }
        }
    }
#pragma unroll
    for (int o = 16; o > 0; o >>= 1) {
#pragma unroll
        for (int r = 0; r < R; ++r) q[r] += __shfl_xor(q[r], o);
    }
    if (!cok) return;
    float gm[8], bt[8];
#pragma unroll
    for (int i = 0; i < 8; ++i) {
        gm[i] = gamma ? gamma[c + i] : 1.f;
        bt[i] = beta ? beta[c + i] : 0.f;
    }
#pragma unroll
    for (int r = 0; r < R; ++r) {
        if (row0 + r < rows) {
            const float rs = rsqrtf(q[r] / (float)C + eps);
            f16x8 o;
#pragma unroll
            for (int i = 0; i < 8; ++i) o[i] = (f16)(((float)v[r][i] - mu[r]) * rs * gm[i] + bt[i]);
            *reinterpret_cast<f16x8*>(y + (int64_t)(row0 + r) * C + c) = o;
            if (y2) {
                const float* tr = table + (int64_t)((row0 + r) % P) * C + c;
                f16x8 o2;
#pragma unroll
                for (int i = 0; i < 8; ++i) o2[i] = (f16)((float)o[i] + tr[i]);
                *reinterpret_cast<f16x8*>(y2 + (int64_t)(row0 + r) * C + c) = o2;
            }
        }
    }
}

}

extern "C" int odise_hip_group_norm_ex(odise_hip_ctx* ctx, const void* x, void* y, const float* gamma, const float* beta, int N,
                                       int HW, int C, int groups, float eps, int act, const void* residual, const void* accum);

extern "C" int odise_hip_group_norm(odise_hip_ctx* ctx, const void* x, void* y, const float* gamma, const float* beta, int N,
                                    int HW, int C, int groups, float eps, int act) {
    return odise_hip_group_norm_ex(ctx, x, y, gamma, beta, N, HW, C, groups, eps, act, nullptr, nullptr);
}

extern "C" int odise_hip_group_norm_ex(odise_hip_ctx* ctx, const void* x, void* y, const float* gamma, const float* beta, int N,
                                       int HW, int C, int groups, float eps, int act, const void* residual, const void* accum) {
    using namespace odise;
    ODISE_REQUIRE(ctx && x && y, "group_norm: null argument");
    ODISE_REQUIRE(N >= 0 && HW > 0 && C > 0 && groups > 0, "group_norm: bad dims");
    ODISE_REQUIRE(C % groups == 0 && C % 8 == 0 && C <= GN_MAX_C, "group_norm: C=%d must be a multiple of 8 and of groups=%d, <= %d", C, groups, GN_MAX_C);
    ODISE_REQUIRE(groups <= 256, "group_norm: groups=%d > 256", groups);
    if (N == 0) return ODISE_OK;
    const int V = C / 8;
    const int VW = V < 256 ? V : 256;
    const int PL = 256 / VW;
    ODISE_REQUIRE((int64_t)HW * (C / 8) < (1ll << 31) - (1 << 24), "group_norm: image too large");
    int64_t want = std::max<int64_t>(1, (int64_t)ctx->cu_count * g_gn_chunk_factor / N);
    int64_t maxc = std::max<int64_t>(1, HW / (4 * PL));
    int nchunks = (int)std::min<int64_t>(std::min<int64_t>(want, maxc), 256);
    const int ppc = (int)ceil_div(HW, nchunks);
    nchunks = (int)ceil_div(HW, ppc);
    const size_t pbytes = ((size_t)N * nchunks * groups * 2 + (size_t)N * groups * 2) * sizeof(float);
    ODISE_REQUIRE(pbytes <= ctx->ws_bytes, "group_norm: workspace too small");
    float* partial = (float*)ctx->ws;
    float* stats = partial + (size_t)N * nchunks * groups * 2;
    hipLaunchKernelGGL(gn_partial_kernel, dim3(nchunks, N), dim3(256), 2 * (size_t)PL * C * sizeof(float), ctx->stream, (const f16*)x,
                       partial, HW, C, groups, ppc);
    ODISE_CHECK_HIP(hipGetLastError());
    const bool fold_in_apply = g_gn_fold_in_apply && nchunks <= 64;
    if (!fold_in_apply) {
        hipLaunchKernelGGL(gn_finalize_kernel, dim3(N), dim3(256), 0, ctx->stream, partial, stats, HW, C, groups, nchunks, eps);
        ODISE_CHECK_HIP(hipGetLastError());
    }
    const int64_t total = (int64_t)HW * (C / 8);
    const int bpi = (int)std::max<int64_t>(1, ceil_div(total, 256 * 4));
    hipLaunchKernelGGL(gn_apply_kernel, dim3(bpi, N), dim3(256), 2 * (size_t)C * sizeof(float), ctx->stream, (const f16*)x, (f16*)y,
                       fold_in_apply ? partial : stats, gamma, beta, HW, C, groups, act, (const f16*)residual, (const f16*)accum, fold_in_apply ? nchunks : 0, eps);
    ODISE_CHECK_HIP(hipGetLastError());
    return ODISE_OK;
}

namespace odise {
int group_norm_from_colpart(odise_hip_ctx* ctx, const void* x, void* y, const float* gamma, const float* beta, int N, int HW, int C, int groups,
                            float eps, int act, const float* colpart, int nblk) {
    ODISE_REQUIRE(ctx && x && y && colpart && nblk > 0, "group_norm: null argument");
    ODISE_REQUIRE(C % groups == 0 && C % 8 == 0 && C <= GN_MAX_C && groups <= 256, "group_norm: bad channel / group count");
    ODISE_REQUIRE((int64_t)HW * (C / 8) < (1ll << 31) - (1 << 24), "group_norm: image too large");
    ODISE_REQUIRE((size_t)N * groups * 2 * sizeof(float) <= ctx->ws_bytes, "group_norm: workspace too small");
    float* stats = (float*)ctx->ws;
    hipLaunchKernelGGL(gn_finalize_cols_kernel, dim3(groups, N), dim3(256), 0, ctx->stream, colpart, stats, HW, C, groups, nblk, eps);
    ODISE_CHECK_HIP(hipGetLastError());
    const int64_t total = (int64_t)HW * (C / 8);
    const int bpi = (int)std::max<int64_t>(1, ceil_div(total, 256 * 4));
    hipLaunchKernelGGL(gn_apply_kernel, dim3(bpi, N), dim3(256), 2 * (size_t)C * sizeof(float), ctx->stream, (const f16*)x, (f16*)y, stats, gamma,
                       beta, HW, C, groups, act, (const f16*)nullptr, (const f16*)nullptr, 0, eps);
    ODISE_CHECK_HIP(hipGetLastError());
    return ODISE_OK;
}
}

namespace odise {
int layer_norm_add_table(odise_hip_ctx* ctx, const void* x, void* y, const float* gamma, const float* beta, int rows, int C, float eps, f16* y2,
                         const float* table, int P) {
    ODISE_REQUIRE(ctx && x && y, "layer_norm: null argument");
    ODISE_REQUIRE(!y2 || (C <= 256 && table && P >= 1), "layer_norm: the second output needs C <= 256 and a table");
    ODISE_REQUIRE(rows >= 0 && C > 0 && C % 8 == 0 && C <= 4096, "layer_norm: C=%d must be a positive multiple of 8, <= 4096", C);
    if (rows == 0) return ODISE_OK;
    auto launch = [&](auto kern, int R) {
        const dim3 grid((unsigned)ceil_div(rows, 4 * R));
        hipLaunchKernelGGL(kern, grid, dim3(256), 0, ctx->stream, (const f16*)x, (f16*)y, gamma, beta, rows, C, eps);
    };
    int many_rows = 2048;
#ifdef ODISE_TOOLS
    if (const char* e = getenv("ODISE_LN_MANY_ROWS")) many_rows = atoi(e);
#endif
    const bool many = rows >= many_rows;
    if (C <= 256) {
        if (many) hipLaunchKernelGGL(layer_norm_half_kernel<4>, dim3((unsigned)ceil_div(rows, 4 * 2 * 4)), dim3(256), 0, ctx->stream, (const f16*)x, (f16*)y, gamma, beta, rows, C, eps, y2, table, P);
        else hipLaunchKernelGGL(layer_norm_half_kernel<1>, dim3((unsigned)ceil_div(rows, 4 * 2)), dim3(256), 0, ctx->stream, (const f16*)x, (f16*)y, gamma, beta, rows, C, eps, y2, table, P);
    } else if (C <= 512) { if (rows >= g_ln_rows8) launch(layer_norm_kernel<1, 8>, 8); else if (many) launch(layer_norm_kernel<1, 4>, 4); else launch(layer_norm_kernel<1, 1>, 1); }
    else if (C <= 1024) { if (many) launch(layer_norm_kernel<2, 4>, 4); else launch(layer_norm_kernel<2, 1>, 1); }
    else if (C <= 2048) { if (many) launch(layer_norm_kernel<4, 2>, 2); else launch(layer_norm_kernel<4, 1>, 1); }
    else launch(layer_norm_kernel<8, 1>, 1);
    ODISE_CHECK_HIP(hipGetLastError());
    return ODISE_OK;
}
}

extern "C" int odise_hip_layer_norm(odise_hip_ctx* ctx, const void* x, void* y, const float* gamma, const float* beta,
                                    int rows, int C, float eps) {
    return odise::layer_norm_add_table(ctx, x, y, gamma, beta, rows, C, eps, nullptr, nullptr, 1);
}

extern "C" int odise_hip_gn_tuning(int chunk_factor, int fold_in_apply) {
    if (chunk_factor >= 1) odise::g_gn_chunk_factor = chunk_factor;
    if (chunk_factor < 0) odise::g_ln_rows8 = -chunk_factor;
    odise::g_gn_fold_in_apply = fold_in_apply != 0;
    return 0;
}
```

Before: 52.01.

## Fuse GroupNorm+SiLU into 3x3 halo conv operand load for VAE resnet blocks

```diff
diff --git a/include/odise_hip_tools.h b/include/odise_hip_tools.h
--- a/include/odise_hip_tools.h
+++ b/include/odise_hip_tools.h
@@ -20,6 +20,8 @@
                       float* final_out, const float* fin, const float* rowsum, float* stats_out);
 int odise_hip_conv2d_gn_forced(odise_hip_ctx* ctx, const odise_conv_desc* d, int tile, int splitk, const float* gamma, const float* beta,
                                int groups, float eps, int act, void* y_norm, float* stats_scratch, int* stats_blocks);
+int odise_hip_conv2d_prenorm(odise_hip_ctx* ctx, const odise_conv_desc* d, const float* gamma, const float* beta, int groups, float eps, int act,
+                             const float* colpart, int nblk, float* table, void* x_norm);
 int odise_hip_gemm_debug(int flags);
 
 int odise_hip_post_generic(int on);
diff --git a/odise_amd/csrc/common.h b/odise_amd/csrc/common.h
--- a/odise_amd/csrc/common.h
+++ b/odise_amd/csrc/common.h
@@ -64,6 +64,28 @@
         case ODISE_ACT_QUICKGELU: return mul_sigmoid(v, 1.702f * v);
         default: return v;
     }
+}
+
+__device__ __forceinline__ void gn_scale_shift(float mu, float rs, float gamma, float beta, float& sc, float& sh) {
+    sc = rs * gamma;
+    sh = beta - mu * sc;
+}
+
+__device__ __forceinline__ f16x8 gn_act8(const f16x8& v, const float (&sc)[8], const float (&sh)[8], const f16x8& r, const f16x8& a, int act) {
+    float t[8];
+#pragma unroll
+    for (int i = 0; i < 8; ++i) t[i] = (float)v[i] * sc[i] + sh[i] + (float)r[i];
+    if (act == ODISE_ACT_SILU) {
+#pragma unroll
+        for (int i = 0; i < 8; ++i) t[i] = mul_sigmoid(t[i], t[i]);
+    } else if (act != ODISE_ACT_NONE) {
+#pragma unroll
+        for (int i = 0; i < 8; ++i) t[i] = act_apply(t[i], act);
+    }
+    f16x8 o;
+#pragma unroll
+    for (int i = 0; i < 8; ++i) o[i] = (f16)(t[i] + (float)a[i]);
+    return o;
 }
 
 }
diff --git a/odise_amd/csrc/engine.cpp b/odise_amd/csrc/engine.cpp
--- a/odise_amd/csrc/engine.cpp
+++ b/odise_amd/csrc/engine.cpp
@@ -249,6 +249,36 @@
     return odise_hip_conv2d(ctx, &d);
 }
 
+int Exec::conv_gn(const Act& x, const NormW& nw, float eps, int act, const ConvW& w, Act& y, const Act* residual) {
+    if (x.c != w.cin_pad || w.k != 3) {
+        set_error("conv_gn: input has %d channels, weight expects %d (3x3 only, k = %d)", x.c, w.cin_pad, w.k);
+        return ODISE_ERR_ARG;
+    }
+    if (!y.p) ODISE_TRY(alloc(y, x.n, x.h, x.w, w.cout));
+    odise_conv_desc d;
+    memset(&d, 0, sizeof(d));
+    d.N = x.n; d.H = x.h; d.W = x.w; d.Cin = x.c;
+    d.Cout = w.cout; d.KH = 3; d.KW = 3; d.stride = 1; d.pad_t = 1; d.pad_l = 1; d.OH = x.h; d.OW = x.w;
+    d.X = x.p; d.Wt = w.w; d.Y = y.p; d.y_dtype = ODISE_F16;
+    d.bias = w.b;
+    d.residual = residual ? residual->p : nullptr;
+    d.act = ODISE_ACT_NONE;
+    const int rc = conv_prenorm(ctx, &d, nullptr, act, nullptr, nullptr);
+    if (rc != ODISE_OK) {
+        if (rc < 0) return rc;
+        Act t;
+        ODISE_TRY(group_norm(x, nw, t, eps, act));
+        return conv(t, w, y, 1, 1, false, residual);
+    }
+    float* table = (float*)alloc_bytes((size_t)x.n * x.c * 2 * sizeof(float));
+    if (!table) return ODISE_ERR_NOMEM;
+    const bool colpart = x.gn_part && x.gn_blocks > 0;
+    ODISE_TRY(group_norm_table(ctx, x.p, nw.g, nw.b, x.n, x.h * x.w, x.c, 32, eps, colpart ? x.gn_part : nullptr, colpart ? x.gn_blocks : 0, table));
+    ms->macs += (double)x.n * x.h * x.w * w.cout * 9 * w.cin;
+    y.gn_blocks = 0;
+    return conv_prenorm(ctx, &d, table, act, y.gn_part, &y.gn_blocks);
+}
+
 int Exec::alloc_gn_stats(Act& a) {
     const int64_t blocks = ceil_div((int64_t)a.h * a.w, 64);
     a.gn_part = (float*)alloc_bytes((size_t)a.n * blocks * a.c * 2 * sizeof(float));
diff --git a/odise_amd/csrc/engine.h b/odise_amd/csrc/engine.h
--- a/odise_amd/csrc/engine.h
+++ b/odise_amd/csrc/engine.h
@@ -148,6 +148,7 @@
     int linear(const f16* x, int64_t M, const LinW& w, f16* y, int act = ODISE_ACT_NONE, const f16* residual = nullptr,
                bool geglu = false);
     int group_norm(const Act& x, const NormW& w, Act& y, float eps, int act);
+    int conv_gn(const Act& x, const NormW& nw, float eps, int act, const ConvW& w, Act& y, const Act* residual = nullptr);
     int layer_norm(const f16* x, f16* y, int64_t rows, const NormW& w, float eps);
     int gemm(const odise_gemm_desc& d);
     int attention(const odise_attn_desc& d);
@@ -297,5 +298,8 @@
 int conv_forced(odise_hip_ctx* ctx, const odise_conv_desc* d, int force_tile, int force_split, float* gn_stats, int* stats_blocks);
 int group_norm_from_colpart(odise_hip_ctx* ctx, const void* x, void* y, const float* gamma, const float* beta, int N, int HW, int C, int groups,
                             float eps, int act, const float* colpart, int nblk);
+int conv_prenorm(odise_hip_ctx* ctx, const odise_conv_desc* d, const float* table, int act, float* gn_stats, int* stats_blocks);
+int group_norm_table(odise_hip_ctx* ctx, const void* x, const float* gamma, const float* beta, int N, int HW, int C, int groups, float eps,
+                     const float* colpart, int nblk, float* table);
 
 }
diff --git a/odise_amd/csrc/extractor.cpp b/odise_amd/csrc/extractor.cpp
--- a/odise_amd/csrc/extractor.cpp
+++ b/odise_amd/csrc/extractor.cpp
@@ -314,18 +314,16 @@
     ODISE_REQUIRE(out.n == x.n && out.h == x.h && out.w == x.w && out.c == w.c1.cout, "vae block: output tensor does not match");
     ODISE_TRY(ex.alloc_gn_stats(out));
     const size_t mk = ex.ms->arena.mark();
-    Act t1, h, t2, sk;
-    ODISE_TRY(ex.group_norm(x, w.n1, t1, 1e-6f, ODISE_ACT_SILU));
+    Act h, sk;
     ODISE_TRY(ex.alloc(h, x.n, x.h, x.w, w.c1.cout));
     ODISE_TRY(ex.alloc_gn_stats(h));
-    ODISE_TRY(ex.conv(t1, w.c1, h, 1, 1));
-    ODISE_TRY(ex.group_norm(h, w.n2, t2, 1e-6f, ODISE_ACT_SILU));
+    ODISE_TRY(ex.conv_gn(x, w.n1, 1e-6f, ODISE_ACT_SILU, w.c1, h));
     const Act* resid = &x;
     if (w.has_nin) {
         ODISE_TRY(ex.conv(x, w.nin, sk, 1, 0));
         resid = &sk;
     }
-    ODISE_TRY(ex.conv(t2, w.c2, out, 1, 1, false, resid));
+    ODISE_TRY(ex.conv_gn(h, w.n2, 1e-6f, ODISE_ACT_SILU, w.c2, out, resid));
     ex.ms->arena.release(mk);
     return ODISE_OK;
 }
diff --git a/odise_amd/csrc/gemm.hip b/odise_amd/csrc/gemm.hip
--- a/odise_amd/csrc/gemm.hip
+++ b/odise_amd/csrc/gemm.hip
@@ -59,7 +59,11 @@
     int dbg;
     int stats_blocks;
     int epi_block;
+    const float* pre_tab;
+    int pre_act;
 };
+
+constexpr int kPreTabMaxBytes = 4096;
 
 __device__ __forceinline__ void lds_barrier() {
     asm volatile("s_waitcnt lgkmcnt(0)" ::: "memory");
@@ -1899,7 +1903,7 @@
 }
 
 
-template <int BN, int PT>
+template <int BN, int PT, bool PRE>
 __global__ void __launch_bounds__(512) conv3_halo_kernel(GemmArgs g) {
     constexpr int BM = 256, BK = 64, WAVES_N = 2, WAVES_M = 4;
     constexpr int WTN = BN / WAVES_N;
@@ -1950,6 +1954,12 @@
     const int per_img = g.cg.halo_tx * g.cg.halo_ty;
     const int img = by / per_img, pr = by - img * per_img;
     const int py0 = (pr / g.cg.halo_tx) * 16 - 1, px0 = (pr % g.cg.halo_tx) * 16 - 1;
+    constexpr int TAB0 = halo_lds_bytes(BN);
+    constexpr bool pre = PRE;
+    if (pre) {
+        const float4* src = reinterpret_cast<const float4*>(g.pre_tab + (int64_t)img * g.cg.Cin * 2);
+        for (int i = tid; i < g.cg.Cin / 2; i += 512) reinterpret_cast<float4*>(smem + TAB0)[i] = src[i];
+    }
 
     int64_t h_off[H];
 #pragma unroll
@@ -1974,6 +1984,25 @@
             glds16(src, dst + (group < HGROUPS ? group : HGROUPS) * 1024);
         }
     };
+    auto transform_halo = [&](int chunk) {
+        char* hb = smem + HALO0 + (chunk & 1) * HALO_BYTES;
+        const float* tab = reinterpret_cast<const float*>(smem + TAB0) + chunk * BK * 2;
+        const f16x8 zero = {0, 0, 0, 0, 0, 0, 0, 0};
+#pragma unroll
+        for (int h = 0; h < H; ++h) {
+            if (h_off[h] < 0) continue;
+            f16x8* slot = reinterpret_cast<f16x8*>(hb + (h * 8 + wave) * 1024 + lane * 16);
+            const float4* t = reinterpret_cast<const float4*>(tab + (int)((h_off[h] >> 3) & 7) * 16);
+            float sc[8], sh[8];
+#pragma unroll
+            for (int q = 0; q < 4; ++q) {
+                const float4 v = t[q];
+                sc[2 * q] = v.x; sh[2 * q] = v.y; sc[2 * q + 1] = v.z; sh[2 * q + 1] = v.w;
+            }
+            *slot = gn_act8(*slot, sc, sh, zero, zero, g.pre_act);
+            __builtin_amdgcn_sched_barrier(0);
+        }
+    };
     const int rbase = wave * 8 + (lane >> 3);
     const int ls = (lane & 7) ^ ((rbase >> 1) & 7);
     const int b_row0 = (wave >> 2) * WTN + (wave & 3) * 8;
@@ -2037,6 +2066,11 @@
         } else {
             wait_vmcnt<0>();
         }
+        if (pre) {
+            lds_barrier();
+            transform_halo(t0.chunk);
+            asm volatile("s_waitcnt lgkmcnt(0)" ::: "memory");
+        }
     }
     t2 = t1;
     advance(t2);
@@ -2072,6 +2106,7 @@
                 if (halo_next) issue_halo(tc.chunk + 1);
                 if (halo_next) { if (has1) wait_vmcnt<LB + H>(); else wait_vmcnt<H>(); }
                 else { if (has1) wait_vmcnt<LB>(); else wait_vmcnt<0>(); }
+                if (pre && tc.ky == 0 && tc.kx == 1 && kt + 8 < kt_end) transform_halo(tc.chunk + 1);
             } else {
                 if (has2) {
 #pragma unroll
@@ -2118,7 +2153,7 @@
                   epi16_rows_if_enabled(BM, BN, WAVES_M, halo_lds_bytes(BN)), false, halo_lds_bytes(BN)>(g, acc, smem, m0, n0, z, zb, split);
 }
 
-template <int BN>
+template <int BN, bool PRE>
 __global__ void __launch_bounds__(256, 2) conv3_halo4_kernel(GemmArgs g) {
     constexpr int BM = 256, BK = 64, WAVES_M = 4, WAVES_N = 1;
     constexpr int TM = 2, TN = BN / 32;
@@ -2162,6 +2197,12 @@
     const int img = by / per_img, pr = by - img * per_img;
     const int py0 = (pr / g.cg.halo_tx) * 16 - 1, px0 = (pr % g.cg.halo_tx) * 16 - 1;
     const f16* Ab = g.A + (int64_t)img * g.cg.H * g.cg.W * g.cg.Cin;
+    constexpr int TAB0 = halo4_lds_bytes(BN);
+    constexpr bool pre = PRE;
+    if (pre) {
+        const float4* src = reinterpret_cast<const float4*>(g.pre_tab + (int64_t)img * g.cg.Cin * 2);
+        for (int i = tid; i < g.cg.Cin / 2; i += 256) reinterpret_cast<float4*>(smem + TAB0)[i] = src[i];
+    }
 
     int h_off[H];
 #pragma unroll
@@ -2185,6 +2226,24 @@
             glds16(src, smem + HALO0 + (group < HGROUPS ? group : HGROUPS) * 1024);
         }
     };
+    auto transform_halo = [&](int chunk) {
+        const float* tab = reinterpret_cast<const float*>(smem + TAB0) + chunk * BK * 2;
+        const f16x8 zero = {0, 0, 0, 0, 0, 0, 0, 0};
+#pragma unroll
+        for (int h = 0; h < H; ++h) {
+            if (h_off[h] < 0) continue;
+            f16x8* slot = reinterpret_cast<f16x8*>(smem + HALO0 + (h * 4 + wave) * 1024 + lane * 16);
+            const float4* t = reinterpret_cast<const float4*>(tab + ((h_off[h] >> 3) & 7) * 16);
+            float sc[8], sh[8];
+#pragma unroll
+            for (int q = 0; q < 4; ++q) {
+                const float4 v = t[q];
+                sc[2 * q] = v.x; sh[2 * q] = v.y; sc[2 * q + 1] = v.z; sh[2 * q + 1] = v.w;
+            }
+            *slot = gn_act8(*slot, sc, sh, zero, zero, g.pre_act);
+            __builtin_amdgcn_sched_barrier(0);
+        }
+    };
     const int rb = wave * 8 + (lane >> 3);
     const int ls = (lane & 7) ^ ((rb >> 1) & 7);
     const int64_t b_off0 = (int64_t)(n0 + rb) * g.ldw + ls * 8;
@@ -2218,6 +2277,11 @@
     for (int kt = kt_begin; kt < kt_end; ++kt) {
         const int cur = (kt - kt_begin) & 1;
         asm volatile("s_waitcnt vmcnt(0)" ::: "memory");
+        if (pre && ky == 0 && kx == 0) {
+            if (kt == kt_begin) lds_barrier();
+            transform_halo(chunk);
+            asm volatile("s_waitcnt lgkmcnt(0)" ::: "memory");
+        }
         __builtin_amdgcn_s_barrier();
         int nky = ky, nkx = kx + 1, nchunk = chunk;
         if (nkx == 3) { nkx = 0; if (++nky == 3) { nky = 0; ++nchunk; } }
@@ -2354,12 +2418,13 @@
 static int launch_conv3_halo(odise_hip_ctx* ctx, GemmArgs& g) {
     constexpr int lds = halo_lds_bytes(BN);
     static_assert(epi_lds_bytes(256, BN, 4, epi_wave_rows(256, BN, 4, lds)) <= lds, "epilogue staging exceeds the LDS request");
-    auto kern = conv3_halo_kernel<BN, PT>;
-    static LdsAttrOnce once;
-    ODISE_TRY(ensure_dyn_lds(ctx, once, (const void*)kern, lds));
+    static_assert(lds + kPreTabMaxBytes <= 160 * 1024, "the operand transform's table must fit");
+    auto kern = g.pre_tab ? conv3_halo_kernel<BN, PT, true> : conv3_halo_kernel<BN, PT, false>;
+    static LdsAttrOnce once[2];
+    ODISE_TRY(ensure_dyn_lds(ctx, once[g.pre_tab ? 1 : 0], (const void*)kern, lds + (g.pre_tab ? kPreTabMaxBytes : 0)));
     const int n_img = g.M / (g.cg.OH * g.cg.OW);
     dim3 grid((unsigned)ceil_div(g.N, BN), (unsigned)(n_img * g.cg.halo_tx * g.cg.halo_ty), (unsigned)(g.splitk > 1 ? g.splitk : 1));
-    hipLaunchKernelGGL(kern, grid, dim3(512), lds, ctx->stream, g);
+    hipLaunchKernelGGL(kern, grid, dim3(512), lds + (g.pre_tab ? g.cg.Cin * 8 : 0), ctx->stream, g);
     ODISE_CHECK_HIP(hipGetLastError());
     if (g.splitk > 1) {
         const int64_t total = (int64_t)g.M * ceil_div(g.N, 8);
@@ -2373,14 +2438,14 @@
 template <int BN>
 static int launch_conv3_halo4(odise_hip_ctx* ctx, GemmArgs& g) {
     constexpr int lds = halo4_lds_bytes(BN);
-    static_assert(2 * lds <= 160 * 1024, "two blocks must fit a CU's LDS");
+    static_assert(2 * (lds + kPreTabMaxBytes) <= 160 * 1024, "two blocks must fit a CU's LDS, with the operand transform's table");
     static_assert(epi_lds_bytes(256, BN, 4, epi_wave_rows(256, BN, 4, lds)) <= lds, "epilogue staging exceeds the LDS request");
-    auto kern = conv3_halo4_kernel<BN>;
-    static LdsAttrOnce once;
-    ODISE_TRY(ensure_dyn_lds(ctx, once, (const void*)kern, lds));
+    auto kern = g.pre_tab ? conv3_halo4_kernel<BN, true> : conv3_halo4_kernel<BN, false>;
+    static LdsAttrOnce once[2];
+    ODISE_TRY(ensure_dyn_lds(ctx, once[g.pre_tab ? 1 : 0], (const void*)kern, lds + (g.pre_tab ? kPreTabMaxBytes : 0)));
     const int n_img = g.M / (g.cg.OH * g.cg.OW);
     dim3 grid((unsigned)ceil_div(g.N, BN), (unsigned)(n_img * g.cg.halo_tx * g.cg.halo_ty), (unsigned)(g.splitk > 1 ? g.splitk : 1));
-    hipLaunchKernelGGL(kern, grid, dim3(256), lds, ctx->stream, g);
+    hipLaunchKernelGGL(kern, grid, dim3(256), lds + (g.pre_tab ? g.cg.Cin * 8 : 0), ctx->stream, g);
     ODISE_CHECK_HIP(hipGetLastError());
     if (g.splitk > 1) {
         const int64_t total = (int64_t)g.M * ceil_div(g.N, 8);
@@ -2454,6 +2519,9 @@
     return rc;
 }
 
+constexpr int kPrenormDeclined = 1;
+static const float* const kPrenormQuery = reinterpret_cast<const float*>(16);
+
 static int flags_early() { return g_conv_flags | env_gemm_flags(); }
 template <bool CONV>
 static int launch_gemm_select(odise_hip_ctx* ctx, GemmArgs& g, int batch, int force_tile, int force_split, unsigned tile_mask) {
@@ -2508,6 +2576,10 @@
     }
     if (force_tile >= 0 && force_tile < kNumTiles && !(force_tile == 6 && !pp_ok) && !(force_tile >= 7 && force_tile <= 9 && !(halo_ok && pp_base)))
         tile = force_tile;
+    if (g.pre_tab) {
+        if (!(CONV && tile >= 7 && !g.cg.ups && g.N <= kTileBN[tile] && g.cg.Cin * 8 <= kPreTabMaxBytes)) return kPrenormDeclined;
+        if (g.pre_tab == kPrenormQuery) return ODISE_OK;
+    }
     g.splitk = 1;
     g.ktiles_per_split = nk;
     if (force_split > 0 && batch == 1) best_split = std::min(force_split, nk);
@@ -2625,13 +2697,28 @@
         ODISE_REQUIRE((!ln->part || (ln->P > 0 && ln->colsum)) && (!ln->fin || ln->rowsum), "gemm_ln: incomplete LayerNorm terms");
     }
     g.cg = ConvGeom{};
+    g.pre_tab = nullptr; g.pre_act = 0;
     if (ln) return launch_gemm<false>(ctx, g, batch, force_tile, 1, ln->stats_out ? (1u << 4) : (1u << 4) | (1u << 5));
     return launch_gemm<false>(ctx, g, batch, force_tile, force_split);
 }
 
 int gemm_ln(odise_hip_ctx* ctx, const odise_gemm_desc* d, const LnEpi& ln) { return gemm_forced(ctx, d, -1, 1, &ln); }
 
+static int conv_impl(odise_hip_ctx* ctx, const odise_conv_desc* d, int force_tile, int force_split, float* gn_stats, int* stats_blocks,
+                     const float* pre_tab, int pre_act);
 int conv_forced(odise_hip_ctx* ctx, const odise_conv_desc* d, int force_tile, int force_split, float* gn_stats, int* stats_blocks) {
+    return conv_impl(ctx, d, force_tile, force_split, gn_stats, stats_blocks, nullptr, 0);
+}
+
+int conv_prenorm(odise_hip_ctx* ctx, const odise_conv_desc* d, const float* table, int act, float* gn_stats, int* stats_blocks) {
+    ODISE_REQUIRE(ctx && d, "conv2d_prenorm: null argument");
+    if (stats_blocks) *stats_blocks = 0;
+    if (d->N == 0 || d->KH != 3 || d->KW != 3 || d->stride != 1 || d->upsample2x || conv3_c8_ok(d)) return kPrenormDeclined;
+    return conv_impl(ctx, d, -1, 0, gn_stats, stats_blocks, table ? table : kPrenormQuery, act);
+}
+
+static int conv_impl(odise_hip_ctx* ctx, const odise_conv_desc* d, int force_tile, int force_split, float* gn_stats, int* stats_blocks,
+                     const float* pre_tab, int pre_act) {
     ODISE_REQUIRE(ctx && d, "conv2d: null argument");
     ODISE_REQUIRE(d->N >= 0 && d->H > 0 && d->W > 0 && d->Cin > 0 && d->Cout > 0, "conv2d: bad dims");
     ODISE_REQUIRE(d->Cin % 8 == 0, "conv2d: Cin=%d must be a multiple of 8 (pad the input channels)", d->Cin);
@@ -2639,7 +2726,7 @@
     ODISE_REQUIRE(d->X && d->Wt && d->Y, "conv2d: null device pointer");
     ODISE_REQUIRE(((uintptr_t)d->X & 15) == 0 && ((uintptr_t)d->Wt & 15) == 0, "conv2d: X/Wt must be 16-byte aligned");
     if (d->N == 0) return ODISE_OK;
-    if (force_tile < 0 && force_split <= 0 && conv3_c8_ok(d)) return launch_conv3_c8(ctx, d, gn_stats, stats_blocks);
+    if (force_tile < 0 && force_split <= 0 && !pre_tab && conv3_c8_ok(d)) return launch_conv3_c8(ctx, d, gn_stats, stats_blocks);
     GemmArgs g;
     g.M = d->N * d->OH * d->OW;
     g.N = d->Cout;
@@ -2660,10 +2747,12 @@
     g.cg.H = d->H; g.cg.W = d->W; g.cg.Cin = d->Cin; g.cg.KH = d->KH; g.cg.KW = d->KW;
     g.cg.stride = d->stride; g.cg.pad_t = d->pad_t; g.cg.pad_l = d->pad_l; g.cg.OH = d->OH; g.cg.OW = d->OW;
     g.cg.ups = d->upsample2x;
+    g.pre_tab = pre_tab; g.pre_act = pre_act;
     const int64_t in_bytes = (int64_t)d->N * d->H * d->W * d->Cin * 2;
     g.cg.chunk_major = (d->Cin % 64 == 0 && d->KH * d->KW > 1 && in_bytes <= (128ll << 20)) ? 1 : 0;
+    if (pre_tab == kPrenormQuery) return launch_gemm_select<true>(ctx, g, 1, force_tile, force_split, ~0u);
     if (d->KH == 1 && d->KW == 1 && d->stride == 1 && d->pad_t == 0 && d->pad_l == 0 && !d->upsample2x && d->OH == d->H &&
-        d->OW == d->W) {
+        d->OW == d->W && !pre_tab) {
         g.lda = d->Cin;
         return launch_gemm<false>(ctx, g, 1, force_tile, force_split);
     }
@@ -2674,6 +2763,8 @@
 
 int group_norm_from_colpart(odise_hip_ctx* ctx, const void* x, void* y, const float* gamma, const float* beta, int N, int HW, int C, int groups,
                             float eps, int act, const float* colpart, int nblk);
+int group_norm_table(odise_hip_ctx* ctx, const void* x, const float* gamma, const float* beta, int N, int HW, int C, int groups, float eps,
+                     const float* colpart, int nblk, float* table);
 
 }
 
@@ -2707,3 +2798,21 @@
         return odise::group_norm_from_colpart(ctx, d->Y, y_norm, gamma, beta, d->N, d->OH * d->OW, d->Cout, groups, eps, act, stats_scratch, *stats_blocks);
     return odise_hip_group_norm(ctx, d->Y, y_norm, gamma, beta, d->N, d->OH * d->OW, d->Cout, groups, eps, act);
 }
+extern "C" int odise_hip_conv2d_prenorm(odise_hip_ctx* ctx, const odise_conv_desc* d, const float* gamma, const float* beta, int groups, float eps,
+                                        int act, const float* colpart, int nblk, float* table, void* x_norm) {
+    using namespace odise;
+    ODISE_REQUIRE(ctx && d && table, "conv2d_prenorm: null argument");
+    const int HW = d->H * d->W;
+    const int rc = conv_prenorm(ctx, d, nullptr, act, nullptr, nullptr);
+    if (rc == ODISE_OK) {
+        ODISE_TRY(group_norm_table(ctx, d->X, gamma, beta, d->N, HW, d->Cin, groups, eps, colpart, nblk, table));
+        return conv_prenorm(ctx, d, table, act, nullptr, nullptr);
+    }
+    if (rc != kPrenormDeclined) return rc;
+    ODISE_REQUIRE(x_norm, "conv2d_prenorm: this shape takes the two-pass form, which needs x_norm");
+    if (colpart && nblk > 0) ODISE_TRY(group_norm_from_colpart(ctx, d->X, x_norm, gamma, beta, d->N, HW, d->Cin, groups, eps, act, colpart, nblk));
+    else ODISE_TRY(odise_hip_group_norm(ctx, d->X, x_norm, gamma, beta, d->N, HW, d->Cin, groups, eps, act));
+    odise_conv_desc d2 = *d;
+    d2.X = x_norm;
+    return conv_forced(ctx, &d2, -1, 0);
+}
diff --git a/odise_amd/csrc/norm.hip b/odise_amd/csrc/norm.hip
--- a/odise_amd/csrc/norm.hip
+++ b/odise_amd/csrc/norm.hip
@@ -73,7 +73,8 @@
 }
 
 __global__ void __launch_bounds__(256) gn_finalize_kernel(const float* __restrict__ partial, float* __restrict__ stats, int HW, int C, int G,
-                                                         int nchunks, float eps) {
+                                                         int nchunks, float eps, const float* __restrict__ gamma,
+                                                         const float* __restrict__ beta, float* __restrict__ table) {
     __shared__ double red[2 * 256];
     const int n = blockIdx.x, tid = threadIdx.x;
     const int cpg = C / G;
@@ -100,14 +101,23 @@
         const double mu = s / cnt;
         double var = q / cnt - mu * mu;
         if (var < 0.0) var = 0.0;
-        stats[((int64_t)n * G + tid) * 2] = (float)mu;
-        stats[((int64_t)n * G + tid) * 2 + 1] = (float)(1.0 / sqrt(var + (double)eps));
+        const float muf = (float)mu, rsf = (float)(1.0 / sqrt(var + (double)eps));
+        stats[((int64_t)n * G + tid) * 2] = muf;
+        stats[((int64_t)n * G + tid) * 2 + 1] = rsf;
+        if (table) {
+            for (int c = tid * cpg; c < (tid + 1) * cpg; ++c) {
+                float* o = table + ((int64_t)n * C + c) * 2;
+                gn_scale_shift(muf, rsf, gamma ? gamma[c] : 1.f, beta ? beta[c] : 0.f, o[0], o[1]);
+            }
+        }
     }
 }
 
 __global__ void __launch_bounds__(256) gn_finalize_cols_kernel(const float* __restrict__ colpart, float* __restrict__ stats, int HW, int C, int G,
-                                                              int nblk, float eps) {
+                                                              int nblk, float eps, const float* __restrict__ gamma,
+                                                              const float* __restrict__ beta, float* __restrict__ table) {
     __shared__ double red[2 * 256];
+    __shared__ float fin[2];
     const int gI = blockIdx.x, n = blockIdx.y, tid = threadIdx.x;
     const int cpg = C / G;
     double s = 0.0, q = 0.0;
@@ -141,8 +151,17 @@
         const double mu = red[0] / cnt;
         double var = red[1] / cnt - mu * mu;
         if (var < 0.0) var = 0.0;
-        stats[((int64_t)n * G + gI) * 2] = (float)mu;
-        stats[((int64_t)n * G + gI) * 2 + 1] = (float)(1.0 / sqrt(var + (double)eps));
+        fin[0] = (float)mu;
+        fin[1] = (float)(1.0 / sqrt(var + (double)eps));
+        stats[((int64_t)n * G + gI) * 2] = fin[0];
+        stats[((int64_t)n * G + gI) * 2 + 1] = fin[1];
+    }
+    if (table) {
+        __syncthreads();
+        for (int c = gI * cpg + tid; c < (gI + 1) * cpg; c += 256) {
+            float* o = table + ((int64_t)n * C + c) * 2;
+            gn_scale_shift(fin[0], fin[1], gamma ? gamma[c] : 1.f, beta ? beta[c] : 0.f, o[0], o[1]);
+        }
     }
 }
 
@@ -191,9 +210,7 @@
         const int gI = c / cpg;
         const float mu = nchunks > 0 ? gstat[2 * gI] : stats[((int64_t)n * G + gI) * 2];
         const float rs = nchunks > 0 ? gstat[2 * gI + 1] : stats[((int64_t)n * G + gI) * 2 + 1];
-        const float sc = rs * (gamma ? gamma[c] : 1.f);
-        scale[c] = sc;
-        shift[c] = (beta ? beta[c] : 0.f) - mu * sc;
+        gn_scale_shift(mu, rs, gamma ? gamma[c] : 1.f, beta ? beta[c] : 0.f, scale[c], shift[c]);
     }
     __syncthreads();
     const int C8 = C >> 3;
@@ -225,19 +242,7 @@
             const float4 h0 = *reinterpret_cast<const float4*>(shift + c0), h1 = *reinterpret_cast<const float4*>(shift + c0 + 4);
             const float sc[8] = {s0.x, s0.y, s0.z, s0.w, s1.x, s1.y, s1.z, s1.w};
             const float sh[8] = {h0.x, h0.y, h0.z, h0.w, h1.x, h1.y, h1.z, h1.w};
-            float t[8];
-#pragma unroll
-            for (int i = 0; i < 8; ++i) t[i] = (float)v[u][i] * sc[i] + sh[i] + (float)r[u][i];
-            if (act == ODISE_ACT_SILU) {
-#pragma unroll
-                for (int i = 0; i < 8; ++i) t[i] = mul_sigmoid(t[i], t[i]);
-            } else if (act != ODISE_ACT_NONE) {
-#pragma unroll
-                for (int i = 0; i < 8; ++i) t[i] = act_apply(t[i], act);
-            }
-            f16x8 o;
-#pragma unroll
-            for (int i = 0; i < 8; ++i) o[i] = (f16)(t[i] + (float)a[u][i]);
+            const f16x8 o = gn_act8(v[u], sc, sh, r[u], a[u], act);
             __builtin_nontemporal_store(o, reinterpret_cast<f16x8*>(yb + (int64_t)idx * 8));
         }
     }
@@ -396,6 +401,47 @@
     }
 }
 
+static int gn_partials(odise_hip_ctx* ctx, const void* x, int N, int HW, int C, int groups, int* nchunks_out, float** partial, float** stats) {
+    const int V = C / 8;
+    const int VW = V < 256 ? V : 256;
+    const int PL = 256 / VW;
+    int64_t want = std::max<int64_t>(1, (int64_t)ctx->cu_count * g_gn_chunk_factor / N);
+    int64_t maxc = std::max<int64_t>(1, HW / (4 * PL));
+    int nchunks = (int)std::min<int64_t>(std::min<int64_t>(want, maxc), 256);
+    const int ppc = (int)ceil_div(HW, nchunks);
+    nchunks = (int)ceil_div(HW, ppc);
+    const size_t pbytes = ((size_t)N * nchunks * groups * 2 + (size_t)N * groups * 2) * sizeof(float);
+    ODISE_REQUIRE(pbytes <= ctx->ws_bytes, "group_norm: workspace too small");
+    *partial = (float*)ctx->ws;
+    *stats = *partial + (size_t)N * nchunks * groups * 2;
+    *nchunks_out = nchunks;
+    hipLaunchKernelGGL(gn_partial_kernel, dim3(nchunks, N), dim3(256), 2 * (size_t)PL * C * sizeof(float), ctx->stream, (const f16*)x,
+                       *partial, HW, C, groups, ppc);
+    ODISE_CHECK_HIP(hipGetLastError());
+    return ODISE_OK;
+}
+
+int group_norm_table(odise_hip_ctx* ctx, const void* x, const float* gamma, const float* beta, int N, int HW, int C, int groups, float eps,
+                     const float* colpart, int nblk, float* table) {
+    ODISE_REQUIRE(ctx && x && table, "group_norm_table: null argument");
+    ODISE_REQUIRE(N > 0 && HW > 0 && C > 0 && groups > 0 && groups <= 256, "group_norm_table: bad dims");
+    ODISE_REQUIRE(C % groups == 0 && C % 8 == 0 && C <= GN_MAX_C, "group_norm_table: C=%d must be a multiple of 8 and of groups=%d, <= %d", C, groups, GN_MAX_C);
+    ODISE_REQUIRE((int64_t)HW * (C / 8) < (1ll << 31) - (1 << 24), "group_norm_table: image too large");
+    if (colpart && nblk > 0) {
+        ODISE_REQUIRE((size_t)N * groups * 2 * sizeof(float) <= ctx->ws_bytes, "group_norm_table: workspace too small");
+        hipLaunchKernelGGL(gn_finalize_cols_kernel, dim3(groups, N), dim3(256), 0, ctx->stream, colpart, (float*)ctx->ws, HW, C, groups, nblk, eps,
+                           gamma, beta, table);
+    } else {
+        int nchunks = 0;
+        float* partial = nullptr;
+        float* stats = nullptr;
+        ODISE_TRY(gn_partials(ctx, x, N, HW, C, groups, &nchunks, &partial, &stats));
+        hipLaunchKernelGGL(gn_finalize_kernel, dim3(N), dim3(256), 0, ctx->stream, partial, stats, HW, C, groups, nchunks, eps, gamma, beta, table);
+    }
+    ODISE_CHECK_HIP(hipGetLastError());
+    return ODISE_OK;
+}
+
 }
 
 extern "C" int odise_hip_group_norm_ex(odise_hip_ctx* ctx, const void* x, void* y, const float* gamma, const float* beta, int N,
@@ -414,25 +460,15 @@
     ODISE_REQUIRE(C % groups == 0 && C % 8 == 0 && C <= GN_MAX_C, "group_norm: C=%d must be a multiple of 8 and of groups=%d, <= %d", C, groups, GN_MAX_C);
     ODISE_REQUIRE(groups <= 256, "group_norm: groups=%d > 256", groups);
     if (N == 0) return ODISE_OK;
-    const int V = C / 8;
-    const int VW = V < 256 ? V : 256;
-    const int PL = 256 / VW;
     ODISE_REQUIRE((int64_t)HW * (C / 8) < (1ll << 31) - (1 << 24), "group_norm: image too large");
-    int64_t want = std::max<int64_t>(1, (int64_t)ctx->cu_count * g_gn_chunk_factor / N);
-    int64_t maxc = std::max<int64_t>(1, HW / (4 * PL));
-    int nchunks = (int)std::min<int64_t>(std::min<int64_t>(want, maxc), 256);
-    const int ppc = (int)ceil_div(HW, nchunks);
-    nchunks = (int)ceil_div(HW, ppc);
-    const size_t pbytes = ((size_t)N * nchunks * groups * 2 + (size_t)N * groups * 2) * sizeof(float);
-    ODISE_REQUIRE(pbytes <= ctx->ws_bytes, "group_norm: workspace too small");
-    float* partial = (float*)ctx->ws;
-    float* stats = partial + (size_t)N * nchunks * groups * 2;
-    hipLaunchKernelGGL(gn_partial_kernel, dim3(nchunks, N), dim3(256), 2 * (size_t)PL * C * sizeof(float), ctx->stream, (const f16*)x,
-                       partial, HW, C, groups, ppc);
-    ODISE_CHECK_HIP(hipGetLastError());
+    int nchunks = 0;
+    float* partial = nullptr;
+    float* stats = nullptr;
+    ODISE_TRY(gn_partials(ctx, x, N, HW, C, groups, &nchunks, &partial, &stats));
     const bool fold_in_apply = g_gn_fold_in_apply && nchunks <= 64;
     if (!fold_in_apply) {
-        hipLaunchKernelGGL(gn_finalize_kernel, dim3(N), dim3(256), 0, ctx->stream, partial, stats, HW, C, groups, nchunks, eps);
+        hipLaunchKernelGGL(gn_finalize_kernel, dim3(N), dim3(256), 0, ctx->stream, partial, stats, HW, C, groups, nchunks, eps, (const float*)nullptr,
+                           (const float*)nullptr, (float*)nullptr);
         ODISE_CHECK_HIP(hipGetLastError());
     }
     const int64_t total = (int64_t)HW * (C / 8);
@@ -451,7 +487,8 @@
     ODISE_REQUIRE((int64_t)HW * (C / 8) < (1ll << 31) - (1 << 24), "group_norm: image too large");
     ODISE_REQUIRE((size_t)N * groups * 2 * sizeof(float) <= ctx->ws_bytes, "group_norm: workspace too small");
     float* stats = (float*)ctx->ws;
-    hipLaunchKernelGGL(gn_finalize_cols_kernel, dim3(groups, N), dim3(256), 0, ctx->stream, colpart, stats, HW, C, groups, nblk, eps);
+    hipLaunchKernelGGL(gn_finalize_cols_kernel, dim3(groups, N), dim3(256), 0, ctx->stream, colpart, stats, HW, C, groups, nblk, eps,
+                       (const float*)nullptr, (const float*)nullptr, (float*)nullptr);
     ODISE_CHECK_HIP(hipGetLastError());
     const int64_t total = (int64_t)HW * (C / 8);
     const int bpi = (int)std::max<int64_t>(1, ceil_div(total, 256 * 4));
```

Result: no change. 52.08 (median of 6 runs) (+0.1%).
